# ducha-aiki/pydegensac

Hardware: AMD Instinct MI355X
Metric: models/sec, findFundamentalMatrix @2000 corrs (LO-RANSAC + DEGENSAC, batched pairs) (higher is better)
Workload: dtype f64

## Files before the change

include/mi_degensac.h:

```cpp
#ifndef MI_DEGENSAC_H
#define MI_DEGENSAC_H
#include <stdint.h>

#ifdef __cplusplus
extern "C" {
#endif

#define MI_DEGENSAC_OK        0
#define MI_DEGENSAC_EINVAL   -1
#define MI_DEGENSAC_ENODEV   -2
#define MI_DEGENSAC_EHIP     -3
#define MI_DEGENSAC_ENOMEM   -4

#define MI_DEGENSAC_F_SAMPSON        0
#define MI_DEGENSAC_F_SYMM_EPIPOLAR  1
#define MI_DEGENSAC_H_SAMPSON        0
#define MI_DEGENSAC_H_SYMM_SQ_MAX    1
#define MI_DEGENSAC_H_SYMM_MAX       2
#define MI_DEGENSAC_H_SYMM_SQ_SUM    3
#define MI_DEGENSAC_H_SYMM_SUM       4

#define MI_DEGENSAC_FLAG_FINAL_LAF_FILTER 1u

#define MI_DEGENSAC_FLAG_LEGACY_F 2u
// ... 150 lines not shown
const char *mi_degensac_match_last_error(void);

int mi_degensac_match_knn2_batch_dev(int norm, const void *d_desc1, const void *d_desc2, const int64_t *offsets1_host,
                                     const int64_t *offsets2_host, int n_pairs, int dim, int device, void *stream,
                                     int32_t *d_idx, float *d_dist);
int mi_degensac_match_fginn_knn2_batch_dev(int norm, const void *d_desc1, const void *d_desc2, const int64_t *offsets1_host,
                                           const int64_t *offsets2_host, int n_pairs, int dim, const double *d_kp2, int kp_dim,
                                           double spatial_th, int device, void *stream, int32_t *d_idx, float *d_dist);
typedef struct mi_degensac_match_params {
    int32_t norm;
    int32_t dim;
    float   ratio;
    int32_t mutual;
    int32_t struct_size;
    int32_t second_nn;
    double  spatial_th;
} mi_degensac_match_params;
int mi_degensac_match_verify_batch_dev(int homography, const mi_degensac_match_params *mp, const void *d_desc1, const void *d_desc2,
                                       const int64_t *offsets1_host, const int64_t *offsets2_host, const double *d_kp1, const double *d_kp2,
                                       int kp_dim, int n_pairs, const mi_degensac_params *prm, const uint32_t *d_seeds, int device, void *stream,
                                       double *d_model, int32_t *d_match, uint8_t *d_inlier, int32_t *d_stats, int32_t *h_counts );
int mi_degensac_match_verify_batch(int homography, const mi_degensac_match_params *mp, const void *desc1, const void *desc2,
                                   const int64_t *offsets1, const int64_t *offsets2, const double *kp1, const double *kp2, int kp_dim,
                                   int n_pairs, const mi_degensac_params *prm, const uint32_t *seeds, int device,
                                   double *model, int32_t *match, uint8_t *inlier, int32_t *stats , int32_t *counts );

int mi_degensac_match_knn2_pairs_dev(int norm, const void *d_desc1, const void *d_desc2, const int64_t *offsets1_host, int n_images1,
                                     const int64_t *offsets2_host, int n_images2, const int32_t *pairs_host, int n_pairs, int dim,
                                     int device, void *stream, int32_t *d_idx, float *d_dist);
int mi_degensac_match_verify_pairs_dev(int homography, const mi_degensac_match_params *mp, const void *d_desc1, const void *d_desc2,
                                       const int64_t *offsets1_host, int n_images1, const int64_t *offsets2_host, int n_images2,
                                       const double *d_kp1, const double *d_kp2, int kp_dim, const int32_t *pairs_host, int n_pairs,
                                       const mi_degensac_params *prm, const uint32_t *d_seeds, int device, void *stream, double *d_model,
                                       int32_t *d_match, uint8_t *d_inlier, int32_t *d_stats, int32_t *h_counts );
int mi_degensac_match_verify_pairs(int homography, const mi_degensac_match_params *mp, const void *desc1, const void *desc2,
                                   const int64_t *offsets1, int n_images1, const int64_t *offsets2, int n_images2, const double *kp1,
                                   const double *kp2, int kp_dim, const int32_t *pairs, int n_pairs, const mi_degensac_params *prm,
                                   const uint32_t *seeds, int device, double *model, int32_t *match, uint8_t *inlier,
                                   int32_t *stats , int32_t *counts );

typedef struct mi_degensac_guide_params {
    int32_t homography;
    int32_t error_type;
    double  px_th;
    int32_t struct_size;
    int32_t reserved;
} mi_degensac_guide_params;
int mi_degensac_match_guided_knn2_batch_dev(int norm, const void *d_desc1, const void *d_desc2, const int64_t *offsets1_host,
                                            const int64_t *offsets2_host, int n_pairs, int dim, const double *d_kp1, const double *d_kp2,
                                            int kp_dim, const double *d_models, const mi_degensac_guide_params *gp, int device, void *stream,
                                            int32_t *d_idx, float *d_dist);
int mi_degensac_match_guided_batch_dev(const mi_degensac_match_params *mp, const void *d_desc1, const void *d_desc2, const int64_t *offsets1_host,
                                       const int64_t *offsets2_host, const double *d_kp1, const double *d_kp2, int kp_dim, int n_pairs,
                                       const double *d_models, const mi_degensac_guide_params *gp, int device, void *stream, int32_t *d_idx,
                                       float *d_dist, int32_t *d_match, int32_t *d_counts , int32_t *h_counts );
int mi_degensac_match_guided_batch(const mi_degensac_match_params *mp, const void *desc1, const void *desc2, const int64_t *offsets1,
                                   const int64_t *offsets2, const double *kp1, const double *kp2, int kp_dim, int n_pairs, const double *models,
                                   const mi_degensac_guide_params *gp, int device, int32_t *idx, float *dist, int32_t *match,
                                   int32_t *counts );

int mi_degensac_score_models(const double *pts1, const double *pts2, int n, int dim,
                             const double *models, int n_models, int kind, double th, int device,
                             uint32_t *I, double *J, double *resid );
int mi_degensac_sample_stream(uint32_t seed, int n, int sample_size, int iters, int device,
                              int32_t *samples );
int mi_degensac_sample_stream_ex(uint32_t seed, int n, int sample_size, int iters, int device,
                                 int seq_pool, int32_t *samples);
int mi_degensac_solve7(const double *pts1, const double *pts2, int n, int dim,
                       const int32_t *samples, int n_samples, int device,
                       int32_t *nsol, int32_t *root_idx , double *models );
int mi_degensac_mat3(int op, const double *in, int count, int device, double *out, int32_t *flag);
int mi_degensac_screen_counts(const double *pts1, const double *pts2, int n, int dim, const double *models, int n_models,
                              int kind, double th, int device, uint32_t *c1, uint32_t *c2);

int mi_degensac_screen_counts_h(const double *pts1, const double *pts2, int n, int dim, const double *models, int n_models,
                                double th, int device, uint32_t *cnt, uint8_t *cand);

int mi_degensac_rng_wave(uint32_t seed, int skip, int block, int count, int device, int32_t *out);

#define MI_DEGENSAC_TIMING_LEN 8
int mi_degensac_set_call_timing(int on);
int mi_degensac_last_call_timing(double *out );

int         mi_degensac_device_count(void);
const char *mi_degensac_last_error(void);
const char *mi_degensac_version(void);
const char *mi_degensac_kernel_name(int homography);
int         mi_degensac_pool_stage_parallel(int device);

#ifdef __cplusplus
}
#endif
#endif
```

pydegensac_amd/_lib.py:

```python
import ctypes as C
import os
import numpy as np

_HERE = os.path.dirname(os.path.abspath(__file__))
LIB_PATH = os.environ.get("MI_DEGENSAC_LIB") or os.path.join(_HERE, "libmi_degensac.so")
STATS_LEN = 16
STAT_NAMES = ["samples", "lo_runs", "rejected", "I", "models", "degen", "Ih", "best_sample",
              "full_passes", "ex_passes", "h_passes", "aux_passes", "ticks_best", "ticks_total", "threads", "placement"]
FLAG_FINAL_LAF_FILTER = 1
FLAG_LEGACY_F = 2
FLAG_NO_STREAM, FLAG_STREAM_ON, FLAG_NO_HJOB, FLAG_STREAM_AUTO, FLAG_HJOB_ON = 4, 8, 16, 64, 128


def FLAG_STREAM_TEST(b): return (int(b) & 3) << 8
TUNE_LATENCY, TUNE_THROUGHPUT, TUNE_THROUGHPUT4 = 1, 2, 3
TUNE_PLACE_HBM, TUNE_PLACE_LDS, TUNE_PLACE_POOL_LDS = 1 << 2, 2 << 2, 3 << 2
TUNE_SEQ_POOL = 1 << 4
TUNE_H_SERIAL_LO = 1 << 5
TUNE_COOP_ALL_PASSES = 1 << 6
TUNE_F_SERIAL_REPS = 1 << 7


def TUNE_HELPERS(h): return (int(h) & 255) << 8
def TUNE_SET_ASIDE(t): return (int(t) & 255) << 16
# ... 106 lines not shown
        l.mi_degensac_ctx_destroy.argtypes = [C.c_void_p]
        l.mi_degensac_ctx_stream.restype = C.c_void_p
        l.mi_degensac_ctx_stream.argtypes = [C.c_void_p]
        if hasattr(l, "mi_degensac_ctx_set_scheduling"):
            l.mi_degensac_ctx_set_scheduling.restype = C.c_int
            l.mi_degensac_ctx_set_scheduling.argtypes = [C.c_void_p, C.c_int, C.c_int]
        l.mi_degensac_release_scratch.restype = C.c_int
        l.mi_degensac_release_scratch.argtypes = [C.c_int, C.c_void_p]
        l.mi_degensac_pool_stage_parallel.restype = C.c_int
        l.mi_degensac_pool_stage_parallel.argtypes = [C.c_int]
        l.mi_degensac_sample_stream_ex.restype = C.c_int
        l.mi_degensac_sample_stream_ex.argtypes = [C.c_uint32, C.c_int, C.c_int, C.c_int, C.c_int, C.c_int, ip]
        l.mi_degensac_score_models.restype = C.c_int
        l.mi_degensac_score_models.argtypes = [dp, dp, C.c_int, C.c_int, dp, C.c_int, C.c_int, C.c_double, C.c_int, up, dp, dp]
        l.mi_degensac_sample_stream.restype = C.c_int
        l.mi_degensac_sample_stream.argtypes = [C.c_uint32, C.c_int, C.c_int, C.c_int, C.c_int, ip]
        l.mi_degensac_solve7.restype = C.c_int
        l.mi_degensac_solve7.argtypes = [dp, dp, C.c_int, C.c_int, ip, C.c_int, C.c_int, ip, ip, dp]
        for name in ("mi_degensac_find_fundamental_resids", "mi_degensac_find_homography_resids"):
            f = getattr(l, name); f.restype = C.c_int
            f.argtypes = [dp, dp, C.c_int, C.c_int, pp, C.c_uint32, C.c_int, dp, bp, ip, dp, C.c_int]
        l.mi_degensac_find_fundamental_hist.restype = C.c_int
        l.mi_degensac_find_fundamental_hist.argtypes = [dp, dp, C.c_int, C.c_int, pp, C.c_uint32, C.c_int, dp, bp, ip, ip]
        l.mi_degensac_match.restype = C.c_int
        l.mi_degensac_match.argtypes = [C.c_int, C.c_void_p, C.c_int, C.c_void_p, C.c_int, C.c_int, C.c_float, C.c_int, C.c_int, ip,
                                        C.POINTER(C.c_float), bp]
        l.mi_degensac_match_knn2_dev.restype = C.c_int
        l.mi_degensac_match_knn2_dev.argtypes = [C.c_int, C.c_void_p, C.c_int, C.c_void_p, C.c_int, C.c_int, C.c_int, C.c_void_p, C.c_void_p, C.c_void_p]
        l.mi_degensac_match_filter_dev.restype = C.c_int
        l.mi_degensac_match_filter_dev.argtypes = [C.c_void_p, C.c_void_p, C.c_int, C.c_float, C.c_void_p, C.c_int, C.c_void_p, C.c_void_p]
        l.mi_degensac_match_knn2_batch_dev.restype = C.c_int
        l.mi_degensac_match_knn2_batch_dev.argtypes = [C.c_int, C.c_void_p, C.c_void_p, lp, lp, C.c_int, C.c_int, C.c_int, C.c_void_p, C.c_void_p,
                                                       C.c_void_p]
        if hasattr(l, "mi_degensac_match_fginn_knn2_batch_dev"):
            l.mi_degensac_match_fginn_knn2_batch_dev.restype = C.c_int
            l.mi_degensac_match_fginn_knn2_batch_dev.argtypes = [C.c_int, C.c_void_p, C.c_void_p, lp, lp, C.c_int, C.c_int, C.c_void_p, C.c_int,
                                                                 C.c_double, C.c_int, C.c_void_p, C.c_void_p, C.c_void_p]
        mpp = C.POINTER(MatchParams)
        l.mi_degensac_match_verify_batch_dev.restype = C.c_int
        l.mi_degensac_match_verify_batch_dev.argtypes = [C.c_int, mpp, C.c_void_p, C.c_void_p, lp, lp, C.c_void_p, C.c_void_p, C.c_int, C.c_int, pp,
                                                         C.c_void_p, C.c_int, C.c_void_p, C.c_void_p, C.c_void_p, C.c_void_p, C.c_void_p, ip]
        l.mi_degensac_match_verify_batch.restype = C.c_int
        l.mi_degensac_match_verify_batch.argtypes = [C.c_int, mpp, C.c_void_p, C.c_void_p, lp, lp, dp, dp, C.c_int, C.c_int, pp, up, C.c_int,
                                                     dp, ip, bp, ip, ip]
        if hasattr(l, "mi_degensac_match_knn2_pairs_dev"):
            l.mi_degensac_match_knn2_pairs_dev.restype = C.c_int
            l.mi_degensac_match_knn2_pairs_dev.argtypes = [C.c_int, C.c_void_p, C.c_void_p, lp, C.c_int, lp, C.c_int, ip, C.c_int, C.c_int, C.c_int,
                                                           C.c_void_p, C.c_void_p, C.c_void_p]
            l.mi_degensac_match_verify_pairs_dev.restype = C.c_int
            l.mi_degensac_match_verify_pairs_dev.argtypes = [C.c_int, mpp, C.c_void_p, C.c_void_p, lp, C.c_int, lp, C.c_int, C.c_void_p, C.c_void_p,
                                                             C.c_int, ip, C.c_int, pp, C.c_void_p, C.c_int, C.c_void_p, C.c_void_p, C.c_void_p,
                                                             C.c_void_p, C.c_void_p, ip]
            l.mi_degensac_match_verify_pairs.restype = C.c_int
            l.mi_degensac_match_verify_pairs.argtypes = [C.c_int, mpp, C.c_void_p, C.c_void_p, lp, C.c_int, lp, C.c_int, dp, dp, C.c_int, ip, C.c_int,
                                                         pp, up, C.c_int, dp, ip, bp, ip, ip]
        gpp = C.POINTER(GuideParams)
        l.mi_degensac_match_guided_knn2_batch_dev.restype = C.c_int
        l.mi_degensac_match_guided_knn2_batch_dev.argtypes = [C.c_int, C.c_void_p, C.c_void_p, lp, lp, C.c_int, C.c_int, C.c_void_p, C.c_void_p, C.c_int,
                                                              C.c_void_p, gpp, C.c_int, C.c_void_p, C.c_void_p, C.c_void_p]
        l.mi_degensac_match_guided_batch_dev.restype = C.c_int
        l.mi_degensac_match_guided_batch_dev.argtypes = [mpp, C.c_void_p, C.c_void_p, lp, lp, C.c_void_p, C.c_void_p, C.c_int, C.c_int, C.c_void_p, gpp,
                                                         C.c_int, C.c_void_p, C.c_void_p, C.c_void_p, C.c_void_p, C.c_void_p, ip]
        l.mi_degensac_match_guided_batch.restype = C.c_int
        l.mi_degensac_match_guided_batch.argtypes = [mpp, C.c_void_p, C.c_void_p, lp, lp, dp, dp, C.c_int, C.c_int, dp, gpp, C.c_int, ip,
                                                     C.POINTER(C.c_float), ip, ip]
        l.mi_degensac_kpts_to_xyA.restype = C.c_int
        l.mi_degensac_kpts_to_xyA.argtypes = [C.POINTER(C.c_float), C.c_int, C.c_int, dp]
        l.mi_degensac_kpts_to_xyA_dev.restype = C.c_int
        l.mi_degensac_kpts_to_xyA_dev.argtypes = [C.c_void_p, C.c_int, C.c_int, C.c_void_p, C.c_void_p]
        l.mi_degensac_match_last_error.restype = C.c_char_p
        l.mi_degensac_mat3.restype = C.c_int
        l.mi_degensac_mat3.argtypes = [C.c_int, dp, C.c_int, C.c_int, dp, ip]
        l.mi_degensac_screen_counts.restype = C.c_int
        l.mi_degensac_screen_counts.argtypes = [dp, dp, C.c_int, C.c_int, dp, C.c_int, C.c_int, C.c_double, C.c_int, up, up]
        l.mi_degensac_screen_counts_h.restype = C.c_int
        l.mi_degensac_screen_counts_h.argtypes = [dp, dp, C.c_int, C.c_int, dp, C.c_int, C.c_double, C.c_int, up, bp]
        l.mi_degensac_rng_wave.restype = C.c_int
        l.mi_degensac_rng_wave.argtypes = [C.c_uint32, C.c_int, C.c_int, C.c_int, C.c_int, ip]
        if hasattr(l, "mi_degensac_set_call_timing"):
            l.mi_degensac_set_call_timing.restype = C.c_int
            l.mi_degensac_set_call_timing.argtypes = [C.c_int]
            l.mi_degensac_last_call_timing.restype = C.c_int
            l.mi_degensac_last_call_timing.argtypes = [dp]
        l.mi_degensac_last_error.restype = C.c_char_p
        l.mi_degensac_version.restype = C.c_char_p
        l.mi_degensac_kernel_name.restype = C.c_char_p
        l.mi_degensac_device_count.restype = C.c_int
        _lib = l
    return _lib


def check(rc):
    if rc != 0:
        msg = lib().mi_degensac_last_error().decode()
        if rc == -1:
            raise ValueError(msg)
        raise MiDegensacError(f"mi_degensac error {rc}: {msg}")


def check_match(rc):
    if rc != 0:
        msg = lib().mi_degensac_match_last_error().decode()
        if rc == -1:
            raise ValueError(msg)
        raise MiDegensacError(f"mi_degensac error {rc}: {msg}")


def dptr(a):
    return a.ctypes.data_as(C.POINTER(C.c_double))


def make_params(px_th, conf, max_iters, error_type, sym_check, laf_coef, degen=True, flags=0, tuning=0):
    return Params(float(px_th), float(conf), int(max_iters), int(error_type), int(bool(sym_check)), int(bool(degen)),
                  float(laf_coef), int(flags), int(tuning))


def set_stream_mode(mode):
    f = lib().mi_degensac_set_stream_mode
    f.restype = C.c_int; f.argtypes = [C.c_int]
    return int(f(int(mode)))


def set_hjob_mode(mode):
    f = lib().mi_degensac_set_hjob_mode
    f.restype = C.c_int; f.argtypes = [C.c_int]
    return int(f(int(mode)))


def set_wait_ticks(ticks):
    return int(lib().mi_degensac_set_wait_ticks(int(ticks)))


TIMING_NAMES = ["call_ms", "pack_ms", "enqueue_ms", "wait_ms", "unpack_ms", "dev_h2d_ms", "dev_kernel_ms", "dev_d2h_ms"]


def set_call_timing(on):
    return int(lib().mi_degensac_set_call_timing(int(bool(on))))


def last_call_timing():
    out = (C.c_double * len(TIMING_NAMES))()
    check(lib().mi_degensac_last_call_timing(out))
    return {k: float(v) for k, v in zip(TIMING_NAMES, out)}


def stats_dict(st):
    d = {k: int(v) for k, v in zip(STAT_NAMES, st)}
    d["set_aside"] = (d["placement"] >> 8) & 1
    d["streamed"] = (d["placement"] >> 9) & 1
    d["discarded"] = (d["placement"] >> 10) & 1
    d["rerun"] = (d["placement"] >> 11) & 1
    d["placement"] &= 255
    return d
```

pydegensac_amd/csrc/dg_f_lo.h:

```cpp
#ifndef DG_F_LO_H
#define DG_F_LO_H

__device__ __forceinline__ unsigned dg_hash_list(const int *list, int count, bool small_ids = false)
{
    if (count <= 0) return 0;
    const int lane = (int)(threadIdx.x & 63);
    unsigned hash = (unsigned)__builtin_amdgcn_readfirstlane(count * 4), tmp;
#define DG_HSTEP(v_) { unsigned v = (unsigned)(v_); \
        hash += v & 0xffffu; tmp = ((v >> 16) << 11) ^ hash; hash = (hash << 16) ^ tmp; hash += hash >> 11; }
#define DG_HSTEP16(v_) { unsigned v = (unsigned)(v_); \
        hash += v; hash = (hash << 16) ^ hash; hash += hash >> 11; }
    int k = 0;
    int cur = (lane < count) ? list[lane] : 0;
    int n1 = (64 + lane < count) ? list[64 + lane] : 0, n2 = (128 + lane < count) ? list[128 + lane] : 0, n3 = (192 + lane < count) ? list[192 + lane] : 0;
    for (; k + 64 <= count; k += 64) {
        const int n4 = (k + 256 + lane < count) ? list[k + 256 + lane] : 0;
        if (small_ids) {
#pragma unroll
            for (int i = 0; i < 64; i++) DG_HSTEP16(__builtin_amdgcn_readlane(cur, i))
        } else {
#pragma unroll
            for (int i = 0; i < 64; i++) DG_HSTEP(__builtin_amdgcn_readlane(cur, i))
        }
        cur = n1; n1 = n2; n2 = n3; n3 = n4;
// ... 357 lines not shown
                DG_WSYNC();
                dg_rand_skip(&S->lo_work, assumed, lane);
            }
        }
        __syncthreads();
        DG_LW(0);
        if constexpr (COOP) dg_lo_round_coop<LDSPTS>(c, nr, ssiz, th, mk_full, mk_ex);
        else {
            const int wv = __builtin_amdgcn_readfirstlane(wave);
            if (wv < __builtin_amdgcn_readfirstlane(nr)) dg_lo_rep_wave<LDSPTS>(c, &S->lo[wv], ssiz, th, mk_full, mk_ex, lane, wv);
        }
        __syncthreads();
        DG_LW(1);
        if (tid == 0) {
            int v = 0;
            for (int q = 0; q < nr; q++) {
                dg_lo_log *g = LG(q);
                if (g->aborted) break;
                const int id = *iterID + next + q + 1;
                int draws = 0, cut = 0, n_ex = 0;
                if (g->I0 >= 8) {
                    draws = g->drew0;
                    for (int i = 0; i < g->nit; i++) {
                        n_ex++;
                        const int ret = dg_ht_contains(c.ht, g->it[i].hash, g->it[i].I, id);
                        if (ret == -1) dg_ht_insert(c.ht, g->it[i].hash, g->it[i].I, id);
                        if (ret != -1 && ret != id) { cut = 1; break; }
                        draws += g->it[i].drew;
                    }
                }
                g->cut = cut; g->draws = draws; g->n_ex = n_ex; g->n_fd = (!cut && g->has_fin) ? 2 : 1;
                v++;
                if (draws != assumed) break;
            }
            S->red.bi[0] = v;
        }
        __syncthreads();
        DG_LW(2);
        const int v = S->red.bi[0];
#ifdef DG_LO_PROF
        if (tid == 0) { S->lt[5] += 100000; S->lt[6] += 100000 * v; }
#endif
        for (int q = 0; q < v; q++) {
            const dg_lo_log *g = LG(q);
            c.n_exfds += g->n_ex; c.n_fds += g->n_fd;
            const int cut = g->cut;
            if (!cut && maxS.J < g->J) {
                maxS.I = (unsigned)g->I; maxS.J = g->J; maxS.Is = 0; maxS.Ilafs = 0; *kindBest = g->kind0;
                const int *ibq = COOP ? dg_coop_lo_list(*c.A, c.coop_slot, 2 * q) : c.K->wlist + (size_t)q * c.K->n_max;
                __syncthreads();
                if (tid < 9) Fout[tid] = g->f[tid];
                for (int j = tid; j < g->I; j += DG_T) intbuff_best[j] = ibq[j];
                __syncthreads();
            }
        }
        __syncthreads();
        DG_LW(3);
        if (__builtin_amdgcn_readfirstlane(wave) == 0) {
            for (int q = nr - 1; q >= v; q--) {
                if (lane < 2 * ssiz && LG(q)->upos[lane] >= 0) inliers[LG(q)->upos[lane]] = LG(q)->uval[lane];
                DG_WSYNC();
            }
            if (lane == 0) S->rng = LG(v - 1)->g0;
            DG_WSYNC();
            dg_rand_skip(&S->rng, LG(v - 1)->draws, lane);
        }
        next += v;
        if constexpr (COOP) {
            for (int q = 0; q < v; q++) { const int d = LG(q)->draws; if (d == c.lo_prev || c.lo_prev < 0) assumed = d; c.lo_prev = d; }
        }
#ifdef DG_LO_PROF
        __syncthreads();
#endif
        DG_LW(4);
    }
    if constexpr (COOP) c.lo_assumed = assumed;
    *iterID += DG_RAN_REP;
    __syncthreads();
    for (int j = tid; j < (int)maxS.I; j += DG_T) inliers[j] = intbuff_best[j];
    __syncthreads();
    return maxS;
}

template <int LDSPTS>
__device__ __forceinline__ dg_score dg_inFrani(CTX &c, int ninl, double th, double *Fout, int *iterID, int mk_full, int mk_ex, int *kindBest)
{
    if (c.rrun || c.A->innerh_serial || c.A->trace) return dg_inFrani_serial<LDSPTS>(c, ninl, th, Fout, iterID, mk_full, mk_ex, kindBest);
    if (c.cb) {
        if constexpr (LDSPTS == 0) return dg_inFrani_waves<LDSPTS, true>(c, ninl, th, Fout, iterID, mk_full, mk_ex, kindBest);
        else return dg_inFrani_serial<LDSPTS>(c, ninl, th, Fout, iterID, mk_full, mk_ex, kindBest);
    }
    return dg_inFrani_waves<LDSPTS, false>(c, ninl, th, Fout, iterID, mk_full, mk_ex, kindBest);
}

#endif
```

pydegensac_amd/csrc/dg_f_sched.h:

```cpp
#ifndef DG_F_SCHED_H
#define DG_F_SCHED_H

#define DG_FLAST(M) do { if (legacy_sym) { __syncthreads(); if (tid < 9) S->flast[tid] = (M)[tid]; D.flast_k = no_sam; __syncthreads(); } } while (0)
#define DG_PARK_SPARE   0
#define DG_PARK_CLAIMED 32
#define DG_PARK_HEAD    64
#define DG_PARK_DYN_OFF ((sizeof(dg_f_shared) + 255) & ~(size_t)255)

__device__ __forceinline__ void dg_copy16(void *dst, const void *src, size_t bytes, int tid)
{
    const size_t nv = bytes / 16;
    const uint4 *s4 = (const uint4 *)src; uint4 *d4 = (uint4 *)dst;
    for (size_t i = tid; i < nv; i += DG_T) d4[i] = s4[i];
    const size_t done = nv * 16;
    for (size_t i = done + tid; i < bytes; i += DG_T) ((unsigned char *)dst)[i] = ((const unsigned char *)src)[i];
}

__device__ __forceinline__ long long dg_park_take(const dg_args &A, long long *bc , const int q)
{
    __syncthreads();
    if (__builtin_amdgcn_readfirstlane((int)(threadIdx.x >> 6)) == 0) {
        int *const p_head = A.park_ctl + DG_PARK_HEAD + 64 * q, *const p_cl = A.park_ctl + DG_PARK_CLAIMED + 64 * q;
        const long long *const pq = A.park_q + (size_t)q * A.park_cap;
        int h;
        for (;;) {
            h = __builtin_amdgcn_readfirstlane(__hip_atomic_load(p_head, __ATOMIC_RELAXED, __HIP_MEMORY_SCOPE_AGENT));
            const int cl = __builtin_amdgcn_readfirstlane(__hip_atomic_load(p_cl, __ATOMIC_RELAXED, __HIP_MEMORY_SCOPE_AGENT));
            if (h >= cl) { h = -1; break; }
            int ok = 0;
            if (threadIdx.x == 0) {
                int expect = h;
                ok = __hip_atomic_compare_exchange_strong(p_head, &expect, h + 1, __ATOMIC_RELAXED, __ATOMIC_RELAXED, __HIP_MEMORY_SCOPE_AGENT) ? 1 : 0;
            }
            if (__builtin_amdgcn_readfirstlane(ok)) break;
        }
        long long e = -1;
        if (h >= 0) {
            for (;;) {
                const long long v = __hip_atomic_load(pq + h, __ATOMIC_RELAXED, __HIP_MEMORY_SCOPE_AGENT);
                const int lo = __builtin_amdgcn_readfirstlane((int)(v & 0xffffffffll)), hi = __builtin_amdgcn_readfirstlane((int)(v >> 32));
                e = ((long long)hi << 32) | (unsigned)lo;
                if (e >= 0) break;
                __builtin_amdgcn_s_sleep(4);
            }
            __builtin_amdgcn_fence(__ATOMIC_ACQUIRE, "agent");
        }
        *bc = e;
    }
    __syncthreads();
    return *bc;
}

#define DG_STREAM_TIMEOUT 400000000ll
__device__ __forceinline__ dg_stream_ent *dg_stream_entry(const dg_args &A, int oslot, int seq)
{
    return (dg_stream_ent *)(A.ring + ((size_t)oslot * A.stream_depth + (size_t)(seq % A.stream_depth)) * A.stream_ent_bytes);
}
template <class Pred>
__device__ __forceinline__ int dg_stream_wait(const dg_args &A, int *flag, int *stop, Pred pred, int *bc , const long long limit = DG_STREAM_TIMEOUT)
{
    __syncthreads();
    if (__builtin_amdgcn_readfirstlane((int)(threadIdx.x >> 6)) == 0) {
        const long long t0 = wall_clock64();
        int v;
        for (;;) {
            v = __builtin_amdgcn_readfirstlane(__hip_atomic_load(flag, __ATOMIC_RELAXED, __HIP_MEMORY_SCOPE_AGENT));
            if (pred(v) && limit != 0) break;
            if (stop && __builtin_amdgcn_readfirstlane(__hip_atomic_load(stop, __ATOMIC_RELAXED, __HIP_MEMORY_SCOPE_AGENT))) { v = -1; break; }
            if (wall_clock64() - t0 > limit) { if (threadIdx.x == 0) __hip_atomic_store(A.err_flag, 1, __ATOMIC_RELAXED, __HIP_MEMORY_SCOPE_AGENT); v = -1;
                break; }
            __builtin_amdgcn_s_sleep(8);
        }
        __builtin_amdgcn_fence(__ATOMIC_ACQUIRE, "agent");
        *bc = v;
    }
    __syncthreads();
    return *bc;
}
__device__ __forceinline__ void dg_stream_publish(int *flag, int v)
{
    __syncthreads();
    if (__builtin_amdgcn_readfirstlane((int)(threadIdx.x >> 6)) == 0) {
        __builtin_amdgcn_fence(__ATOMIC_RELEASE, "agent");
        asm volatile("s_waitcnt vmcnt(0)" ::: "memory");
        if (threadIdx.x == 0) __hip_atomic_store(flag, v, __ATOMIC_RELAXED, __HIP_MEMORY_SCOPE_AGENT);
    }
// ... 49 lines not shown
```

pydegensac_amd/csrc/dg_kernel_common.h:

```cpp
#ifndef DG_KERNEL_COMMON_H
#define DG_KERNEL_COMMON_H
#include "dg_geom.h"

#ifndef DG_CHUNK
#define DG_CHUNK   256
#endif
#ifdef MI_DEGENSAC_DEV
#define DG_CLK() wall_clock64()
#define DG_DEVT(x) x
#else
#define DG_CLK() 0ll
#define DG_DEVT(x) do {} while (0)
#endif
#ifndef DG_MINW
#define DG_MINW    2
#endif
#define DG_MCAP    96
#define DG_HT_CAP  4096
#define DG_MTAB_BYTES ((((size_t)3 * DG_CHUNK * 9 * sizeof(double)) + 255) & ~(size_t)255)
#define DG_PRE_BYTES  ((size_t)DG_CHUNK * 2 * sizeof(int))

#define DG_ITER_SAM 50
#define DG_RAN_REP 10
#define DG_ILSQ_ITERS 4
#define DG_TC 4
#define DG_MWM (9/4)

struct dg_params {
    double th;
    double sym_th;
    double laf_coef;
    double conf;
    int    max_iters;
    int    error_type;
    int    degen;
    int    final_laf_filter;
    int    h2_do_lo, h2_inl_limit;
    int    legacy;
};

struct dg_ws_layout {
    size_t stride;
    size_t off_lists;
    size_t off_flags;
    size_t off_ht;
    size_t off_models;
    size_t off_pts;
    size_t off_pool;
    size_t off_stage;
    size_t off_wave;
    size_t off_res;
    size_t off_mslot;
    size_t off_park;
    size_t off_hjbuf;
    size_t off_job;
    size_t off_hrep;
    int    hrep;
    int    n_max;
};

struct dg_hrep_it { double hl[9]; double J; unsigned hash; int I; };
struct alignas(128) dg_hrep_log {
    double h0[9]; double J0; int I0;
    int nit;
    int last_short;
    int has_fin;
    dg_hrep_it it[4];
    double hf[9]; double Jf; int If;
    int ids[12];
};

struct dg_coop_cb {
    int gen;
    int done;
    int next;
    int fpad0;
    unsigned long long tau_bits;
    int fpad[26];
    int stage, n_units, Mtot, n, kind, slice, use_l1, err;
    double th, ext[4];
    int mtab, mpad;
    double ppad[6];
};
static_assert(sizeof(dg_coop_cb) == 256, "control block = two 128-byte lines");

struct dg_coop_job {
    double F[9], thJ, thL, thL2;
    int kind, wantJ, listStrict, has_list, has_list2, slice, n, pad;
};
struct dg_coop_rec { unsigned I, nL, nL2, nJ; };
#define DG_COOP_MAX_SLICES 64

enum { DG_ST_IDLE = 0, DG_ST_REQ = 1, DG_ST_BUSY = 2, DG_ST_ATTACHED = 3, DG_ST_RELEASED = 4 };
struct dg_stream_cb {
    int state;
    int head;
    int tail;
    int stop;
    int owner_sam;
    int max_sam;
    unsigned long long tau_bits;
    int claim;
    int fpad[23];
    int pair, wsid, img_sam, fan_kind;
    double fan_th, fan_ext[4];
    int ppad[18];
};
static_assert(sizeof(dg_stream_cb) == 256, "stream control block = two 128-byte lines");

struct dg_hjob_cb {
    int gen;
    int next;
    int done;
    int fpad[29];
    int n, kind, ssiz, wsid; double th; int ppad[26];
};
static_assert(sizeof(dg_hjob_cb) == 256, "job control block = two 128-byte lines");

struct dg_args {
    const double *pts1, *pts2;
    const long long *offsets;
    const unsigned *seeds;
    double *model_out;
    unsigned char *mask_out;
    int *stats_out;
    char *ws;
    dg_ws_layout wl;
    dg_params prm;
    int dim, n_pairs, pts_in_lds;
    int dev_knob;
    double *resids_out;
    int resid_runs;
    int lo_width;
    int *hist_out;
    int *screen_out;
    int *ticket;
    const int *order;
    int coop_k;
    int coop_pass_min;
    dg_coop_cb *coop;
    int park_sam;
    int n_res, n_ws;
    int dyn_bytes;
    int *park_ctl;
    long long *park_q;
    int park_cap;
    int park_long;
    int lo_serial;
    int pool_seq;
    int innerh_serial;
    int variant_threads, mode;
    int stream_on;
    int stream_early;
    int stream_min_sam, stream_min_left;
    int stream_depth;
    int stream_test;
    size_t stream_ent_bytes;
    dg_stream_cb *scb;
    char *ring;
    int *done_pairs;
    dg_hjob_cb *hjob;
    int fan_k;
    int fan_ws0;
    int *fan_flags;
    int *err_flag;
    int *trace;
    int trace_cap;
    int wait_ticks;
    long long *phase_out;
};

__device__ __forceinline__ bool dg_wait_count(const dg_args &A, int *cnt, int target, int code, int sleep_ticks)
{
    const long long t0 = wall_clock64(), limit = (long long)A.wait_ticks;
    for (;;) {
// ... 194 lines not shown
```

pydegensac_amd/csrc/dg_kernel_f.h:

```cpp
#ifndef DG_KERNEL_F_H
#define DG_KERNEL_F_H
#include <stddef.h>
#include "dg_lsq.h"

struct dg_score { unsigned I; double J; unsigned Is; unsigned Ilafs; };

#define DG_WPAD ((2 * DG_CHUNK * 7 * 4 > DG_NW * (int)sizeof(dg_wave_ws)) ? (2 * DG_CHUNK * 7 * 4 - DG_NW * (int)sizeof(dg_wave_ws) + 7) / 8 : 1)
struct dg_f_drv {
    dg_score maxS, maxSs;
    int no_sam, max_sam, iter_cnt, degen_cnt, iterID, Ihmax; unsigned non_degen;
    int best_sample; long long t_best, t_start;
    long long t_parked;
    int flast_k, has_last;
    int finKind, accepted, perm[4], p4, e4kind, track, done;
    unsigned seed; int cur, chunk_s[3], chunk_base;
    int n_fds, n_exfds, n_hds, n_aux;
};

#ifndef DG_LO_AHEAD_MAX
#define DG_LO_AHEAD_MAX 5
#endif
#define DG_LO_AHEAD (DG_NW - 1 < DG_LO_AHEAD_MAX ? DG_NW - 1 : DG_LO_AHEAD_MAX)
struct dg_lo_ahead { dg_rng before, after; int pos[32], val[32]; double F[9]; };

// ... 76 lines not shown

struct dg_stream_ev { double model[9]; double J; unsigned I; short k; unsigned char r, pad; unsigned char ridx[4]; };
#define DG_STREAM_EV_MAX 40
struct dg_stream_ent {
    int cn, Mtot, n_ev, overflow; double tau_used, pad1;
    unsigned seeds[DG_CHUNK]; int draws[DG_CHUNK][8];
    unsigned char nv[DG_CHUNK];
    dg_stream_ev ev[DG_STREAM_EV_MAX];
};

template <int LDSPTS>
struct dg_f_ctx {
    dg_f_shared *S;
    const __attribute__((address_space(3))) dg_f_cshared *K;
    const dg_pt *P;
    int *pool;
    int n, tid;
    const dg_args *A;
    long long off;
    dg_ht ht;
    unsigned *seeds; int (*draws)[8];
    int n_fds, n_exfds, n_hds, n_aux;
    double *rrun;
    dg_coop_cb *cb; int *coop_gen; int coop_slot;
    double *hlt;
    int hjob_gen;
    int lo_assumed, lo_prev;

    __device__ __forceinline__ dg_pt pt(int i) const { return P[i]; }
    __device__ __forceinline__ dg_pt laf_pt(int i, int which) const {
        const double *a = A->pts1 + (size_t)(off + i) * 6, *b = A->pts2 + (size_t)(off + i) * 6;
        dg_pt p;
        if (which == 1) { p.x1 = a[0] + a[3]; p.y1 = a[1] + a[5]; p.x2 = b[0] + b[3]; p.y2 = b[1] + b[5]; }
        else            { p.x1 = a[0] + a[2]; p.y1 = a[1] + a[4]; p.x2 = b[0] + b[2]; p.y2 = b[1] + b[4]; }
        return p;
    }
};

#define DG_JBUF_LDS_BYTES (offsetof(dg_f_shared, wpad) + sizeof(((dg_f_shared *)0)->wpad) - offsetof(dg_f_shared, ww))
static_assert(offsetof(dg_f_shared, wpad) == offsetof(dg_f_shared, ww) + sizeof(((dg_f_shared *)0)->ww), "ww and wpad must be contiguous");
static_assert(DG_JBUF_LDS_BYTES >= 2 * DG_CHUNK * 7 * sizeof(int), "pool-stage scratch does not fit");

__device__ __forceinline__ void dg_fill_views(dg_f_cshared *K, char *ws, const dg_ws_layout &wl)
{
    for (int i = 0; i < 10; i++) K->L[i] = (int *)(ws + wl.off_lists) + (size_t)i * wl.n_max;
    for (int i = 0; i < 5; i++) K->Fl[i] = (unsigned char *)(ws + wl.off_flags) + (size_t)i * wl.n_max;
    K->gmodels = (double *)(ws + wl.off_models);
    K->stage = (dg_pt *)(ws + wl.off_stage);
    K->res_J = (double *)(ws + wl.off_res); K->res_I = (unsigned *)(K->res_J + 3 * DG_CHUNK); K->rf = (int (*)[5])(K->res_I + 3 * DG_CHUNK);
    K->hrep = wl.hrep ? ws + wl.off_hrep : (char *)0;
    K->n_max = wl.n_max; K->wlist = (int *)(ws + wl.off_wave); K->wstage = (dg_pt *)(ws + wl.off_wave + (size_t)DG_NW * wl.n_max * sizeof(int));
}

#define CTX dg_f_ctx<LDSPTS>
#define DG_RESIDS_M 62

template <int LDSPTS>
__device__ __forceinline__ void dg_dump_resid(CTX &c, int row, const double *M, int kind)
{
    if (!c.rrun) return;
    double m[9], Hinv[9], H1[9];
#pragma unroll
    for (int i = 0; i < 9; i++) { m[i] = M[i]; Hinv[i] = 0; H1[i] = 0; }
    if (kind > 10) dg_hsym_prepare(m, Hinv, H1);
    double *out = c.rrun + (size_t)row * c.n;
    for (int j = c.tid; j < c.n; j += DG_T) {
        const dg_pt q = dg_ldpt<LDSPTS>(c.P, j);
        out[j] = kind < 10 ? dg_Ferr(kind, m, q) : dg_Herr(kind - 10, m, Hinv, H1, q);
    }
}
template <int LDSPTS>
__device__ __forceinline__ void dg_resid_begin(CTX &c, int run )
{
    c.rrun = 0;
    if (!c.A->resids_out || run >= c.A->resid_runs) return;
    c.rrun = c.A->resids_out + ((size_t)c.off * c.A->resid_runs + (size_t)run * c.n) * DG_RESIDS_M;
    const double nan_ = __longlong_as_double(0x7ff8000000000000ll);
    for (size_t j = c.tid; j < (size_t)DG_RESIDS_M * c.n; j += DG_T) c.rrun[j] = nan_;
}

#define DG_TRACE(c, tag, I, J) do { if ((c).A->trace && (c).tid == 0) { int *t_ = (c).A->trace; int k_ = t_[0]; \
    if (k_ < (c).A->trace_cap) { long long jb_ = __double_as_longlong((double)(J)); t_[1+4*k_] = (tag); t_[2+4*k_] = (int)(I); \
    t_[3+4*k_] = (int)(jb_ & 0xffffffffll); t_[4+4*k_] = (int)(jb_ >> 32); t_[0] = k_ + 1; } } } while (0)

template <int LDSPTS>
__device__ __noinline__ dg_pass_res dg_coop_pass(CTX &c, const double *Fm , int kind, const dg_pass_cfg &cfg);

template <int LDSPTS>
__device__ __forceinline__ dg_pass_res dg_f_pass(CTX &c, const double *Fm , int kind, dg_pass_cfg cfg)
{
    if (LDSPTS == 0 && c.cb && !cfg.src && !cfg.flags && !cfg.wantC && cfg.n >= c.A->coop_pass_min) return dg_coop_pass<LDSPTS>(c, Fm, kind, cfg);
    double F[9];
#pragma unroll
    for (int i = 0; i < 9; i++) F[i] = Fm[i];
    const dg_pt *P = c.P;
    cfg.jbuf = (double *)c.K->stage; cfg.jl = (double *)c.S->ww; cfg.jl_cap = (int)(DG_JBUF_LDS_BYTES / sizeof(double));
    return dg_pass(&c.S->red, cfg, [&](int pid, int) { return dg_Ferr(kind, F, dg_ldpt<LDSPTS>(P, pid)); }, c.tid);
}
template <int LDSPTS>
__device__ __forceinline__ dg_pass_res dg_h_pass(CTX &c, const double *Hm , dg_pass_cfg cfg)
{
    double H[9];
#pragma unroll
    for (int i = 0; i < 9; i++) H[i] = Hm[i];
    const dg_pt *P = c.P;
    cfg.jbuf = (double *)c.K->stage; cfg.jl = (double *)c.S->ww; cfg.jl_cap = (int)(DG_JBUF_LDS_BYTES / sizeof(double));
    return dg_pass(&c.S->red, cfg, [&](int pid, int) { dg_pt p = dg_ldpt<LDSPTS>(P, pid); return dg_HDs(H, p.x1, p.y1, p.x2, p.y2); }, c.tid);
}
__device__ __forceinline__ dg_pass_cfg dg_cfg0(int n)
{
    dg_pass_cfg c; c.n = n; c.src = 0; c.p0 = 0; c.wantJ = 0; c.thJ = 0; c.jbuf = 0; c.jl = 0; c.jl_cap = 0; c.wantC = 0; c.thC = 0; c.list = 0; c.thL = 0;
        c.listStrict = 0; c.list2 = 0; c.thL2 = 0; c.flags = 0; c.thF = 0;
    return c;
}

template <int LDSPTS>
__device__ __forceinline__ void dg_gather(CTX &c, const int *ids, int len, double *px)
{
    for (int i = 0; i < len; i++) { dg_pt p = dg_ldpt<LDSPTS>(c.P, ids[i]); px[4*i] = p.x1; px[4*i+1] = p.y1; px[4*i+2] = p.x2; px[4*i+3] = p.y2; }
}

template <int LDSPTS>
__device__ __forceinline__ void dg_gather_wave(CTX &c, int id, int len, double *px, int lane)
{
    if (lane < len) { dg_pt p = dg_ldpt<LDSPTS>(c.P, id); px[4*lane] = p.x1; px[4*lane+1] = p.y1; px[4*lane+2] = p.x2; px[4*lane+3] = p.y2; }
}

template <int LDSPTS>
__device__ __forceinline__ void dg_u2f_list(CTX &c, const int *list, int len, const double *wmodel, int wkind, double *Fout)
{
    dg_f_shared *S = c.S;
    if (len <= 16) {
        __syncthreads();
        if (c.tid < 64) {
            const int lane = c.tid;
            dg_gather_wave(c, lane < len ? list[lane] : 0, len, S->lsq.px, lane);
            if (wmodel && lane < len) {
                dg_pt q = dg_ldpt<LDSPTS>(c.P, list[lane]);
                if (wkind == DG_K_FDS) S->lsq.part[0][lane] = dg_exFDs_w(wmodel, q.x1, q.y1, q.x2, q.y2);
                else { double w; dg_exFDsSym(wmodel, q.x1, q.y1, q.x2, q.y2, &w); S->lsq.part[0][lane] = w; }
            }
            DG_WSYNC();
            dg_u2f_small_w(&S->lsq, S->lsq.px, wmodel ? S->lsq.part[0] : 0, len, Fout, c.tid);
        }
        __syncthreads();
    } else {
        const dg_pt *P = c.P;
        dg_u2f_big(&S->red, &S->lsq, [&](int i) { return dg_ldpt<LDSPTS>(P, i); }, list, len, c.tid, Fout, c.K->stage, 2 * c.K->n_max,
                   DG_LSQ_LTAB(S));
    }
}

template <int LDSPTS>
__device__ __forceinline__ int dg_f_checks(CTX &c, const double *f, const int *list, int cnt, dg_score &S, const dg_score &maxS, int mkind)
{
    const dg_params &pr = c.A->prm;
    if (pr.sym_th > 0) {
        dg_pass_cfg cfg = pr.legacy ? dg_cfg0(c.n) : dg_cfg0(cnt); if (!pr.legacy) cfg.src = list; cfg.wantC = 1; cfg.thC = pr.sym_th;
        dg_pass_res r = dg_f_pass(c, f, DG_K_FSYM, cfg);
        S.Is = r.C;
        if (S.Is < maxS.Is) return 0;
    }
    if (pr.laf_coef > 0) {
        double thl = pr.laf_coef * pr.th;
        double F[9];
        for (int i = 0; i < 9; i++) F[i] = f[i];
        dg_pass_cfg cfg = dg_cfg0(cnt); cfg.src = list; cfg.wantC = 1; cfg.thC = thl;
        dg_pass_res r1 = dg_pass(&c.S->red, cfg, [&](int pid, int) { return dg_Ferr(mkind, F, c.laf_pt(pid, 1)); }, c.tid);
        dg_pass_res r2 = dg_pass(&c.S->red, cfg, [&](int pid, int) { return dg_Ferr(mkind, F, c.laf_pt(pid, 2)); }, c.tid);
        S.Ilafs = r2.C < r1.C ? r2.C : r1.C;
        if (S.Ilafs < maxS.Ilafs) { if (c.tid == 0) c.S->n_lafrej++; return 0; }
    }
    return 1;
}

template <int LDSPTS>
__device__ __noinline__ int dg_checksample(CTX &c, const double *F , const double (*u7)[4] , double th, double *H )
{
    dg_f_shared *S = c.S; const int tid = c.tid, lane = tid & 63, wave = tid >> 6;
    __syncthreads();
#if DG_NW >= 5
    for (int tr = wave; tr < 5; tr += DG_NW) {
        dg_wave_ws *w = &S->ww[wave];
        const unsigned char IDXS[5][3] = {{0,1,2}, {3,4,5}, {0,1,6}, {3,4,6}, {2,5,6}};
        if (lane == 0) {
            dg_Hdetect(F, u7, IDXS[tr], w->H);
            for (int j = 0; j < 7; j++) { w->Ds[j] = dg_HDs(w->H, u7[j][0], u7[j][1], u7[j][2], u7[j][3]); w->sDs[j] = w->Ds[j]; w->idx[j] = j; }
            for (int a = 0; a < 7; ++a)
                for (int b = a + 1; b < 7; ++b)
                    if (w->sDs[b] < w->sDs[a]) { double t = w->sDs[b]; w->sDs[b] = w->sDs[a]; w->sDs[a] = t; int ti = w->idx[b]; w->idx[b] = w->idx[a];
                        w->idx[a] = ti; }
            for (int j = 0; j < 5; ++j) { const double *q = u7[w->idx[j]]; w->cpx[4*j] = q[0]; w->cpx[4*j+1] = q[1]; w->cpx[4*j+2] = q[2]; w->cpx[4*j+3] = q[3];
                }
        }
        DG_WSYNC();
        dg_u2h_norm_w(w, w->cpx, 5, w->H, lane);
        if (lane == 0) {
            int inlCount = 0;
            for (int j = 0; j < 7; ++j) if (dg_HDs(w->H, u7[j][0], u7[j][1], u7[j][2], u7[j][3]) < th) ++inlCount;
            S->csRes[tr] = inlCount > 4;
            for (int j = 0; j < 9; j++) S->csH[tr][j] = w->H[j];
        }
        DG_WSYNC();
    }
#else
    static_assert(sizeof(dg_lsq_scratch) >= (size_t)DG_NW * DG_X2_DOUBLES * sizeof(double), "second-problem scratch");
    for (int base = wave; base < 5; base += 2 * DG_NW) {
        dg_wave_ws *w = &S->ww[wave];
        double *x2 = (double *)&S->lsq + (size_t)wave * DG_X2_DOUBLES;
        const bool uph = lane >= 32, two = base + DG_NW < 5, mine = (lane & 31) == 0 && (!uph || two);
        const int tr = uph ? base + DG_NW : base;
        double *Hh = uph ? x2 + DG_X2_USER : w->H, *Ds = uph ? x2 + DG_X2_USER + 9 : w->Ds, *sDs = uph ? x2 + DG_X2_USER + 16 : w->sDs;
        int *idx = uph ? (int *)(x2 + DG_X2_USER + 23) : w->idx;
        double *cpx = uph ? x2 + DG_X2_USER + 27 : w->cpx;
        const unsigned char IDXS[5][3] = {{0,1,2}, {3,4,5}, {0,1,6}, {3,4,6}, {2,5,6}};
        if (mine) {
            dg_Hdetect(F, u7, IDXS[tr], Hh);
            for (int j = 0; j < 7; j++) { Ds[j] = dg_HDs(Hh, u7[j][0], u7[j][1], u7[j][2], u7[j][3]); sDs[j] = Ds[j]; idx[j] = j; }
            for (int a = 0; a < 7; ++a)
                for (int b = a + 1; b < 7; ++b)
                    if (sDs[b] < sDs[a]) { double t = sDs[b]; sDs[b] = sDs[a]; sDs[a] = t; int ti = idx[b]; idx[b] = idx[a]; idx[a] = ti; }
            for (int j = 0; j < 5; ++j) { const double *q = u7[idx[j]]; cpx[4*j] = q[0]; cpx[4*j+1] = q[1]; cpx[4*j+2] = q[2]; cpx[4*j+3] = q[3]; }
        }
        DG_WSYNC();
        dg_fit_norm_w2<true>(w, x2, w->cpx, x2 + DG_X2_USER + 27, 5, w->H, two ? x2 + DG_X2_USER : (double *)0, lane);
        if (mine) {
            int inlCount = 0;
            for (int j = 0; j < 7; ++j) if (dg_HDs(Hh, u7[j][0], u7[j][1], u7[j][2], u7[j][3]) < th) ++inlCount;
            S->csRes[tr] = inlCount > 4;
            for (int j = 0; j < 9; j++) S->csH[tr][j] = Hh[j];
        }
        DG_WSYNC();
    }
#endif
    __syncthreads();
    int win = -1;
    for (int i = 4; i >= 0; i--) if (S->csRes[i]) win = i;
    if (win >= 0 && tid < 9) H[tid] = S->csH[win][tid];
    __syncthreads();
    return win >= 0;
}
// ... 232 lines not shown
        }
        itJ = mJ;
    }
    DG_WSYNC();
    if (lane < 9) lg->h[lane] = h[lane];
    if (lane == 0) { lg->itJ = itJ; lg->passes = passes; lg->draws = draws; __hip_atomic_store(&lg->pub, draws, __ATOMIC_RELAXED, __HIP_MEMORY_SCOPE_WORKGROUP);
        }
    DG_WSYNC();
}

template <int LDSPTS>
__device__ __noinline__ unsigned dg_innerH_waves(CTX &c, double *H , double th, unsigned inlLimit, unsigned char *inl_flags)
{
    dg_f_shared *S = c.S; const int n = c.n, tid = c.tid, lane = tid & 63, wave = tid >> 6;
    int *inliers = c.K->L[3], *bak = c.K->L[4];
    const int lim = (int)inlLimit;
    dg_pass_cfg cfg = dg_cfg0(n); cfg.list = inliers; cfg.thL = th;
    dg_pass_res r0 = dg_h_pass(c, H, cfg); c.n_hds++;
    const int ninl = (int)r0.nL;
    if (ninl >= 8) {
        int ssiz = ninl / 2; if (ssiz > 12) ssiz = 12;
        double maxJ = 0;
        int next = 0;
        while (next < DG_RAN_REP) {
            const int nr = DG_RAN_REP - next < DG_NW ? DG_RAN_REP - next : DG_NW;
            __syncthreads();
            if (__builtin_amdgcn_readfirstlane(wave) == 0) {
                if (lane == 0) { S->ih_start = S->rng; S->ih_work = S->rng; }
                for (int j = lane; j < ninl; j += 64) bak[j] = inliers[j];
                DG_WSYNC();
                for (int q = 0; q < nr; q++) {
                    int id = 0;
                    dg_randsubset_wave(&S->ih_work, inliers, ninl, ssiz, lane, &id);
                    if (lane < ssiz) S->ih[q].ids[lane] = id;
                    if (lane == 0) { S->ih[q].g = S->ih_work; S->ih[q].pub = -1; S->ih[q].aborted = 0; }
                    DG_WSYNC();
                    dg_rand_skip(&S->ih_work, 5 * (int)lim, lane);
                }
            }
            __syncthreads();
            if (wave < nr) dg_innerH_rep_wave<LDSPTS>(c, &S->ih[wave], ssiz, th, lim, lane, wave);
            __syncthreads();
            int v = 0;
            for (int q = 0; q < nr; q++) {
                if (S->ih[q].aborted) break;
                c.n_hds += S->ih[q].passes;
                if (maxJ < S->ih[q].itJ) { maxJ = S->ih[q].itJ; __syncthreads(); if (tid < 9) H[tid] = S->ih[q].h[tid]; __syncthreads(); }
                v++;
                if (S->ih[q].draws != 5 * lim) break;
            }
            __syncthreads();
            if (__builtin_amdgcn_readfirstlane(wave) == 0) {
                if (lane == 0) S->rng = S->ih[v - 1].g;
                if (v < nr) {
                    for (int j = lane; j < ninl; j += 64) inliers[j] = bak[j];
                    if (lane == 0) S->ih_work = S->ih_start;
                    DG_WSYNC();
                    for (int q = 0; q < v; q++) {
                        int id = 0;
                        dg_randsubset_wave(&S->ih_work, inliers, ninl, ssiz, lane, &id);
                        dg_rand_skip(&S->ih_work, S->ih[q].draws, lane);
                    }
                }
            }
            next += v;
        }
        __syncthreads();
    }
    {
        double Hr[9]; for (int i = 0; i < 9; i++) Hr[i] = H[i];
        const dg_pt *P = c.P;
        unsigned cnt = 0;
        for (int base = 0; base < n; base += DG_T) {
            int j = base + tid; bool in = false;
            if (j < n) { dg_pt p = dg_ldpt<LDSPTS>(P, j); in = dg_HDs(Hr, p.x1, p.y1, p.x2, p.y2) <= th; inl_flags[j] = in ? 1 : 0; }
            cnt += in ? 1u : 0u;
        }
        cnt = dg_block_sum_u(&c.S->red, cnt, tid);
        __syncthreads();
        return cnt;
    }
}

template <int LDSPTS>
__device__ __forceinline__ unsigned dg_innerH(CTX &c, double *H , double th, unsigned inlLimit, unsigned char *inl_flags)
{
    if (c.A->innerh_serial || inlLimit > 12) return dg_innerH_serial<LDSPTS>(c, H, th, inlLimit, inl_flags);
    return dg_innerH_waves<LDSPTS>(c, H, th, inlLimit, inl_flags);
}

template <int LDSPTS>
__device__ __forceinline__ unsigned dg_wave_count_lt(const dg_pt *P, int n, const double *F, double thr, int lane)
{
    unsigned cnt = 0;
    for (int p0 = lane; p0 < n; p0 += 64 * DG_PU) {
        dg_pt q[DG_PU];
#pragma unroll
        for (int u = 0; u < DG_PU; u++) { const int p = p0 + 64 * u; q[u] = dg_ldpt<LDSPTS>(P, p < n ? p : p0); }
#pragma unroll
        for (int u = 0; u < DG_PU; u++) cnt += (p0 + 64 * u < n && dg_FDs(F, q[u].x1, q[u].y1, q[u].x2, q[u].y2) < thr) ? 1u : 0u;
    }
    return dg_wave_sum_u(cnt);
}
template <int LDSPTS>
__device__ __forceinline__ unsigned dg_wave_list_lt(const dg_pt *P, int n, const double *F, double thr, int *list, int lane)
{
    unsigned off = 0;
    for (int base = 0; base < n; base += 64 * DG_PU) {
        dg_pt q[DG_PU]; bool in[DG_PU];
#pragma unroll
        for (int u = 0; u < DG_PU; u++) { const int p = base + 64 * u + lane; q[u] = dg_ldpt<LDSPTS>(P, p < n ? p : 0); }
#pragma unroll
        for (int u = 0; u < DG_PU; u++) in[u] = base + 64 * u + lane < n && dg_FDs(F, q[u].x1, q[u].y1, q[u].x2, q[u].y2) < thr;
#pragma unroll
        for (int u = 0; u < DG_PU; u++) {
            const unsigned long long b = __ballot(in[u]);
            if (in[u]) list[off + (unsigned)__popcll(b & ((1ull << lane) - 1ull))] = base + 64 * u + lane;
            off += (unsigned)__popcll(b);
        }
    }
    return off;
}

template <int LDSPTS>
__device__ __forceinline__ unsigned dg_wave_list_lt_stage(const dg_pt *P, int n, const double *F, double thr, int *list, dg_pt *stage_, int lane)
{
    typedef __attribute__((address_space(1))) double dg_gdbl;
    dg_gdbl *stage = (dg_gdbl *)(double *)stage_;
    unsigned off = 0;
    for (int base = 0; base < n; base += 64 * DG_PU) {
        dg_pt q[DG_PU]; bool in[DG_PU];
#pragma unroll
        for (int u = 0; u < DG_PU; u++) { const int p = base + 64 * u + lane; q[u] = dg_ldpt<LDSPTS>(P, p < n ? p : 0); }
#pragma unroll
        for (int u = 0; u < DG_PU; u++) in[u] = base + 64 * u + lane < n && dg_FDs(F, q[u].x1, q[u].y1, q[u].x2, q[u].y2) < thr;
#pragma unroll
        for (int u = 0; u < DG_PU; u++) {
            const unsigned long long b = __ballot(in[u]);
            if (in[u]) {
                const unsigned pos = off + (unsigned)__popcll(b & ((1ull << lane) - 1ull));
                list[pos] = base + 64 * u + lane;
                dg_gdbl *o = stage + 4 * (size_t)pos; o[0] = q[u].x1; o[1] = q[u].y1; o[2] = q[u].x2; o[3] = q[u].y2;
            }
            off += (unsigned)__popcll(b);
        }
    }
    return off;
}

template <int LDSPTS>
__device__ __noinline__ unsigned dg_u2Fit_wave(dg_wave_ws *w, const dg_pt *P, int n, double *F, double th, double ths, unsigned iters,
                                              int *list, dg_pt *stage, int stage_cap, int lane, double *thf, int *n_aux)
{
    double dth = (ths - th) / (iters - 1);
    for (unsigned iter = 0; iter < iters; ++iter) {
        double Fr[9];
#pragma unroll
        for (int i = 0; i < 9; i++) Fr[i] = F[i];
        unsigned cnt = dg_wave_list_lt_stage<LDSPTS>(P, n, Fr, ths, list, stage, lane); (*n_aux)++;
        if (cnt < 8) { *thf = ths; return cnt; }
        DG_WSYNC();
        if (cnt <= 14) {
            if (lane < (int)cnt) { dg_pt q = dg_ldpt<LDSPTS>(P, list[lane]); w->px[4*lane] = q.x1; w->px[4*lane+1] = q.y1; w->px[4*lane+2] = q.x2;
                w->px[4*lane+3] = q.y2; }
            DG_WSYNC();
            if (cnt > 8) dg_u2f_norm_w(w, w->px, (const double *)0, (int)cnt, F, lane);
            else {
                if (lane == 0) { for (int i = 0; i < 72; i++) w->Z[i] = 0.;
                    for (int i = 0; i < 8; i++) { double a[3] = {w->px[4*i], w->px[4*i+1], 1.0}, b[3] = {w->px[4*i+2], w->px[4*i+3], 1.0};
                    for (int k = 0; k < 3; k++) for (int l = 0; l < 3; l++) w->Z[(k*3+l)*8 + i] = b[k] * a[l]; } }
// ... 281 lines not shown
```

pydegensac_amd/csrc/dg_kernel_f_main.h:

```cpp
#ifndef DG_KERNEL_F_MAIN_H
#define DG_KERNEL_F_MAIN_H
#include "dg_kernel_f.h"
#include "dg_score_tiles.h"

#include "dg_f_lo.h"
#include "dg_f_solve7.h"
#include "dg_f_sampler.h"
#include "dg_f_score.h"
#include "dg_f_sched.h"
#include "dg_f_fan.h"
#include "dg_f_coop.h"

template <int T, int LDSPTS>
__device__ __forceinline__ int dg_f_pair(const dg_args &A, dg_f_shared *S, unsigned char *dyn_smem, const int pair, const int slot, const int wsid,
                                         const int resume, int &coop_gen, const int own_wsid, const int oslot)
{
    const int producer = resume == 2;
    dg_stream_cb *const scb = (A.stream_on || A.fan_k > 0) ? A.scb + oslot : (dg_stream_cb *)0;
    int head_seen = 0;
    int gpar = 0, pend_draws = 0;
    int mtab = 0, presolved = 0;
    int strm = 0, img_sam = 0;
    const int coopK = LDSPTS == 0 ? A.coop_k : 0;
    dg_coop_cb *const cb = coopK > 0 ? A.coop + slot : (dg_coop_cb *)0;
    const int tid = threadIdx.x, lane = tid & 63, wave = tid >> 6;
    const bool fan = LDSPTS == 0 && A.fan_k > 0 && coopK > 0 && !resume && !(A.prm.legacy && A.prm.sym_th > 0);
    const bool deep = DG_NW >= 8 && LDSPTS == 0 && coopK > 0 && !A.hist_out && !fan;
    const long long off = A.offsets[pair];
    const int n = (int)(A.offsets[pair + 1] - off);
    const dg_params &pr = A.prm;
    const double th = pr.th;

    char *ws = A.ws + (size_t)wsid * A.wl.stride;
    char *const wsown = A.ws + (size_t)own_wsid * A.wl.stride;
    CTX c;
    c.S = S; c.K = (const __attribute__((address_space(3))) dg_f_cshared *)&S->K; c.n = n; c.tid = tid; c.A = &A; c.off = off;
    __syncthreads();
    if (tid == 0) dg_fill_views(&S->K, wsown, A.wl);
    __syncthreads();
    c.ht.heads = (int *)(ws + A.wl.off_ht); c.ht.count = c.ht.heads + 64; c.ht.ent = c.ht.heads + 80;
    c.seeds = S->seeds3[0]; c.draws = S->draws3[0];
    c.n_fds = c.n_exfds = c.n_hds = c.n_aux = 0; c.rrun = 0; c.hlt = (double *)0;
    c.cb = cb; c.coop_gen = &coop_gen; c.coop_slot = slot; c.lo_assumed = DG_LO_ASSUMED_DRAWS; c.lo_prev = -1;
    dg_pt *Pw; int *pool;
    if (LDSPTS == 1) { Pw = (dg_pt *)dyn_smem; pool = (int *)(dyn_smem + (size_t)n * sizeof(dg_pt)); }
    else             { Pw = (dg_pt *)(ws + A.wl.off_pts); pool = LDSPTS == 2 ? (int *)dyn_smem : (int *)(ws + A.wl.off_pool); }
    c.P = Pw; c.pool = pool;
    const dg_pt *P = Pw;
    int *const pscr = A.pool_seq ? (int *)0 : (int *)S->ww;

    const int mk_full = pr.error_type == 1 ? DG_K_FSYM : DG_K_FDS;
    const int mk_ex   = pr.error_type == 1 ? DG_K_EXFSYM : DG_K_FDS;
    const int doSym = pr.sym_th > 0, doLaf = pr.laf_coef > 0;
    const int legacy_sym = pr.legacy && doSym;

    dg_f_drv D;
    dg_score &maxS = D.maxS, &maxSs = D.maxSs;
    int &no_sam = D.no_sam, &max_sam = D.max_sam, &iter_cnt = D.iter_cnt, &degen_cnt = D.degen_cnt, &iterID = D.iterID, &Ihmax = D.Ihmax;
    unsigned &non_degen = D.non_degen;
    int &best_sample = D.best_sample; long long &t_best = D.t_best, &t_start = D.t_start;
    int &finKind = D.finKind, &accepted = D.accepted;
    int (&perm)[4] = D.perm, &p4 = D.p4, &e4kind = D.e4kind, &track = D.track;
    double *e4F = S->bufF[0];
    int &done = D.done;
    unsigned &seed = D.seed;
    int &cur = D.cur, (&chunk_s)[3] = D.chunk_s, &chunk_base = D.chunk_base;
    int park_on = (A.park_sam > 0 && !resume) ? 1 : 0;

  if (!resume) {
    t_start = wall_clock64();
    double ex0 = 0., ex1 = 0., ex2 = 0., ex3 = 0.;
    for (int i = tid; i < n; i += DG_T) {
        const double *a = A.pts1 + (size_t)(off + i) * A.dim, *b = A.pts2 + (size_t)(off + i) * A.dim;
        dg_pt p; p.x1 = a[0]; p.y1 = a[1]; p.x2 = b[0]; p.y2 = b[1];
        Pw[i] = p; pool[i] = i;
        ex0 = fmax(ex0, fabs(p.x1)); ex1 = fmax(ex1, fabs(p.y1)); ex2 = fmax(ex2, fabs(p.x2)); ex3 = fmax(ex3, fabs(p.y2));
    }
#pragma unroll
    for (int o = 32; o >= 1; o >>= 1) {
        ex0 = fmax(ex0, __shfl_xor(ex0, o, 64)); ex1 = fmax(ex1, __shfl_xor(ex1, o, 64));
        ex2 = fmax(ex2, __shfl_xor(ex2, o, 64)); ex3 = fmax(ex3, __shfl_xor(ex3, o, 64));
    }
    if (lane == 0) { S->extw[wave][0] = ex0; S->extw[wave][1] = ex1; S->extw[wave][2] = ex2; S->extw[wave][3] = ex3; }
    dg_ht_init(c.ht, tid);
    if (A.hist_out) for (int j = tid; j < n + 3; j += DG_T) A.hist_out[(size_t)off + 3 * (size_t)pair + j] = 0;
    if (tid < 9) { S->F[tid] = 0; S->FBest[tid] = 0; }
    if (tid == 0) { S->n_lafrej = 0; S->scnt[0] = S->scnt[1] = S->scnt[2] = S->scnt[3] = 0; }
    __syncthreads();
    if (tid < 4) { double e = 0.; for (int w = 0; w < DG_NW; w++) e = fmax(e, S->extw[w][tid]); S->ext[tid] = e; }
    __syncthreads();

    maxS.I = 8; maxS.J = 0; maxS.Is = 0; maxS.Ilafs = 0; maxSs = maxS;
    no_sam = 0; max_sam = pr.max_iters; iter_cnt = 0; degen_cnt = 0; iterID = 0; Ihmax = 0;
    non_degen = 0;
    best_sample = 0; t_best = t_start;
    finKind = mk_full; accepted = 0;
    perm[0] = 0; perm[1] = 1; perm[2] = 2; perm[3] = 3; p4 = 3; e4kind = mk_full; track = 1;
    done = 0;
    D.flast_k = 0; D.has_last = 0;
    if (coopK > 0 && tid == 0) __hip_atomic_store(&cb->tau_bits, 0ull, __ATOMIC_RELAXED, __HIP_MEMORY_SCOPE_AGENT);

    if (__builtin_amdgcn_readfirstlane(wave) == 0) { dg_srand_wave(&S->rng, A.seeds[pair], lane); const int v_ = dg_rand_block(&S->rng, 1, lane);
        if (lane == 0) S->itmp[31] = v_; }
    __syncthreads();
    seed = (unsigned)S->itmp[31];
    __syncthreads();

    DG_DEVT(if (tid == 0) { for (int i = 0; i < 8; i++) { S->ph[i] = 0; S->dbg[i] = 0; } S->tq = DG_CLK(); });
#ifdef DG_LO_PROF
    if (tid == 0) { for (int i = 0; i < 16; i++) S->lt[i] = 0; S->ltq = wall_clock64(); }
#endif
#define DG_PH(i) DG_DEVT(if (tid == 0) { long long tq2_ = DG_CLK(); S->ph[i] += tq2_ - S->tq; S->tq = tq2_; })
    cur = 0; chunk_s[0] = chunk_s[1] = chunk_s[2] = 0; chunk_base = 0;
    if (tid == 0) S->itmp[23] = 0;
    {
        const int first = (A.stream_on || coopK > 0) ? DG_CHUNK : (DG_CHUNK < 64 ? DG_CHUNK : 64);
        int cn0 = max_sam - no_sam; if (cn0 > first) cn0 = first; if (cn0 < 0) cn0 = 0;
        int cn1 = max_sam - no_sam - cn0; if (cn1 > DG_CHUNK) cn1 = DG_CHUNK; if (cn1 < 0) cn1 = 0;
        chunk_s[0] = cn0; chunk_s[1] = cn1;
        if (wave == 0) {
            unsigned sd = seed;
            if (cn0 > 0) sd = dg_sample_chunk<7, LDSPTS>(sd, cn0, n, pool, S->seeds3[0], S->draws3[0], S->alm3[0], pscr, lane);
            if (cn1 > 0) sd = dg_sample_draws<7>(sd, cn1, n, S->seeds3[1], S->draws3[1], S->alm3[1], lane);
            if (deep) {
                int cn2_ = max_sam - no_sam - cn0 - cn1; if (cn2_ > DG_CHUNK) cn2_ = DG_CHUNK; if (cn2_ < 0) cn2_ = 0;
                if (cn1 > 0) dg_sample_pool<7, LDSPTS>(cn1, n, pool, S->draws3[1], S->alm3[1], pscr, lane, S->dbg);
                if (cn2_ > 0) sd = dg_sample_draws<7>(sd, cn2_, n, S->seeds3[2], S->draws3[2], S->alm3[2], lane);
            }
            if (lane == 0) S->itmp[31] = (int)sd;
        }
        if (deep) { int cn2_ = max_sam - no_sam - cn0 - cn1; if (cn2_ > DG_CHUNK) cn2_ = DG_CHUNK; if (cn2_ < 0) cn2_ = 0; chunk_s[2] = cn2_; }
        __syncthreads();
        seed = (unsigned)S->itmp[31];
        if (fan) {
            if (tid == 0) {
                scb->pair = pair; scb->wsid = wsid; scb->img_sam = 0; scb->fan_kind = mk_full; scb->fan_th = th;
                for (int i = 0; i < 4; i++) scb->fan_ext[i] = S->ext[i];
                __hip_atomic_store(&scb->tau_bits, 0ull, __ATOMIC_RELAXED, __HIP_MEMORY_SCOPE_AGENT);
                __hip_atomic_store(&scb->max_sam, max_sam, __ATOMIC_RELAXED, __HIP_MEMORY_SCOPE_AGENT);
                __hip_atomic_store(&scb->tail, 0, __ATOMIC_RELAXED, __HIP_MEMORY_SCOPE_AGENT);
                __hip_atomic_store(&scb->head, 0, __ATOMIC_RELAXED, __HIP_MEMORY_SCOPE_AGENT);
                __hip_atomic_store(&scb->claim, 0, __ATOMIC_RELAXED, __HIP_MEMORY_SCOPE_AGENT);
                __hip_atomic_store(&scb->stop, 0, __ATOMIC_RELAXED, __HIP_MEMORY_SCOPE_AGENT);
            }
            dg_stream_publish(&scb->state, DG_ST_ATTACHED);
            strm = 2;
        }
    }
  } else {
    const char *pk = ws + A.wl.off_park;
    dg_copy16(S, pk, sizeof(dg_f_shared), tid);
    dg_copy16(dyn_smem, pk + DG_PARK_DYN_OFF, (size_t)A.dyn_bytes, tid);
    __syncthreads();
    if (tid == 0) dg_fill_views(&S->K, wsown, A.wl);
    D = S->park;
    { const long long waited = wall_clock64() - D.t_parked; D.t_start += waited; D.t_best += waited; }
    c.n_fds = D.n_fds; c.n_exfds = D.n_exfds; c.n_hds = D.n_hds; c.n_aux = D.n_aux;
    DG_DEVT(if (tid == 0) S->tq = DG_CLK());
    __syncthreads();
  }
    auto write_image = [&]() {
        D.n_fds = c.n_fds; D.n_exfds = c.n_exfds; D.n_hds = c.n_hds; D.n_aux = c.n_aux; D.t_parked = wall_clock64();
        __syncthreads();
        if (tid == 0) S->park = D;
        __syncthreads();
        char *pk = ws + A.wl.off_park;
        dg_copy16(pk, S, sizeof(dg_f_shared), tid);
        dg_copy16(pk + DG_PARK_DYN_OFF, dyn_smem, (size_t)A.dyn_bytes, tid);
        if (tid == 0) { scb->pair = pair; scb->wsid = wsid; scb->img_sam = no_sam; }
    };
    while (!done && no_sam < max_sam) {
        int coop_no_ev = 0;
        int pre_cnt = 0, cn3 = 0;
        int ff = 0, tail_p = 0;
        int seq = no_sam / DG_CHUNK;
        dg_stream_ent *ent = (dg_stream_ent *)0;
        if (producer) {
            __syncthreads();
            if (tid == 0) {
                S->itmp[24] = __hip_atomic_load(&scb->stop, __ATOMIC_RELAXED, __HIP_MEMORY_SCOPE_AGENT);
                S->itmp[25] = __hip_atomic_load(&scb->tail, __ATOMIC_RELAXED, __HIP_MEMORY_SCOPE_AGENT);
                S->itmp[26] = __hip_atomic_load(&scb->max_sam, __ATOMIC_RELAXED, __HIP_MEMORY_SCOPE_AGENT);
            }
            __syncthreads();
            const int stop_ = S->itmp[24], tail_ = S->itmp[25], omax_ = S->itmp[26];
            tail_p = tail_;
            __syncthreads();
            if (stop_) break;
            if (omax_ < max_sam) max_sam = omax_;
            if (no_sam >= max_sam) break;
            ff = seq < tail_;
            if (!ff) {
                if (seq - tail_ >= A.stream_depth) {
                    const int depth_ = A.stream_depth;
                    if (dg_stream_wait(A, &scb->tail, &scb->stop, [=](int t) { return seq - t < depth_; }, &S->itmp[28], A.wait_ticks) < 0) break;
                }
                ent = dg_stream_entry(A, oslot, seq);
            }
        } else if (scb) {
            if (strm >= 1 && tid == 0) {
                const double tau_ = maxS.J < maxSs.J ? maxS.J : maxSs.J;
                __hip_atomic_store(&scb->tau_bits, (unsigned long long)__double_as_longlong(tau_ < 0 ? 0.0 : tau_), __ATOMIC_RELAXED, __HIP_MEMORY_SCOPE_AGENT);
                __hip_atomic_store(&scb->max_sam, max_sam, __ATOMIC_RELAXED, __HIP_MEMORY_SCOPE_AGENT);
                __hip_atomic_store(&scb->tail, seq, __ATOMIC_RELAXED, __HIP_MEMORY_SCOPE_AGENT);
            }
            if (strm < 2 && !legacy_sym && no_sam >= A.stream_min_sam && max_sam - no_sam >= A.stream_min_left && (strm == 1 || (seq & 3) == 0 ||
                no_sam < 1024)) {
                __syncthreads();
                if (tid == 0) {
                    int act = 0;
                    if (strm == 0) {
                        if ((A.stream_test & 2) || A.stream_early || __hip_atomic_load(A.ticket, __ATOMIC_RELAXED, __HIP_MEMORY_SCOPE_AGENT) >= A.n_pairs) {
                            int e = DG_ST_IDLE;
                            if (__hip_atomic_compare_exchange_strong(&scb->state, &e, DG_ST_BUSY, __ATOMIC_RELAXED, __ATOMIC_RELAXED,
                                __HIP_MEMORY_SCOPE_AGENT)) act = 1;
                        }
                    } else {
                        const int st_ = __hip_atomic_load(&scb->state, __ATOMIC_RELAXED, __HIP_MEMORY_SCOPE_AGENT);
                        if (st_ == DG_ST_REQ) {
                            if (no_sam - img_sam >= 8192) {
                                int e = DG_ST_REQ;
                                if (__hip_atomic_compare_exchange_strong(&scb->state, &e, DG_ST_BUSY, __ATOMIC_RELAXED, __ATOMIC_RELAXED,
                                    __HIP_MEMORY_SCOPE_AGENT)) {
                                    act = 1; __hip_atomic_fetch_add(A.done_pairs + 1, -1, __ATOMIC_RELAXED, __HIP_MEMORY_SCOPE_AGENT);
                                }
                            }
                        } else if (__hip_atomic_load(&scb->head, __ATOMIC_RELAXED, __HIP_MEMORY_SCOPE_AGENT) > seq) act = 2;
                    }
                    S->itmp[30] = act;
                }
                __syncthreads();
                const int act = S->itmp[30];
                __syncthreads();
                if (act == 1) {
                    if (tid == 0) {
                        const double tau_ = maxS.J < maxSs.J ? maxS.J : maxSs.J;
                        __hip_atomic_store(&scb->tau_bits, (unsigned long long)__double_as_longlong(tau_ < 0 ? 0.0 : tau_), __ATOMIC_RELAXED,
                            __HIP_MEMORY_SCOPE_AGENT);
                        __hip_atomic_store(&scb->max_sam, max_sam, __ATOMIC_RELAXED, __HIP_MEMORY_SCOPE_AGENT);
                        __hip_atomic_store(&scb->tail, seq, __ATOMIC_RELAXED, __HIP_MEMORY_SCOPE_AGENT);
                        __hip_atomic_store(&scb->head, 0, __ATOMIC_RELAXED, __HIP_MEMORY_SCOPE_AGENT);
                        __hip_atomic_store(&scb->stop, 0, __ATOMIC_RELAXED, __HIP_MEMORY_SCOPE_AGENT);
                        __hip_atomic_store(&scb->owner_sam, (int)(t_start >> 10), __ATOMIC_RELAXED, __HIP_MEMORY_SCOPE_AGENT);
                    }
                    write_image();
                    dg_stream_publish(&scb->state, DG_ST_REQ);
                    if (tid == 0) __hip_atomic_fetch_add(A.done_pairs + 1, 1, __ATOMIC_RELAXED, __HIP_MEMORY_SCOPE_AGENT);
                    strm = 1; img_sam = no_sam; park_on = 0;
                } else if (act == 2) strm = 2;
            }
        }
        if (fan) {
            DG_PH(3);
            {
                const double tau_now = maxS.J < maxSs.J ? maxS.J : maxSs.J;
                __syncthreads();
                if (__builtin_amdgcn_readfirstlane(wave) == 0) {
                    int cnt = 0, ns = no_sam, msum = 0;
                    const bool fl_ = __hip_atomic_load(dg_fan_flag(A, oslot, seq + lane), __ATOMIC_RELAXED, __HIP_MEMORY_SCOPE_AGENT) == seq + lane + 1;
                    const unsigned long long nb_ = ~__ballot(fl_);
                    const int nready = nb_ ? __ffsll((long long)nb_) - 1 : 64;
                    __builtin_amdgcn_fence(__ATOMIC_ACQUIRE, "agent");
                    for (int s_ = seq; cnt < nready; s_++) {
                        const dg_stream_ent *q_ = dg_stream_entry(A, oslot, s_);
                        const int cn_ = __builtin_amdgcn_readfirstlane(q_->cn), mt_ = __builtin_amdgcn_readfirstlane(q_->Mtot);
                        const int ne_ = __builtin_amdgcn_readfirstlane(q_->n_ev), ov_ = __builtin_amdgcn_readfirstlane(q_->overflow);
                        const double tu_ = q_->tau_used;
                        const bool quiet = ne_ == 0 && !ov_ && !(tu_ > tau_now) && !(A.stream_test & 1) && ns >= DG_ITER_SAM && cn_ > 0 && ns + cn_ < max_sam;
                        if (!__builtin_amdgcn_readfirstlane(quiet ? 1 : 0)) break;
                        ns += cn_; msum += mt_; cnt++;
                    }
                    if (lane == 0) { S->itmp[20] = cnt; S->itmp[21] = ns; S->itmp[22] = msum; }
                }
                __syncthreads();
                if (S->itmp[20] > 0) {
                    DG_DEVT(if (tid == 0) S->dbg[5] += 100000ll * S->itmp[20]);
                    no_sam = S->itmp[21]; c.n_fds += S->itmp[22]; track = 0;
                    seq = no_sam / DG_CHUNK;
                    if (tid == 0) __hip_atomic_store(&scb->tail, seq, __ATOMIC_RELAXED, __HIP_MEMORY_SCOPE_AGENT);
                }
                __syncthreads();
            }
            DG_PH(2);
            {
                const int want = seq + 1;
                if (dg_stream_wait(A, dg_fan_flag(A, oslot, seq), (int *)0, [=](int v) { return v == want; }, &S->itmp[28], A.wait_ticks) < 0) { done = 1;
                    break; }
            }
            DG_PH(0);
        }
        if (park_on && no_sam >= A.park_sam) {
            park_on = 0;
            __syncthreads();
            if (tid == 0) {
                int nw = -1;
                if (__hip_atomic_load(A.ticket, __ATOMIC_RELAXED, __HIP_MEMORY_SCOPE_AGENT) < A.n_pairs) {
                    nw = A.n_res + __hip_atomic_fetch_add(A.park_ctl + DG_PARK_SPARE, 1, __ATOMIC_RELAXED, __HIP_MEMORY_SCOPE_AGENT);
                    if (nw >= A.n_ws) nw = -1;
                }
                S->itmp[30] = nw;
            }
            __syncthreads();
            const int nw = S->itmp[30];
            __syncthreads();
            if (nw >= 0) {
                D.n_fds = c.n_fds; D.n_exfds = c.n_exfds; D.n_hds = c.n_hds; D.n_aux = c.n_aux; D.t_parked = wall_clock64();
                DG_DEVT(if (A.phase_out && tid == 0) { long long *o_ = A.phase_out + ((size_t)A.n_pairs + 4096 + pair) * 16; o_[0] = max_sam - no_sam;
                    o_[1] = iter_cnt; o_[2] = degen_cnt; o_[3] = D.t_parked - t_start; o_[4] = (long long)maxS.I; });
                if (tid == 0) S->park = D;
                __syncthreads();
                char *pk = ws + A.wl.off_park;
                dg_copy16(pk, S, sizeof(dg_f_shared), tid);
                dg_copy16(pk + DG_PARK_DYN_OFF, dyn_smem, (size_t)A.dyn_bytes, tid);
                __syncthreads();
                const int q = (max_sam - no_sam >= A.park_long) ? 1 : 0;
                if (__builtin_amdgcn_readfirstlane(tid >> 6) == 0) {
                    int idx = 0;
                    if (tid == 0) idx = __hip_atomic_fetch_add(A.park_ctl + DG_PARK_CLAIMED + 64 * q, 1, __ATOMIC_RELAXED, __HIP_MEMORY_SCOPE_AGENT);
                    idx = __builtin_amdgcn_readfirstlane(idx);
                    __builtin_amdgcn_fence(__ATOMIC_RELEASE, "agent");
                    asm volatile("s_waitcnt vmcnt(0)" ::: "memory");
                    if (tid == 0) __hip_atomic_store(A.park_q + (size_t)q * A.park_cap + idx, ((long long)pair << 32) | (long long)(unsigned)wsid,
                        __ATOMIC_RELAXED, __HIP_MEMORY_SCOPE_AGENT);
                }
                return nw;
            }
        }
        int chunk = chunk_s[cur]; if (chunk > max_sam - no_sam) chunk = max_sam - no_sam;
        c.seeds = S->seeds3[cur]; c.draws = S->draws3[cur]; chunk_base = no_sam;
        DG_PH(3);
        DG_PH(0);
        int Mtot = 0, nxt = cur, cn2 = 0;
        double tau_scored = 0.0;
      int full = 1;
      if (strm == 2) {
        if (!fan && seq >= head_seen) {
            const int h_ = dg_stream_wait(A, &scb->head, (int *)0, [=](int h) { return h > seq; }, &S->itmp[28], A.wait_ticks);
            if (h_ < 0) { done = 1; break; }
            head_seen = h_;
        }
        DG_PH(0);
        const dg_stream_ent *e_ = dg_stream_entry(A, oslot, seq);
        __syncthreads();
        if (tid == 0) { S->itmp[24] = e_->cn; S->itmp[25] = e_->Mtot; S->itmp[26] = e_->n_ev; S->itmp[27] = e_->overflow; S->dtmp[31] = e_->tau_used; }
        __syncthreads();
        const int cn_ = S->itmp[24], n_ev = S->itmp[26], ovf = S->itmp[27];
        const double tau_used = S->dtmp[31], tau_now = A.hist_out ? 0.0 : (maxS.J < maxSs.J ? maxS.J : maxSs.J);
        if (n_ev == 0 && !ovf && !(tau_used > tau_now) && !(A.stream_test & 1) && no_sam >= DG_ITER_SAM && cn_ > 0 && no_sam + cn_ < max_sam) {
            const int Mt_ = S->itmp[25];
            __syncthreads();
            track = 0;
            no_sam += cn_; c.n_fds += Mt_;
            DG_DEVT(if (tid == 0) S->dbg[5] += 100000);
            continue;
        }
        if (fan) {
            c.seeds = (unsigned *)e_->seeds; c.draws = (int (*)[8])e_->draws;
        } else {
            for (int i = tid; i < DG_CHUNK; i += DG_T) {
                S->seeds3[cur][i] = e_->seeds[i];
#pragma unroll
                for (int q = 0; q < 8; q++) S->draws3[cur][i][q] = e_->draws[i][q];
            }
        }
        __syncthreads();
        chunk = cn_ < max_sam - no_sam ? cn_ : max_sam - no_sam;
        full = ovf || tau_used > tau_now || (A.stream_test & 1);
        __syncthreads();
        if (!full) {
            const unsigned char nvb = tid < DG_CHUNK ? e_->nv[tid] : (unsigned char)0;
            const unsigned v = (tid < chunk && nvb != 255) ? (unsigned)nvb : 0u;
            unsigned incl = v;
#pragma unroll
            for (int o = 1; o < 64; o <<= 1) { unsigned t = __shfl_up(incl, o, 64); if (lane >= o) incl += t; }
            if (lane == 63) S->wave_cnt[wave] = incl;
            __syncthreads();
            unsigned wbase = 0;
            for (int w = 0; w < wave; w++) wbase += S->wave_cnt[w];
            const unsigned excl = wbase + incl - v;
            if (tid < DG_CHUNK) {
                S->moff[tid] = (unsigned short)excl; S->nv[tid] = nvb; S->nsolv[tid] = 0;
                for (unsigned r = 0; r < v; r++) S->mslot[excl + r] = (unsigned short)(tid * 3 + r);
            }
            if (tid == DG_T - 1) S->moff[DG_CHUNK] = (unsigned short)(excl + v);
            __syncthreads();
            Mtot = (int)S->moff[DG_CHUNK];
            for (int i = tid; i < Mtot; i += DG_T) { c.K->res_I[i] = 0; c.K->res_J[i] = 0; }
            __syncthreads();
            for (int e = tid; e < n_ev; e += DG_T) {
                const dg_stream_ev *ev = &e_->ev[e];
                const int k_ = ev->k, r_ = ev->r, mi = (int)S->moff[k_] + r_;
                c.K->res_I[mi] = ev->I; c.K->res_J[mi] = ev->J;
#pragma unroll
                for (int j = 0; j < 9; j++) c.K->gmodels[(size_t)(k_ * 3 + r_) * 9 + j] = ev->model[j];
#pragma unroll
                for (int q = 0; q < 4; q++) S->ridx[k_][q] = ev->ridx[q];
            }
            __syncthreads();
            c.n_fds += Mtot;
            tau_scored = tau_used;
        }
      }
      if (full) {
        const bool fuse = DG_NW >= 8 && !(LDSPTS == 0 && coopK > 0) && strm != 2 && !ff;
        if (fuse) { __syncthreads(); if (tid == 0) { S->itmp[21] = 0; S->itmp[22] = 0; } __syncthreads(); }
        int nvalid = 0, nullbad = 0; unsigned rixp = 0;
        if (presolved >= chunk && chunk > 0) {
            if (tid < chunk) { const int *pre = (const int *)(ws + A.wl.off_models + 2 * DG_MTAB_BYTES) + 2 * tid; const int a_ = pre[0]; nvalid = a_ & 0xff;
                nullbad = (a_ >> 8) & 1; rixp = (unsigned)pre[1]; }
        } else
        if (!fuse && !ff && tid < chunk) {
            int r_ = dg_solve7_lane(P, c.draws[tid], c.K->gmodels + (size_t)tid * 27, &rixp, (double *)&S->ww[wave]);
            if (r_ < 0) nullbad = 1; else nvalid = r_;
        }
        if (!fuse) {
            unsigned v = (unsigned)nvalid, incl = v;
#pragma unroll
            for (int o = 1; o < 64; o <<= 1) { unsigned t = __shfl_up(incl, o, 64); if (lane >= o) incl += t; }
            if (lane == 63) S->wave_cnt[wave] = incl;
            __syncthreads();
            unsigned wbase = 0;
            for (int w = 0; w < wave; w++) wbase += S->wave_cnt[w];
            unsigned excl = wbase + incl - v;
            if (tid < chunk) {
                S->moff[tid] = (unsigned short)excl;
                S->nv[tid] = nullbad ? 255 : (unsigned char)nvalid;
                S->nsolv[tid] = (unsigned char)((rixp >> 8) & 3u);
                for (int r = 0; r < nvalid; r++) {
                    S->ridx[tid][r] = (unsigned char)((rixp >> (2*r)) & 3u);
                    S->mslot[excl + r] = (unsigned short)(tid * 3 + r);
                }
            }
            if (tid == DG_T - 1) S->moff[DG_CHUNK] = (unsigned short)(excl + v);
            __syncthreads();
        }
        Mtot = (ff || fuse) ? 0 : __builtin_amdgcn_readfirstlane((int)S->moff[DG_CHUNK]);
        double tau_c = A.hist_out ? 0.0 : (maxS.J < maxSs.J ? maxS.J : maxSs.J);
        if (producer) {
            __syncthreads();
            if (tid == 0) S->dtmp[31] = __longlong_as_double((long long)__hip_atomic_load(&scb->tau_bits, __ATOMIC_RELAXED, __HIP_MEMORY_SCOPE_AGENT));
            __syncthreads();
            tau_c = S->dtmp[31];
            __syncthreads();
        }
        tau_scored = tau_c;
        const bool coop_screen = th != 0 && tau_c >= 4.0;
        int coop_units = 0;
        if (LDSPTS == 0 && coopK > 0) {
            const dg_coop_ws cv = dg_coop_views(A, slot);
            unsigned short *gms = (unsigned short *)(ws + A.wl.off_mslot);
            for (int i = tid; i < Mtot; i += DG_T) { gms[i] = S->mslot[i]; cv.cnt[i] = 0u; if (!coop_screen) cv.surv[i] = (unsigned short)i; }
            int slice = (n + DG_COOP_SPW * (coopK + 1) - 1) / (DG_COOP_SPW * (coopK + 1)); if (slice < 64 * DG_PU * 4) slice = 64 * DG_PU * 4;
            slice = (slice + 64 * DG_PU - 1) / (64 * DG_PU) * (64 * DG_PU);
            coop_units = coop_screen ? (n + slice - 1) / slice : Mtot;
            if (tid == 0) cb->mtab = mtab;
            if (coop_units > 0) dg_coop_publish(cb, coop_gen, coop_screen ? 1 : 2, coop_units, Mtot, n, mk_full, slice, 0, th, S->ext, tau_c);
        }

        DG_PH(1);
        nxt = cur == 2 ? 0 : cur + 1; const int nx2 = nxt == 2 ? 0 : nxt + 1;
        {
            if (deep) {
                cn3 = max_sam - (no_sam + chunk_s[cur] + chunk_s[nxt] + chunk_s[nx2]); if (cn3 > DG_CHUNK) cn3 = DG_CHUNK; if (cn3 < 0) cn3 = 0;
            } else {
                cn2 = max_sam - (no_sam + chunk_s[cur] + chunk_s[nxt]); if (cn2 > DG_CHUNK) cn2 = DG_CHUNK; if (cn2 < 0) cn2 = 0;
                if (strm == 2) cn2 = 0;
                chunk_s[nx2] = cn2;
            }
            const bool presolve = deep && chunk_s[nxt] > 0;
            if (presolve) pre_cnt = chunk_s[nxt];
            unsigned *const gseedT = (unsigned *)(ws + A.wl.off_models + 2 * DG_MTAB_BYTES + DG_PRE_BYTES) + (size_t)gpar * DG_CHUNK;
            const unsigned *const gseedP = (const unsigned *)(ws + A.wl.off_models + 2 * DG_MTAB_BYTES + DG_PRE_BYTES) + (size_t)(gpar ^ 1) * DG_CHUNK;
            if (strm == 2) {  }
            else if (wave == 0) {
                const int ps = deep ? nx2 : nxt;
                if (deep && pend_draws) {
                    while (__builtin_amdgcn_readfirstlane(__hip_atomic_load(&S->itmp[23], __ATOMIC_RELAXED,
                        __HIP_MEMORY_SCOPE_WORKGROUP)) < 2) __builtin_amdgcn_s_sleep(1);
                    __builtin_amdgcn_fence(__ATOMIC_ACQUIRE, "workgroup");
                }
                if (chunk_s[ps] > 0) dg_sample_pool<7, LDSPTS>(chunk_s[ps], n, pool, S->draws3[ps], S->alm3[ps], pscr, lane, S->dbg);
            } else if (presolve && wave >= 2 && wave < 2 + DG_CHUNK / 64) {
                const int k_ = (wave - 2) * 64 + lane;
                if (k_ < chunk_s[nxt]) {
                    unsigned rx = 0;
                    double *tab = (double *)(ws + A.wl.off_models + (size_t)(mtab ^ 1) * DG_MTAB_BYTES);
                    const int r_ = dg_solve7_lane(P, S->draws3[nxt][k_], tab + (size_t)k_ * 27, &rx, (double *)((char *)&S->lsq + (size_t)(wave - 2) * 1024));
                    int *pre = (int *)(ws + A.wl.off_models + 2 * DG_MTAB_BYTES) + 2 * k_;
                    pre[0] = r_ < 0 ? 0x100 : r_; pre[1] = (int)rx;
                }
            } else if (deep && pend_draws && wave >= 6 && wave < 8) {
                const int cnp = chunk_s[nx2];
                for (int rd = 2 * (wave - 6); rd < 2 * (wave - 6) + 2 && rd < DG_CHUNK / 64; rd++) {
                    dg_sample_draws_round<7>(rd, cnp, n, gseedP, S->draws3[nx2], S->alm3[nx2], lane, S->dbg);
                    const int i_ = rd * 64 + lane; if (i_ < cnp) S->seeds3[nx2][i_] = gseedP[i_];
                }
                __builtin_amdgcn_fence(__ATOMIC_RELEASE, "workgroup");
                if (lane == 0) __hip_atomic_fetch_add(&S->itmp[23], 1, __ATOMIC_RELAXED, __HIP_MEMORY_SCOPE_WORKGROUP);
            } else if (wave == 1) {
                if (cn3 > 0) { unsigned sd = dg_sample_chain<7>(seed, cn3, gseedT, lane, S->dbg); if (lane == 0) S->itmp[31] = (int)sd; }
                else if (cn2 > 0) { unsigned sd = dg_sample_chain<7>(seed, cn2, S->seeds3[nx2], lane, S->dbg); if (lane == 0) S->itmp[31] = (int)sd; }
            }
            {
                const int NS = DG_NW >= 4 ? DG_NW - 2 : DG_NW, wsi = DG_NW >= 4 ? wave - 2 : wave;
                const int capw = (int)((sizeof(dg_lsq_scratch) / NS) & ~(size_t)15);
                int Ms = Mtot;
                if (fuse && wsi >= 0) {
                    constexpr int NB = DG_CHUNK / 64;
                    int nv_ = 0, nb_ = 0; unsigned rx = 0, incl = 0; const int k_ = wsi * 64 + lane;
                    if (wsi < NB) {
                        if (k_ < chunk) {
                            const int r_ = dg_solve7_lane(P, c.draws[k_], c.K->gmodels + (size_t)k_ * 27, &rx,
                                (double *)((char *)&S->lsq + (size_t)wsi * capw));
                            if (r_ < 0) nb_ = 1; else nv_ = r_;
                        }
                        incl = (unsigned)nv_;
#pragma unroll
                        for (int o = 1; o < 64; o <<= 1) { unsigned t = __shfl_up(incl, o, 64); if (lane >= o) incl += t; }
                        if (lane == 63) S->wave_cnt[wsi] = incl;
                        __builtin_amdgcn_fence(__ATOMIC_RELEASE, "workgroup");
                        if (lane == 0) __hip_atomic_fetch_add(&S->itmp[21], 1, __ATOMIC_RELAXED, __HIP_MEMORY_SCOPE_WORKGROUP);
                    }
                    while (__builtin_amdgcn_readfirstlane(__hip_atomic_load(&S->itmp[21], __ATOMIC_RELAXED,
                        __HIP_MEMORY_SCOPE_WORKGROUP)) < NB) __builtin_amdgcn_s_sleep(1);
                    __builtin_amdgcn_fence(__ATOMIC_ACQUIRE, "workgroup");
                    unsigned tot = 0, wbase = 0;
#pragma unroll
                    for (int b = 0; b < NB; b++) { const unsigned t = S->wave_cnt[b]; if (b < wsi) wbase += t; tot += t; }
                    if (wsi < NB) {
                        const unsigned excl = wbase + incl - (unsigned)nv_;
                        if (k_ < chunk) {
                            S->moff[k_] = (unsigned short)excl;
                            S->nv[k_] = nb_ ? 255 : (unsigned char)nv_;
                            S->nsolv[k_] = (unsigned char)((rx >> 8) & 3u);
                            for (int r = 0; r < nv_; r++) {
                                S->ridx[k_][r] = (unsigned char)((rx >> (2*r)) & 3u);
                                S->mslot[excl + r] = (unsigned short)(k_ * 3 + r);
                            }
                        }
                        if (wsi == 0 && lane == 0) S->moff[DG_CHUNK] = (unsigned short)tot;
                        __builtin_amdgcn_fence(__ATOMIC_RELEASE, "workgroup");
                        if (lane == 0) __hip_atomic_fetch_add(&S->itmp[22], 1, __ATOMIC_RELAXED, __HIP_MEMORY_SCOPE_WORKGROUP);
                    }
                    while (__builtin_amdgcn_readfirstlane(__hip_atomic_load(&S->itmp[22], __ATOMIC_RELAXED,
                        __HIP_MEMORY_SCOPE_WORKGROUP)) < NB) __builtin_amdgcn_s_sleep(1);
                    __builtin_amdgcn_fence(__ATOMIC_ACQUIRE, "workgroup");
                    Ms = (int)__builtin_amdgcn_readfirstlane(tot);
                }
                if (!(LDSPTS == 0 && coopK > 0) && wsi >= 0 && !ff)
                    dg_score_chunk_F<LDSPTS>(P, n, c.K->gmodels, S->mslot, Ms, wsi, NS, mk_full, th,
                                             tau_c, S->ext, (char *)&S->lsq + (size_t)wsi * capw, capw,
                                             (double *)(c.K->wstage + (size_t)wave * c.K->n_max), c.K->res_I, c.K->res_J, lane, S->scnt);
            }
        }
        c.n_fds += Mtot;
        if (LDSPTS == 0 && coopK > 0 && coop_units > 0) {
            const dg_coop_ws cv = dg_coop_views(A, slot);
            double *jb0 = (double *)(ws + A.wl.off_hjbuf);
            int units = coop_units;
            for (int st = coop_screen ? 1 : 2; st <= 2; st++) {
                dg_coop_work<T>(A, slot, S, cv, cb, coop_gen, jb0, &S->itmp[28], tid);
                if (__builtin_amdgcn_readfirstlane(tid >> 6) == 0) {
                    dg_wait_count(A, &cb->done, units, 4, 2);
                    if (st == 2) __builtin_amdgcn_fence(__ATOMIC_ACQUIRE, "agent");
                }
                __syncthreads();
                if (st == 2) break;
                unsigned ns = 0;
                for (int base = 0; base < Mtot; base += DG_T) {
                    const int mi = base + tid; const bool have = mi < Mtot;
                    const bool keep = have && ((double)__hip_atomic_load(cv.cnt + (have ? mi : 0), __ATOMIC_RELAXED, __HIP_MEMORY_SCOPE_AGENT) > tau_c);
                    if (have && !keep) { c.K->res_I[mi] = 0; c.K->res_J[mi] = 0; }
                    const unsigned long long bk = __ballot(keep);
                    if (lane == 0) S->wave_cnt[wave] = (unsigned)__popcll(bk);
                    __syncthreads();
                    unsigned off = ns;
                    for (int w = 0; w < DG_NW; w++) { if (w < wave) off += S->wave_cnt[w]; ns += S->wave_cnt[w]; }
                    if (keep) cv.surv[off + (unsigned)__popcll(bk & ((1ull << lane) - 1ull))] = (unsigned short)mi;
                    __syncthreads();
                }
                units = (int)ns;
                if (units == 0) { coop_no_ev = 1; break; }
                dg_coop_publish(cb, coop_gen, 2, units, Mtot, n, mk_full, 0, 0, th, S->ext, tau_c);
            }
        }
        __syncthreads();
        if (tid == 0) S->itmp[23] = 0;
        if (fuse) { Mtot = __builtin_amdgcn_readfirstlane((int)S->moff[DG_CHUNK]); c.n_fds += Mtot; }
        if (cn2 > 0 || cn3 > 0) seed = (unsigned)S->itmp[31];
        if (cn2 > 0 && wave < DG_CHUNK / 64) {
            for (int rd = wave; rd < DG_CHUNK / 64; rd += DG_NW) dg_sample_draws_round<7>(rd, cn2, n, S->seeds3[nx2], S->draws3[nx2], S->alm3[nx2], lane,
                S->dbg);
        }
        DG_PH(2);
        if (producer) {
            if (!ff) {
                __syncthreads();
                if (tid == 0) S->itmp[24] = 0;
                __syncthreads();
                for (int i = tid; i < DG_CHUNK; i += DG_T) {
                    ent->seeds[i] = S->seeds3[cur][i];
#pragma unroll
                    for (int q = 0; q < 8; q++) ent->draws[i][q] = S->draws3[cur][i][q];
                }
                if (tid < DG_CHUNK) {
                    const unsigned char nvb = tid < chunk ? S->nv[tid] : (unsigned char)0;
                    ent->nv[tid] = nvb;
                    if (tid < chunk && nvb != 255)
                        for (int r = 0; r < (int)nvb; r++) {
                            const int mi = (int)S->moff[tid] + r;
                            const double J_ = c.K->res_J[mi];
                            if (J_ > tau_c) {
                                const int sl = atomicAdd(&S->itmp[24], 1);
                                if (sl < DG_STREAM_EV_MAX) {
                                    dg_stream_ev *ev = &ent->ev[sl];
                                    ev->J = J_; ev->I = c.K->res_I[mi]; ev->k = (short)tid; ev->r = (unsigned char)r; ev->pad = 0;
#pragma unroll
                                    for (int j = 0; j < 9; j++) ev->model[j] = c.K->gmodels[(size_t)S->mslot[mi] * 9 + j];
#pragma unroll
                                    for (int q = 0; q < 4; q++) ev->ridx[q] = S->ridx[tid][q];
                                }
                            }
                        }
                }
                __syncthreads();
                if (tid == 0) {
                    const int ne = S->itmp[24];
                    ent->cn = chunk; ent->Mtot = Mtot; ent->n_ev = ne < DG_STREAM_EV_MAX ? ne : DG_STREAM_EV_MAX; ent->overflow = ne > DG_STREAM_EV_MAX ? 1 : 0;
                        ent->tau_used = tau_c;
                }
            }
            if ((seq & 7) == 7 || seq - tail_p < 16 || no_sam + chunk >= max_sam) dg_stream_publish(&scb->head, seq + 1);
            no_sam += chunk;
            __syncthreads();
            cur = nxt;
            continue;
        }
      }
        int k;
        for (k = 0; k < chunk; k++) {
            if (no_sam >= max_sam) break;
            if (no_sam >= DG_ITER_SAM) {
                track = 0;
                int stop = chunk;
                if (!coop_no_ev) {
                    const double tau = maxS.J < maxSs.J ? maxS.J : maxSs.J;
                    bool ev = false;
                    if (tid >= k && tid < chunk && S->nv[tid] != 255)
                        for (int r = 0; r < S->nv[tid]; r++) ev = ev || (tau < c.K->res_J[S->moff[tid] + r]);
                    unsigned long long bal = __ballot(ev);
                    __syncthreads();
                    if (lane == 0) S->wave_cnt[wave] = bal ? (unsigned)(wave * 64 + __ffsll((long long)bal) - 1) : 0xffffffffu;
                    __syncthreads();
                    unsigned kE = S->wave_cnt[0];
                    for (int w = 1; w < DG_NW; w++) kE = S->wave_cnt[w] < kE ? S->wave_cnt[w] : kE;
                    stop = kE == 0xffffffffu ? chunk : (int)kE;
                }
                int skip = stop - k; if (skip > max_sam - no_sam) skip = max_sam - no_sam;
                no_sam += skip; k += skip;
                if (k >= chunk || no_sam >= max_sam) break;
            }
            no_sam++;
            const int nvk = S->nv[k];
            if (nvk == 255) continue;
            int new_max = 0, do_iterate = 0, rng_ready = 0, brk = 0;
            for (int r = 0; r < nvk && !brk; r++) {
                const int mi = S->moff[k] + r, ri = S->ridx[k][r];
                dg_score Sc = {c.K->res_I[mi], c.K->res_J[mi], 0, 0};
                const int phys = perm[ri];
                const bool ev1 = maxS.J < Sc.J, ev2 = maxSs.J < Sc.J;
                if (!(ev1 || ev2)) {
                    if (track && phys == p4) { __syncthreads(); if (tid < 9) e4F[tid] = c.K->gmodels[(size_t)S->mslot[mi]*9 + tid]; e4kind = mk_full;
                        __syncthreads(); }
                    continue;
                }
                __syncthreads();
                if (tid < 9) S->f[tid] = c.K->gmodels[(size_t)S->mslot[mi]*9 + tid];
                __syncthreads();
                if (track && phys == p4) { if (tid < 9) e4F[tid] = S->f[tid]; e4kind = mk_full; __syncthreads(); }
                if (ev1) {
                    int pass = 1;
                    if (doSym || doLaf) {
                        dg_pass_cfg cl = dg_cfg0(n); cl.list = c.K->L[0]; cl.thL = th;
                        dg_pass_res rl = dg_f_pass(c, S->f, mk_full, cl);
                        pass = dg_f_checks(c, S->f, c.K->L[0], (int)rl.nL, Sc, maxS, mk_full);
                    }
                    if (!pass) continue;
                    { int t = perm[ri]; perm[ri] = perm[3]; perm[3] = t; }
                    maxS = Sc;
                    __syncthreads();
                    if (tid < 9) S->F[tid] = S->f[tid];
                    __syncthreads();
                    new_max = 1; accepted = 1; finKind = mk_full; best_sample = no_sam; t_best = wall_clock64();
                }
                if (maxSs.J < Sc.J) {
                    maxSs = Sc;
                    DG_TRACE(c, 30, Sc.I, Sc.J);
                    int degenerate = 0;
                    if (pr.degen) {
                        __syncthreads();
                        if (tid < 7) {
                            dg_pt q = dg_ldpt<LDSPTS>(P, c.draws[k][6 - tid]);
                            S->u7[tid][0] = q.x1; S->u7[tid][1] = q.y1; S->u7[tid][2] = q.x2; S->u7[tid][3] = q.y2;
                        }
                        __syncthreads();
                        { int dgn = dg_checksample(c, S->f, S->u7, 3*th, S->H); if (tid == 0) S->itmp[1] = dgn; }
                        __syncthreads();
                        degenerate = S->itmp[1];
                    }
                    if (degenerate) {
                        DG_PH(3);
                        if (!rng_ready) {
                            __syncthreads();
                            if (__builtin_amdgcn_readfirstlane(wave) == 0) { dg_srand_wave(&S->rng, c.seeds[k], lane); dg_rand_skip(&S->rng, 8, lane); }
                            __syncthreads();
                            rng_ready = 1;
                        }
                        dg_pass_cfg ch = dg_cfg0(n); ch.flags = c.K->Fl[1]; ch.thF = th*3;
                        dg_pass_res rh = dg_h_pass(c, S->H, ch); c.n_hds++;
                        unsigned I = rh.nF;
                        DG_TRACE(c, 31, I, no_sam);
                        if (I < 8) { DG_FLAST(S->f); brk = 1; c.n_fds -= (nvk - 1 - r); if (A.hist_out) { __syncthreads();
                            if (tid == 0) S->nv[k] = (unsigned char)(r + 1); __syncthreads(); } break; }
                        { long long ti0 = DG_CLK(); I = dg_innerH(c, S->H, 16*th, 10, c.K->Fl[0]); DG_DEVT(if (tid == 0) S->dbg[0] += DG_CLK() - ti0);
                            (void)ti0; }
                        DG_TRACE(c, 32, I, 0);
                        if ((int)I > Ihmax) Ihmax = (int)I;
                        if (I > 6) {
                            I = dg_rFtH(c, c.K->Fl[0], th, S->H, S->f);
                            DG_TRACE(c, 33, I, maxS.I);
                            if (ri == (int)S->nsolv[k] - 1) DG_FLAST(S->f);
                            int dphys;
                            if (I > maxS.I) {
                                maxS.I = I;
                                __syncthreads();
                                if (tid < 9) S->F[tid] = S->f[tid];
                                __syncthreads();
                                new_max = 1; accepted = 1; finKind = mk_full; best_sample = no_sam; t_best = wall_clock64();
                                dphys = perm[3];
                            } else dphys = perm[ri];
                            dg_pass_cfg cj = dg_cfg0(n); cj.wantJ = 1; cj.thJ = th;
                            dg_pass_res rj = dg_f_pass(c, S->f, mk_full, cj); c.n_fds++;
                            if (new_max) maxS.J = rj.J;
                            if (track && dphys == p4) { __syncthreads(); if (tid < 9) e4F[tid] = S->f[tid]; e4kind = mk_full; __syncthreads(); }
                            ++degen_cnt;
                            {
                                const double tau_new = maxS.J < maxSs.J ? maxS.J : maxSs.J;
                                if (tau_new < tau_scored && !A.hist_out && th != 0) {
                                    __syncthreads();
                                    if (strm == 2 && !full) {
                                        if (tid >= k && tid < chunk) {
                                            unsigned rixp = 0;
                                            const int r_ = dg_solve7_lane(P, c.draws[tid], c.K->gmodels + (size_t)tid * 27, &rixp, (double *)&S->ww[wave]);
                                            const int nvv = r_ < 0 ? 0 : r_;
                                            S->nsolv[tid] = (unsigned char)((rixp >> 8) & 3u);
                                            for (int q = 0; q < nvv; q++) S->ridx[tid][q] = (unsigned char)((rixp >> (2*q)) & 3u);
                                        }
                                        __syncthreads();
                                    }
                                    if (LDSPTS == 0 && coopK > 0 && tid == 0)
                                        __hip_atomic_store(&cb->tau_bits, (unsigned long long)__double_as_longlong(tau_new < 0 ? 0.0 : tau_new),
                                            __ATOMIC_RELAXED, __HIP_MEMORY_SCOPE_AGENT);
                                    {
                                        const int capr = (int)((sizeof(dg_lsq_scratch) / DG_NW) & ~(size_t)15);
                                        dg_score_chunk_F<LDSPTS>(P, n, c.K->gmodels, S->mslot, Mtot, wave, DG_NW, mk_full, th, tau_new, S->ext,
                                                                 (char *)&S->lsq + (size_t)wave * capr, capr,
                                                                 (double *)(c.K->wstage + (size_t)wave * c.K->n_max), c.K->res_I, c.K->res_J, lane,
                                                                     (unsigned *)0,
                                                                 (int)S->moff[k] + r + 1);
                                    }
                                    __syncthreads();
                                    tau_scored = tau_new;
                                }
                            }
                        }
                        DG_PH(5);
                    } else {
                        do_iterate = (no_sam > DG_ITER_SAM);
                        p4 = phys;
                        track = 1;
                        __syncthreads();
                        if (tid < 9) { e4F[tid] = S->f[tid]; S->FBest[tid] = S->f[tid]; }
                        if (tid < 7) S->samidxBest[tid] = c.draws[k][6 - tid];
                        e4kind = mk_full;
                        __syncthreads();
                        non_degen++;
                    }
                }
            }
            if (no_sam == DG_ITER_SAM && non_degen) do_iterate = 1;
            if (scb && strm >= 1 && tid == 0) {
                const double tau_ = maxS.J < maxSs.J ? maxS.J : maxSs.J;
                __hip_atomic_store(&scb->tau_bits, (unsigned long long)__double_as_longlong(tau_ < 0 ? 0.0 : tau_), __ATOMIC_RELAXED, __HIP_MEMORY_SCOPE_AGENT);
                __hip_atomic_store(&scb->max_sam, max_sam, __ATOMIC_RELAXED, __HIP_MEMORY_SCOPE_AGENT);
            }

            if (do_iterate) {
                if (!rng_ready) {
                    __syncthreads();
                    if (__builtin_amdgcn_readfirstlane(wave) == 0) { dg_srand_wave(&S->rng, c.seeds[k], lane); dg_rand_skip(&S->rng, 8, lane); }
                    __syncthreads();
                    rng_ready = 1;
                }
                iter_cnt++; track = 0;
                DG_PH(3);
                dg_resid_begin(c, iter_cnt - 1); __syncthreads();
                dg_dump_resid(c, 0, e4F, e4kind);
                dg_pass_cfg ca = dg_cfg0(n); ca.list = c.K->L[0]; ca.thL = DG_TC * th * DG_MWM;
                dg_pass_res ra = dg_f_pass(c, e4F, e4kind, ca);
                DG_TRACE(c, 1, ra.nL, no_sam);
                dg_u2f_list(c, c.K->L[0], (int)ra.nL, 0, 0, S->f);
                dg_pass_cfg cb = dg_cfg0(n); cb.wantJ = 1; cb.thJ = th; cb.list = c.K->L[0]; cb.thL = th;
                dg_pass_res rb = dg_f_pass(c, S->f, mk_full, cb); c.n_fds++;
                dg_dump_resid(c, 1, S->f, mk_full);
                DG_TRACE(c, 2, rb.nL, rb.J);
                int kb;
                DG_FLAST(S->f);
                dg_score Sl = dg_inFrani(c, (int)rb.nL, th, S->Hx , &iterID, mk_full, mk_ex, &kb);
                if (Sl.J > 0) DG_FLAST(S->Hx);
                if (maxS.J < Sl.J) {
                    if (dg_f_checks(c, S->Hx, c.K->L[0], (int)Sl.I, Sl, maxS, mk_full)) {
                        maxS = Sl;
                        __syncthreads();
                        if (tid < 9) S->F[tid] = S->Hx[tid];
                        __syncthreads();
                        new_max = 1; accepted = 1; finKind = kb; best_sample = no_sam; t_best = wall_clock64();
                    }
                }
                if (new_max && !pr.legacy) {
                    int new_sam = dg_nsamples((int)maxS.I + 1, n, 7, pr.conf);
                    if (new_sam < max_sam) max_sam = new_sam;
                }
                if (scb && strm >= 1 && tid == 0) {
                    const double tau_ = maxS.J < maxSs.J ? maxS.J : maxSs.J;
                    __hip_atomic_store(&scb->tau_bits, (unsigned long long)__double_as_longlong(tau_ < 0 ? 0.0 : tau_), __ATOMIC_RELAXED,
                        __HIP_MEMORY_SCOPE_AGENT);
                    __hip_atomic_store(&scb->max_sam, max_sam, __ATOMIC_RELAXED, __HIP_MEMORY_SCOPE_AGENT);
                }
                DG_PH(4);
            }
            if (new_max && pr.legacy) {
                int new_sam = dg_nsamples((int)maxS.I + 1, n, 7, pr.conf);
                if (new_sam < max_sam) max_sam = new_sam;
            }
        }
        if (A.hist_out) {
            int *hist = A.hist_out + (size_t)off + 3 * (size_t)pair;
            const int reached = no_sam - chunk_base;
            if (tid < reached && tid < chunk && S->nv[tid] != 255) {
                unsigned best = 0;
                for (int r = 0; r < S->nv[tid]; r++) { const unsigned I_ = c.K->res_I[S->moff[tid] + r]; best = I_ > best ? I_ : best; }
                atomicAdd(&hist[2 + best], 1);
            }
        }
        if (k < chunk) { c.n_fds -= (Mtot - (int)S->moff[k]); done = 1; }
        else if (no_sam >= max_sam) done = 1;
        __syncthreads();
        if (legacy_sym && !done) {
            const bool cand = tid < chunk && S->nv[tid] != 255;
            const unsigned long long bal = __ballot(cand);
            if (lane == 0) S->wave_cnt[wave] = bal ? (unsigned)(wave * 64 + 63 - __clzll((long long)bal)) : 0xffffffffu;
            __syncthreads();
            int kf = -1;
            for (int w = 0; w < DG_NW; w++) if (S->wave_cnt[w] != 0xffffffffu) kf = (int)S->wave_cnt[w];
            __syncthreads();
            if (kf >= 0) { if (tid < 7) S->lastIds[tid] = c.draws[kf][tid]; D.has_last = 1; }
            __syncthreads();
        }
        if (!done) {
            if (deep) { chunk_s[cur] = cn3; pend_draws = cn3 > 0; gpar ^= 1; }
            cur = nxt;
            presolved = pre_cnt;
            if (pre_cnt > 0) { mtab ^= 1; if (tid == 0) S->K.gmodels = (double *)(ws + A.wl.off_models + (size_t)mtab * DG_MTAB_BYTES); }
        }
    }
    if (producer) {
        dg_stream_publish(&scb->head, no_sam / DG_CHUNK + (no_sam % DG_CHUNK ? 1 : 0));
        __syncthreads();
        if (tid == 0) __hip_atomic_store(&scb->state, DG_ST_RELEASED, __ATOMIC_RELAXED, __HIP_MEMORY_SCOPE_AGENT);
        return -1;
    }

    if (!iter_cnt && !degen_cnt && non_degen) {
        int degenerate = 0;
        __syncthreads();
        {
            int dgn = 0;
            if (pr.degen) {
                if (tid < 7) { dg_pt q = dg_ldpt<LDSPTS>(P, S->samidxBest[tid]); S->u7[tid][0] = q.x1; S->u7[tid][1] = q.y1; S->u7[tid][2] = q.x2;
                    S->u7[tid][3] = q.y2; }
                __syncthreads();
                dgn = dg_checksample(c, S->FBest, S->u7, 3*th, S->H);
            }
            if (tid == 0) S->itmp[1] = dgn;
        }
        __syncthreads();
        degenerate = S->itmp[1];
        __syncthreads();
        if (__builtin_amdgcn_readfirstlane(wave) == 0) {
            int li = no_sam - 1 - chunk_base; if (li < 0) li = 0;
            dg_srand_wave(&S->rng, c.seeds[li], lane); dg_rand_skip(&S->rng, 8, lane);
        }
        __syncthreads();
        if (degenerate) {
            dg_pass_cfg ch = dg_cfg0(n); ch.flags = c.K->Fl[1]; ch.thF = th*3;
            dg_pass_res rh = dg_h_pass(c, S->H, ch); c.n_hds++;
            unsigned I = rh.nF;
            if (I >= 8) I = dg_innerH(c, S->H, 16*th, 10, c.K->Fl[0]);
            else { for (int j = tid; j < n; j += DG_T) c.K->Fl[0][j] = 0; __syncthreads(); }
            if ((int)I > Ihmax) Ihmax = (int)I;
            if (I > 6) {
                __syncthreads();
                if (tid < 9) S->f[tid] = S->FBest[tid];
                __syncthreads();
                I = dg_rFtH(c, c.K->Fl[0], th, S->H, S->f);
                DG_FLAST(S->f);
                int nm = 0;
                if (I > maxS.I) {
                    maxS.I = I;
                    __syncthreads();
                    if (tid < 9) S->F[tid] = S->f[tid];
                    __syncthreads();
                    nm = 1; accepted = 1; finKind = mk_full; best_sample = no_sam; t_best = wall_clock64();
                }
                dg_pass_cfg cj = dg_cfg0(n); cj.wantJ = 1; cj.thJ = th;
                dg_pass_res rj = dg_f_pass(c, S->f, mk_full, cj); c.n_fds++;
                if (nm) maxS.J = rj.J;
                ++degen_cnt;
            }
        } else {
            iter_cnt++;
            dg_resid_begin(c, iter_cnt - 1); __syncthreads();
            dg_pass_cfg ca = dg_cfg0(n); ca.list = c.K->L[0]; ca.thL = DG_TC * th * DG_MWM;
            dg_pass_res ra = dg_f_pass(c, S->FBest, mk_full, ca);
            dg_u2f_list(c, c.K->L[0], (int)ra.nL, 0, 0, S->f);
            dg_pass_cfg cb = dg_cfg0(n); cb.list = c.K->L[0]; cb.thL = th;
            dg_pass_res rb = dg_f_pass(c, S->f, mk_full, cb); c.n_fds++;
            dg_dump_resid(c, 1, S->f, mk_full);
            int kb;
            DG_FLAST(S->f);
            dg_score Sl = dg_inFrani(c, (int)rb.nL, th, S->Hx, &iterID, mk_full, mk_ex, &kb);
            if (Sl.J > 0) DG_FLAST(S->Hx);
            if (maxS.J < Sl.J) {
                if (dg_f_checks(c, S->Hx, c.K->L[0], (int)Sl.I, Sl, maxS, mk_full)) {
                    maxS = Sl;
                    __syncthreads();
                    if (tid < 9) S->F[tid] = S->Hx[tid];
                    __syncthreads();
                    accepted = 1; finKind = kb; best_sample = no_sam; t_best = wall_clock64();
                }
            }
        }
    }

    DG_PH(3);
    unsigned char *mask = A.mask_out + off;
    if (!accepted) {
        for (int j = tid; j < n; j += DG_T) mask[j] = 0;
    } else {
        double F[9];
        for (int i = 0; i < 9; i++) F[i] = S->F[i];
        for (int j = tid; j < n; j += DG_T) mask[j] = dg_Ferr(finKind, F, dg_ldpt<LDSPTS>(P, j)) <= th ? 1 : 0;
        __syncthreads();
        if (legacy_sym) {
            const int li = no_sam - 1 - chunk_base;
            const bool cand = tid <= li && tid < DG_CHUNK && S->nv[tid] != 255;
            const unsigned long long bal = __ballot(cand);
            if (lane == 0) S->wave_cnt[wave] = bal ? (unsigned)(wave * 64 + 63 - __clzll((long long)bal)) : 0xffffffffu;
            __syncthreads();
            int kf = -1;
            for (int w = 0; w < DG_NW; w++) if (S->wave_cnt[w] != 0xffffffffu) kf = (int)S->wave_cnt[w];
            __syncthreads();
            int have = 0;
            if (kf >= 0 && D.flast_k == chunk_base + kf + 1) have = 1;
            else if (kf >= 0 || D.has_last) {
                if (tid == 0) { int ids[7]; for (int i = 0; i < 7; i++) ids[i] = kf >= 0 ? c.draws[kf][i] : S->lastIds[i];
                                S->itmp[2] = dg_solve7_lastroot(P, ids, S->flast, (double *)&S->ww[0]); }
                __syncthreads();
                have = S->itmp[2];
            }
            __syncthreads();
            if (have) {
                double Fl[9]; for (int i = 0; i < 9; i++) Fl[i] = S->flast[i];
                for (int j = tid; j < n; j += DG_T) if (dg_Ferr(DG_K_FSYM, Fl, dg_ldpt<LDSPTS>(P, j)) > pr.sym_th) mask[j] = 0;
            }
        } else if (doSym || (doLaf && pr.final_laf_filter)) {
            dg_pass_cfg cl = dg_cfg0(n); cl.list = c.K->L[0]; cl.thL = th;
            dg_pass_res rl = dg_f_pass(c, S->F, finKind, cl);
            const int cnt = (int)rl.nL; const int *lst = c.K->L[0];
            if (doSym)
                for (int j = tid; j < cnt; j += DG_T) if (dg_Ferr(DG_K_FSYM, F, dg_ldpt<LDSPTS>(P, lst[j])) > pr.sym_th) mask[j] = 0;
            if (doLaf && pr.final_laf_filter) {
                double thl = pr.laf_coef * th;
                for (int j = tid; j < cnt; j += DG_T) {
                    if (dg_Ferr(mk_full, F, c.laf_pt(lst[j], 1)) > thl) mask[j] = 0;
                    if (dg_Ferr(mk_full, F, c.laf_pt(lst[j], 2)) > thl) mask[j] = 0;
                }
            }
        }
    }
    if (tid < 9) A.model_out[(size_t)pair * 9 + tid] = accepted ? S->F[tid] : 0.0;
    if (A.hist_out && tid == 0) { int *hist = A.hist_out + (size_t)off + 3 * (size_t)pair; hist[0] = no_sam; hist[1] = iter_cnt; }
    if (A.screen_out && tid == 0) { int *so = A.screen_out + (size_t)pair * 4; for (int i = 0; i < 4; i++) so[i] = (int)S->scnt[i]; }
    if (A.stats_out && tid == 0) {
        int *st = A.stats_out + (size_t)pair * 16;
        long long t_end = wall_clock64();
        st[0] = no_sam; st[1] = iter_cnt; st[2] = S->n_lafrej; st[3] = (int)maxS.I; st[4] = c.n_fds + c.n_exfds;
        st[5] = degen_cnt; st[6] = Ihmax; st[7] = best_sample; st[8] = c.n_fds; st[9] = c.n_exfds;
        st[10] = c.n_hds; st[11] = c.n_aux; st[12] = (int)(t_best - t_start); st[13] = (int)(t_end - t_start);
        st[14] = A.variant_threads; st[15] = A.mode | (resume ? 256 : 0) | (strm == 2 ? 512 : 0);
    }
    if (fan) {
        if (tid == 0) __hip_atomic_store(&scb->stop, 1, __ATOMIC_RELAXED, __HIP_MEMORY_SCOPE_AGENT);
    } else if (scb && strm >= 1) {
        __syncthreads();
        int gone = 0;
        if (tid == 0) {
            int e = DG_ST_REQ;
                gone = __hip_atomic_compare_exchange_strong(&scb->state, &e, DG_ST_IDLE, __ATOMIC_RELAXED, __ATOMIC_RELAXED, __HIP_MEMORY_SCOPE_AGENT) ? 1 : 0;
                S->itmp[30] = gone;
            if (gone) __hip_atomic_fetch_add(A.done_pairs + 1, -1, __ATOMIC_RELAXED, __HIP_MEMORY_SCOPE_AGENT);
        }
        __syncthreads();
        gone = S->itmp[30];
        __syncthreads();
        if (!gone) {
            if (tid == 0) __hip_atomic_store(&scb->stop, 1, __ATOMIC_RELAXED, __HIP_MEMORY_SCOPE_AGENT);
            dg_stream_wait(A, &scb->state, (int *)0, [](int st_) { return st_ == DG_ST_RELEASED; }, &S->itmp[28]);
            if (tid == 0) {
                __hip_atomic_store(&scb->head, 0, __ATOMIC_RELAXED, __HIP_MEMORY_SCOPE_AGENT);
                __hip_atomic_store(&scb->stop, 0, __ATOMIC_RELAXED, __HIP_MEMORY_SCOPE_AGENT);
                __hip_atomic_store(&scb->state, DG_ST_IDLE, __ATOMIC_RELAXED, __HIP_MEMORY_SCOPE_AGENT);
            }
        }
    }
    if (A.done_pairs && tid == 0) __hip_atomic_fetch_add(A.done_pairs, 1, __ATOMIC_RELAXED, __HIP_MEMORY_SCOPE_AGENT);
    DG_PH(6);
#ifdef DG_LO_PROF
    if (A.phase_out && tid == 0) { for (int i = 0; i < 16; i++) A.phase_out[(size_t)pair * 16 + i] = S->lt[i]; }
    if (0)
#endif
    DG_DEVT(if (A.phase_out && tid == 0) { S->ph[7] = DG_CLK() - t_start; for (int i = 0; i < 8; i++) A.phase_out[(size_t)pair * 16 + i] = S->ph[i];
        for (int i = 0; i < 8; i++) A.phase_out[(size_t)pair * 16 + 8 + i] = S->dbg[i]; A.phase_out[(size_t)pair * 16 + 15] = DG_CLK(); });
#undef DG_PH
    return -1;
}

__device__ __forceinline__ int dg_next_pair(const dg_args &A, int *bc )
{
    __syncthreads();
    if (threadIdx.x == 0) *bc = atomicAdd(A.ticket, 1);
    __syncthreads();
    const int t = *bc;
    if (t >= A.n_pairs) return -1;
    return A.order ? A.order[t] : t;
}

__device__ __noinline__ void dg_discard_if_failed(const dg_args &A, const int pair, int *bc )
{
    __syncthreads();
    if (threadIdx.x == 0) *bc = __hip_atomic_load(A.err_flag, __ATOMIC_RELAXED, __HIP_MEMORY_SCOPE_AGENT);
    __syncthreads();
    const int failed = *bc;
    __syncthreads();
    if (!failed) return;
    const long long off = A.offsets[pair];
    const int n = (int)(A.offsets[pair + 1] - off);
    for (int j = (int)threadIdx.x; j < n; j += (int)blockDim.x) A.mask_out[(size_t)off + j] = 0;
    if (threadIdx.x < 9) A.model_out[(size_t)pair * 9 + threadIdx.x] = 0.0;
    if (A.stats_out && threadIdx.x == 0) { A.stats_out[(size_t)pair * 16 + 3] = 0; A.stats_out[(size_t)pair * 16 + 15] |= 1024; }
}

template <int T, int LDSPTS>
__global__ __launch_bounds__(DG_T, DG_MINW) void dg_find_fundamental_kernel(dg_args A)
{
    extern __shared__ __attribute__((aligned(16))) unsigned char dyn_smem[];
    __shared__ __attribute__((aligned(16))) dg_f_shared Sh;
    __shared__ int next_pair;
    __shared__ long long next_parked;
    __shared__ dg_args As;
    if (threadIdx.x == 0) As = A;
    __syncthreads();
    if (LDSPTS == 0 && As.fan_k > 0) {
        const int base = As.n_res * (As.coop_k + 1);
        if ((int)blockIdx.x >= base) {
            const int w = (int)blockIdx.x - base;
            if (w % As.fan_k == 0) dg_f_fan_sampler<T>(As, &Sh, w / As.fan_k, As.fan_ws0 + w, &next_pair);
            else dg_f_fan_worker<T>(As, &Sh, w / As.fan_k, As.fan_ws0 + w, &next_pair);
            return;
        }
    }
    int slot = (int)blockIdx.x, coop_gen = 0;
    DG_DEVT(if (As.phase_out && threadIdx.x == 0) { long long *o_ = As.phase_out + ((size_t)As.n_pairs + blockIdx.x) * 16; o_[10] = DG_CLK(); o_[11] = 0; });
    if (LDSPTS == 0 && As.coop_k > 0) {
        slot = (int)blockIdx.x / (As.coop_k + 1);
        const int h = (int)blockIdx.x % (As.coop_k + 1);
        if (h != 0) { dg_f_helper<T>(As, &Sh, slot, h, &next_pair); return; }
    }
    int wsid = slot;
    for (;;) {
        int resume = 0;
        int pair = dg_next_pair(As, &next_pair);
        if (pair < 0 && As.park_sam > 0) {
            long long e = dg_park_take(As, &next_parked, 1);
            if (e < 0) e = dg_park_take(As, &next_parked, 0);
            if (e < 0) e = dg_park_take(As, &next_parked, 1);
            if (e >= 0) { pair = (int)(e >> 32); wsid = (int)(e & 0xffffffffll); resume = 1; }
        }
        int img_wsid = wsid, oslot = slot;
        if (pair < 0 && As.stream_on) {
            const int j = dg_stream_find(As, &next_pair);
            if (j >= 0) { pair = As.scb[j].pair; img_wsid = As.scb[j].wsid; oslot = j; resume = 2; }
        }
        if (pair < 0) break;
        const int spare = dg_f_pair<T, LDSPTS>(As, &Sh, dyn_smem, pair, slot, img_wsid, resume, coop_gen, wsid, oslot);
        if (spare >= 0) wsid = spare;
        else if (resume != 2) dg_discard_if_failed(As, pair, &next_pair);
    }
    if (LDSPTS == 0 && As.coop_k > 0 && threadIdx.x == 0)
        __hip_atomic_store(&As.coop[slot].gen, -1, __ATOMIC_RELAXED, __HIP_MEMORY_SCOPE_AGENT);
    DG_DEVT(if (As.phase_out && threadIdx.x == 0) As.phase_out[((size_t)As.n_pairs + blockIdx.x) * 16] = DG_CLK());
    DG_DEVT(if (As.phase_out && (threadIdx.x & 63) == 0) As.phase_out[((size_t)As.n_pairs + blockIdx.x) * 16 + 1 + (threadIdx.x >> 6)] =
                (long long)__builtin_amdgcn_s_getreg((31 << 11) | 4) | ((long long)__builtin_amdgcn_s_getreg((31 << 11) | 20) << 32));

}

#endif
```

pydegensac_amd/csrc/dg_variant.h:

```cpp
#ifndef DG_VARIANT_H
#define DG_VARIANT_H
#include <hip/hip_runtime.h>
#include "dg_kernel_common.h"

enum { DG_MODE_HBM = 0, DG_MODE_LDS = 1, DG_MODE_POOL_LDS = 2 };

#define DG_VARIANT_DECL(T_) \
    hipError_t dg_variant_##T_##_init(const unsigned C[8][32], const unsigned Ct[32][8], const unsigned G[32], const unsigned T[31][32], int max_lds, \
        int static_lds[2]); \
    hipError_t dg_variant_##T_##_resident(int homography, int mode, size_t dyn, int *blocks_per_cu); \
    hipError_t dg_variant_##T_##_launch(int homography, int mode, int grid, size_t dyn, hipStream_t stream, const dg_args &A);
DG_VARIANT_DECL(512)
DG_VARIANT_DECL(256)
DG_VARIANT_DECL(128)
#endif
```

pydegensac_amd/csrc/dg_variant_impl.h:

```cpp
#define DG_VCAT2(a, b, c) a##b##c
#define DG_VCAT(a, b, c) DG_VCAT2(a, b, c)
#include "dg_variant.h"

hipError_t DG_VCAT(dg_variant_, DG_T, _init)(const unsigned C[8][32], const unsigned Ct[32][8], const unsigned G[32], const unsigned T[31][32], int max_lds,
    int static_lds[2])
{
    hipError_t e;
    if ((e = hipMemcpyToSymbol(HIP_SYMBOL(dg_rng_T), T, sizeof(unsigned) * 31 * 32)) != hipSuccess) return e;
    if ((e = hipMemcpyToSymbol(HIP_SYMBOL(dg_rng_C), C, sizeof(unsigned) * 8 * 32)) != hipSuccess) return e;
    if ((e = hipMemcpyToSymbol(HIP_SYMBOL(dg_rng_Ct), Ct, sizeof(unsigned) * 32 * 8)) != hipSuccess) return e;
    if ((e = hipMemcpyToSymbol(HIP_SYMBOL(dg_rng_G), G, sizeof(unsigned) * 32)) != hipSuccess) return e;
    hipFuncAttributes fa;
    const void *kf[3] = {(const void *)dg_find_fundamental_kernel<DG_T, DG_MODE_LDS>, (const void *)dg_find_fundamental_kernel<DG_T, DG_MODE_POOL_LDS>,
                         (const void *)dg_find_fundamental_kernel<DG_T, DG_MODE_HBM>};
    const void *kh[3] = {(const void *)dg_find_homography_kernel<DG_T, DG_MODE_LDS>, (const void *)dg_find_homography_kernel<DG_T, DG_MODE_POOL_LDS>,
                         (const void *)dg_find_homography_kernel<DG_T, DG_MODE_HBM>};
    for (int h = 0; h < 2; h++) {
        const void **k = h ? kh : kf;
        static_lds[h] = (int)sizeof(dg_f_shared);
        for (int m = 0; m < 3; m++) {
            if ((e = hipFuncGetAttributes(&fa, k[m])) != hipSuccess) return e;
            if ((int)fa.sharedSizeBytes > static_lds[h]) static_lds[h] = (int)fa.sharedSizeBytes;
        }
        for (int m = 0; m < 2; m++)
            if ((e = hipFuncSetAttribute(k[m], hipFuncAttributeMaxDynamicSharedMemorySize, max_lds - static_lds[h] - 256)) != hipSuccess) return e;
    }
    return hipSuccess;
}

static const void *DG_VCAT(dg_variant_, DG_T, _fn)(int homography, int mode)
{
    if (!homography) {
        if (mode == DG_MODE_LDS)      return (const void *)dg_find_fundamental_kernel<DG_T, DG_MODE_LDS>;
        if (mode == DG_MODE_POOL_LDS) return (const void *)dg_find_fundamental_kernel<DG_T, DG_MODE_POOL_LDS>;
        return (const void *)dg_find_fundamental_kernel<DG_T, DG_MODE_HBM>;
    }
    if (mode == DG_MODE_LDS)      return (const void *)dg_find_homography_kernel<DG_T, DG_MODE_LDS>;
    if (mode == DG_MODE_POOL_LDS) return (const void *)dg_find_homography_kernel<DG_T, DG_MODE_POOL_LDS>;
    return (const void *)dg_find_homography_kernel<DG_T, DG_MODE_HBM>;
}

hipError_t DG_VCAT(dg_variant_, DG_T, _resident)(int homography, int mode, size_t dyn, int *blocks_per_cu)
{
    return hipOccupancyMaxActiveBlocksPerMultiprocessor(blocks_per_cu, DG_VCAT(dg_variant_, DG_T, _fn)(homography, mode), DG_T, dyn);
}

hipError_t DG_VCAT(dg_variant_, DG_T, _launch)(int homography, int mode, int grid, size_t dyn, hipStream_t stream, const dg_args &A)
{
    const dim3 g(grid), b(DG_T);
    if (!homography) {
        if (mode == DG_MODE_LDS)           hipLaunchKernelGGL((dg_find_fundamental_kernel<DG_T, DG_MODE_LDS>), g, b, dyn, stream, A);
        else if (mode == DG_MODE_POOL_LDS) hipLaunchKernelGGL((dg_find_fundamental_kernel<DG_T, DG_MODE_POOL_LDS>), g, b, dyn, stream, A);
        else                               hipLaunchKernelGGL((dg_find_fundamental_kernel<DG_T, DG_MODE_HBM>), g, b, 0, stream, A);
    } else {
        if (mode == DG_MODE_LDS)           hipLaunchKernelGGL((dg_find_homography_kernel<DG_T, DG_MODE_LDS>), g, b, dyn, stream, A);
        else if (mode == DG_MODE_POOL_LDS) hipLaunchKernelGGL((dg_find_homography_kernel<DG_T, DG_MODE_POOL_LDS>), g, b, dyn, stream, A);
        else                               hipLaunchKernelGGL((dg_find_homography_kernel<DG_T, DG_MODE_HBM>), g, b, 0, stream, A);
    }
    return hipGetLastError();
}
```

pydegensac_amd/csrc/mi_degensac_host.inc:

```
#include <math.h>
#include "mi_match_batch.h"

static thread_local char g_err[512] = "";
static void set_err(const char *fmt, const char *a = "", const char *b = "") { snprintf(g_err, sizeof g_err, fmt, a, b); }
#define HIPCHK(x) do { hipError_t e_ = (x); if (e_ != hipSuccess) { set_err("%s failed: %s", #x, hipGetErrorString(e_)); (void)hipGetLastError(); \
    return MI_DEGENSAC_EHIP; } } while (0)

extern "C" const char *mi_degensac_last_error(void) { return g_err; }
extern "C" const char *mi_degensac_version(void) { return "mi_degensac 0.2 (gfx950)"; }
extern "C" const char *mi_degensac_kernel_name(int homography) { return homography ? "dg_find_homography_kernel" : "dg_find_fundamental_kernel"; }
extern "C" int mi_degensac_device_count(void) { int n = 0; if (hipGetDeviceCount(&n) != hipSuccess) { (void)hipGetLastError(); return 0; } return n; }

struct DevGuard {
    int prev = -1; bool armed = false;
    int enter(int device)
    {
        if (hipGetDevice(&prev) != hipSuccess) { (void)hipGetLastError(); prev = -1; }
        if (prev != device) { HIPCHK(hipSetDevice(device)); armed = prev >= 0; }
        return 0;
    }
    ~DevGuard() { if (armed) (void)hipSetDevice(prev); }
};

struct DevState { bool init = false; int max_lds = 0, cus = 0, pool_par_ok = 0;
                  int static_lds[3][2] = {{0, 0}, {0, 0}, {0, 0}};    };
static const int g_variant_threads[3] = {512, 256, 128};
typedef hipError_t (*dg_resident_fn)(int, int, size_t, int *);
typedef hipError_t (*dg_launch_fn)(int, int, int, size_t, hipStream_t, const dg_args &);
static const dg_resident_fn g_variant_resident[3] = {dg_variant_512_resident, dg_variant_256_resident, dg_variant_128_resident};
static const dg_launch_fn   g_variant_launch[3]   = {dg_variant_512_launch, dg_variant_256_launch, dg_variant_128_launch};
static DevState g_dev[64];
static std::mutex g_mu;
static std::mutex g_dev_mu[64];
static uint32_t g_env_tuning = 0;

static void rng_state_table(unsigned T[31][32])
{
    for (int j = 0; j < 31; j++) {
        unsigned r[31]; for (int i = 0; i < 31; i++) r[i] = (i == j);
        int f = 3, b = 0;
        for (int t = 0; t < 310; t++) { r[f] += r[b]; if (++f >= 31) f = 0; if (++b >= 31) b = 0; }
        for (int p = 0; p < 31; p++) T[j][p] = r[p];
        T[j][31] = 0;
    }
}
static void rng_tables(unsigned C[8][32], unsigned G[32])
{
    for (int j = 0; j < 31; j++) {
        unsigned r[31]; for (int i = 0; i < 31; i++) r[i] = (i == j);
        int f = 3, b = 0;
        for (int t = 0; t < 310 + 8; t++) {
            r[f] += r[b];
            if (t >= 310) C[t - 310][j] = r[f];
            if (++f >= 31) f = 0; if (++b >= 31) b = 0;
        }
    }
    for (int k = 0; k < 8; k++) C[k][31] = 0;
    unsigned long long g = 1;
    for (int j = 0; j < 32; j++) { G[j] = (unsigned)g; g = (g * 16807ull) % 2147483647ull; }
}

__global__ void dg_exchange_order_kernel(int reps, long long *out)
{
    __shared__ int tab[64];
    const int lane = threadIdx.x; long long bad = 0, tot = 0;
    for (int rep = 0; rep < reps; rep++) {
        for (int K = 1; K <= 64; K = (K < 8 ? K + 1 : K * 2)) {
            tab[lane] = 0;
            DG_WSYNC();
            const int addr = (lane * 7 + rep) % K;
            const int old = __hip_atomic_exchange(&tab[addr], lane + 1, __ATOMIC_RELAXED, __HIP_MEMORY_SCOPE_WORKGROUP);
            int expect = 0;
            for (int l2 = 0; l2 < lane; l2++) if ((l2 * 7 + rep) % K == addr) expect = l2 + 1;
            bad += (old != expect); tot++;
            DG_WSYNC();
        }
    }
    for (int o = 32; o >= 1; o >>= 1) { bad += __shfl_xor(bad, o, 64); tot += __shfl_xor(tot, o, 64); }
    if (lane == 0) { out[0] = bad; out[1] = tot; }
}

static int exchange_order_probe(int reps, long long out[2])
{
    long long *d = nullptr;
    HIPCHK(hipMalloc((void **)&d, 16));
    hipLaunchKernelGGL(dg_exchange_order_kernel, dim3(1), dim3(64), 0, 0, reps, d);
    hipError_t e = hipGetLastError();
    if (e == hipSuccess) e = hipMemcpy(out, d, 16, hipMemcpyDeviceToHost);
    (void)hipFree(d);
    HIPCHK(e);
    return 0;
}

static int dev_init(int device)
{
    if (device < 0 || device >= 64) { set_err("bad device index"); return MI_DEGENSAC_EINVAL; }
    int ndev = 0;
    if (hipGetDeviceCount(&ndev) != hipSuccess || ndev == 0) { (void)hipGetLastError(); set_err("no HIP device: this library has no CPU path");
        return MI_DEGENSAC_ENODEV; }
    if (device >= ndev) { set_err("device index out of range"); return MI_DEGENSAC_ENODEV; }
    std::lock_guard<std::mutex> lk(g_mu);
    DevState &d = g_dev[device];
    if (!d.init) {
        hipDeviceProp_t prop; HIPCHK(hipGetDeviceProperties(&prop, device));
        if (strncmp(prop.gcnArchName, "gfx950", 6) != 0) { set_err("device is %s, this build targets gfx950 only", prop.gcnArchName); return MI_DEGENSAC_ENODEV;
            }
        unsigned C[8][32], G[32], Ct[32][8]; rng_tables(C, G);
        static unsigned T[31][32]; rng_state_table(T);
        for (int j = 0; j < 32; j++) for (int k = 0; k < 8; k++) Ct[j][k] = C[k][j];
        d.max_lds = (int)prop.sharedMemPerBlock; d.cus = prop.multiProcessorCount;
        HIPCHK(dg_variant_512_init(C, Ct, G, T, d.max_lds, d.static_lds[0]));
// ... 93 lines not shown
            g_retired.push_back(r);
            s->p = nullptr; s->bytes = 0;
        }
        const size_t want = bytes + bytes / 8;
        if (hipMalloc((void **)&s->p, want) != hipSuccess) { (void)hipGetLastError(); s->p = nullptr; set_err("scratch allocation failed");
            return MI_DEGENSAC_ENOMEM; }
        s->bytes = want;
    }
    *out = s->p;
    return 0;
}

extern "C" int mi_degensac_release_scratch(int device, void *stream_or_null)
{
    DevGuard g; int rc = g.enter(device); if (rc) return rc;
    if (device < 0 || device >= 64) { set_err("bad device index"); return MI_DEGENSAC_EINVAL; }
    std::lock_guard<std::mutex> lk(g_dev_mu[device]);
    std::vector<Scratch> &g_scratch = g_scratch_dev[device];
    for (size_t i = 0; i < g_scratch.size();) {
        Scratch &e = g_scratch[i];
        if (e.device == device && (!stream_or_null || e.stream == (hipStream_t)stream_or_null)) {
            if (e.p) { (void)hipStreamSynchronize(e.stream); (void)hipFree(e.p); (void)hipGetLastError(); }
            g_scratch[i] = g_scratch.back(); g_scratch.pop_back();
        } else i++;
    }
    reap_retired_locked(device, true);
    return 0;
}

static int fill_params(const mi_degensac_params *p, int homography, int dim, dg_params *o)
{
    if (!p) { set_err("params is NULL"); return MI_DEGENSAC_EINVAL; }
    memset(o, 0, sizeof *o);
    const double coef = 3.0 * (p->symmetric_error_check ? 1 : 0);
    if (!homography) {
        if (p->error_type != 0 && p->error_type != 1) { set_err("error_type must be 0 or 1 for the fundamental matrix"); return MI_DEGENSAC_EINVAL; }
        o->th = p->px_th * p->px_th; o->sym_th = p->px_th * p->px_th * coef;
    } else {
        switch (p->error_type) {
        case 0: o->th = p->px_th * p->px_th; o->sym_th = p->px_th * coef; break;
        case 1: o->th = p->px_th * p->px_th; o->sym_th = 0; break;
        case 2: o->th = p->px_th;            o->sym_th = 0; break;
        case 3: o->th = p->px_th * p->px_th; o->sym_th = p->px_th * coef; break;
        case 4: o->th = p->px_th;            o->sym_th = p->px_th * coef; break;
        default: set_err("error_type must be 0..4 for the homography"); return MI_DEGENSAC_EINVAL;
        }
    }
    o->laf_coef = (p->laf_consistensy_coef > 0 && dim == 6) ? p->laf_consistensy_coef : 0.0;
    o->conf = p->conf; o->max_iters = p->max_iters; o->error_type = p->error_type;
    o->degen = p->enable_degeneracy_check ? 1 : 0;
    o->final_laf_filter = (p->flags & MI_DEGENSAC_FLAG_FINAL_LAF_FILTER) ? 1 : 0;
    if (p->flags & MI_DEGENSAC_FLAG_LEGACY_F) {
        if (homography) { set_err("MI_DEGENSAC_FLAG_LEGACY_F applies to the fundamental matrix only"); return MI_DEGENSAC_EINVAL; }
        if (o->laf_coef > 0) { set_err("MI_DEGENSAC_FLAG_LEGACY_F takes no LAF check"); return MI_DEGENSAC_EINVAL; }
        if (p->symmetric_error_check) o->sym_th = 16.0 * o->th;
        o->legacy = 1;
    }
    return 0;
}

#ifdef MI_DEGENSAC_DEV
static int *g_trace_dev = nullptr; static int g_trace_cap = 0;
static long long *g_phase_dev = nullptr;
#endif

static std::atomic<int> g_stream_mode{[] { const char *e = getenv("MI_DEGENSAC_STREAM"); return e ? atoi(e) : -1; }()};
extern "C" int mi_degensac_set_stream_mode(int mode) { return g_stream_mode.exchange(mode); }
static std::atomic<int> g_hjob_mode{[] { const char *e = getenv("MI_DEGENSAC_HJOB"); return e ? atoi(e) : 1; }()};
extern "C" int mi_degensac_set_hjob_mode(int mode) { return g_hjob_mode.exchange(mode); }
static const int g_stream_min_sam = [] { const char *e = getenv("MI_DEGENSAC_STREAM_MIN_SAM"); const int v = e ? atoi(e) : -1; return v >= 0 ? v : -1; }();
static std::atomic<int> g_stream_depth{[] { const char *e = getenv("MI_DEGENSAC_STREAM_DEPTH"); const int v = e ? atoi(e) : 0;
    return v >= 2 && v <= 1024 ? v : 0; }()};

static std::atomic<int> g_lo_width{-1};
static std::atomic<int> g_dev_knob{0};
static std::atomic<int> g_fan_k{-1};
static std::atomic<int> g_per_cu_cap{0};
#ifdef MI_DEGENSAC_DEV
extern "C" int mi_degensac_dev_set_per_cu(int v) { return g_per_cu_cap.exchange(v); }
extern "C" int mi_degensac_dev_set_fan(int k) { return g_fan_k.exchange(k); }
extern "C" int mi_degensac_dev_set_lo_width(int w) { return g_lo_width.exchange(w); }
extern "C" int mi_degensac_dev_set_knob(int v) { return g_dev_knob.exchange(v); }
#endif
static std::atomic<long long> g_wait_ticks{400000000ll};
extern "C" long long mi_degensac_set_wait_ticks(long long ticks) { return g_wait_ticks.exchange(ticks >= 0 ? ticks : 400000000ll); }

static int launch_batch_impl(int homography, const double *d_p1, const double *d_p2, const int64_t *d_off, const int64_t *h_off,
                             int n_pairs, int dim, const mi_degensac_params *prm, const uint32_t *d_seeds, int device,
                             hipStream_t stream, double *d_model, uint8_t *d_mask, int32_t *d_stats, const mi_degensac_diag *diag,
                             int *d_err_copy);

static int launch_batch(int homography, const double *d_p1, const double *d_p2, const int64_t *d_off, const int64_t *h_off,
                        int n_pairs, int dim, const mi_degensac_params *prm, const uint32_t *d_seeds, int device,
                        hipStream_t stream, double *d_model, uint8_t *d_mask, int32_t *d_stats, const mi_degensac_diag *diag = nullptr,
                        int *d_err_copy = nullptr )
{
    if (n_pairs <= 0) return 0;
    if (device < 0 || device >= 64) { set_err("bad device index"); return MI_DEGENSAC_EINVAL; }
    std::lock_guard<std::mutex> lk(g_dev_mu[device]);
    return launch_batch_impl(homography, d_p1, d_p2, d_off, h_off, n_pairs, dim, prm, d_seeds, device, stream, d_model, d_mask, d_stats, diag, d_err_copy);
}

static int launch_batch_impl(int homography, const double *d_p1, const double *d_p2, const int64_t *d_off, const int64_t *h_off,
                        int n_pairs, int dim, const mi_degensac_params *prm, const uint32_t *d_seeds, int device,
                             hipStream_t stream, double *d_model, uint8_t *d_mask, int32_t *d_stats, const mi_degensac_diag *diag,
                             int *d_err_copy)
{
    if (n_pairs <= 0) return 0;
    if (dim != 2 && dim != 6) { set_err("points must be [n,2] or [n,6]"); return MI_DEGENSAC_EINVAL; }
    if (!h_off) { set_err("offsets_host is NULL"); return MI_DEGENSAC_EINVAL; }
    int rc = dev_init(device); if (rc) return rc;
    dg_args A; memset(&A, 0, sizeof A);
    rc = fill_params(prm, homography, dim, &A.prm); if (rc) return rc;
    int n_max = 0, n_min = 1 << 30;
    for (int p = 0; p < n_pairs; p++) {
        long long n = h_off[p+1] - h_off[p];
        if (n > 0x7fffffff / 64) { set_err("too many correspondences in one pair"); return MI_DEGENSAC_EINVAL; }
        if (n > n_max) n_max = (int)n; if (n < n_min) n_min = (int)n;
    }
    const int min_pts = homography ? 4 : 8;
    if (n_min < min_pts) { set_err(homography ? "need n >= 4 correspondences" : "need n >= 8 correspondences"); return MI_DEGENSAC_EINVAL; }
    const DevState &ds = g_dev[device];
    uint32_t tune = prm->tuning;
    if (!tune && g_env_tuning) {
        tune = g_env_tuning;
        if (homography) tune &= ~(MI_DEGENSAC_TUNE_F_SERIAL_REPS | MI_DEGENSAC_TUNE_COOP_ALL_PASSES | (7u << 29));
        else            tune &= ~MI_DEGENSAC_TUNE_H_SERIAL_LO;
    }
    if (homography && (tune & MI_DEGENSAC_TUNE_F_SERIAL_REPS)) { set_err("MI_DEGENSAC_TUNE_F_SERIAL_REPS applies to the fundamental matrix only");
        return MI_DEGENSAC_EINVAL; }
    if (!homography && (tune & MI_DEGENSAC_TUNE_H_SERIAL_LO)) { set_err("MI_DEGENSAC_TUNE_H_SERIAL_LO applies to the homography only");
        return MI_DEGENSAC_EINVAL; }
    if (homography && (tune & MI_DEGENSAC_TUNE_COOP_ALL_PASSES)) { set_err("MI_DEGENSAC_TUNE_COOP_ALL_PASSES applies to the fundamental matrix only");
        return MI_DEGENSAC_EINVAL; }
    if (homography && (tune >> 29)) { set_err("MI_DEGENSAC_TUNE_LONG_SHIFT applies to the fundamental matrix only"); return MI_DEGENSAC_EINVAL; }
    const size_t dyn_all = (size_t)n_max * (sizeof(dg_pt) + sizeof(int)), dyn_pool = (size_t)n_max * sizeof(int);
    int variant = 0, mode;
    if (n_pairs > 2 * ds.cus && ds.static_lds[1][homography] + dyn_pool + 512 <= (size_t)ds.max_lds / 2) variant = 1;
    if (homography && n_pairs > 2 * ds.cus && ds.static_lds[2][1] + 512 <= (size_t)ds.max_lds / 4) variant = 2;
    else if (homography && n_pairs > ds.cus && ds.static_lds[1][1] + 512 <= (size_t)ds.max_lds / 2) variant = 1;
    if ((tune & 3u) == 1u) variant = 0; else if ((tune & 3u) == 2u) variant = 1; else if ((tune & 3u) == 3u) variant = 2;
    const size_t room = (size_t)(ds.max_lds - ds.static_lds[variant][homography] - 256);
    if (variant >= 1)           mode = dyn_pool <= room ? DG_MODE_POOL_LDS : DG_MODE_HBM;
    else if (dyn_all <= room)   mode = DG_MODE_LDS;
    else                        mode = dyn_pool <= room ? DG_MODE_POOL_LDS : DG_MODE_HBM;
    if (homography && variant >= 1 && mode == DG_MODE_POOL_LDS) {
        const long long fit_pool = (long long)((size_t)ds.max_lds / (ds.static_lds[variant][1] + dyn_pool + 256));
        long long fit_hbm = (long long)((size_t)ds.max_lds / (ds.static_lds[variant][1] + 256)); if (fit_hbm > 8) fit_hbm = 8;
        if (fit_pool * ds.cus < n_pairs && fit_hbm > fit_pool) mode = DG_MODE_HBM;
    }
    switch ((tune >> 2) & 3u) {
    case 1: mode = DG_MODE_HBM; break;
    case 2: if (dyn_all <= room) mode = DG_MODE_LDS; break;
    case 3: if (dyn_pool <= room) mode = DG_MODE_POOL_LDS; break;
    default: break;
    }
    const size_t dyn = mode == DG_MODE_LDS ? dyn_all : (mode == DG_MODE_POOL_LDS ? dyn_pool : 0);
    int per_cu = 0;
    hipError_t oe = g_variant_resident[variant](homography, mode, dyn, &per_cu);
    if (oe != hipSuccess || per_cu < 1) { (void)hipGetLastError(); per_cu = 1; }
    {
        const int by_lds = (int)((size_t)ds.max_lds / (ds.static_lds[variant][homography] + dyn + 256));
        if (by_lds >= 1 && per_cu > by_lds) per_cu = by_lds;
        if (per_cu > 8) per_cu = 8;
        static const int env_per_cu = [] { const char *e = getenv("MI_DEGENSAC_PER_CU"); const int v = e ? atoi(e) : 0; return v > 0 ? v : 0; }();
        const int cap_pc = g_per_cu_cap.load() > 0 ? g_per_cu_cap.load() : env_per_cu;
        if (cap_pc > 0 && per_cu > cap_pc) per_cu = cap_pc;
    }
    const long long capacity = (long long)per_cu * ds.cus;
    int coop_k = 0;
    if (!homography && mode == DG_MODE_HBM) {
        const unsigned th_ = (tune >> 8) & 255u;
        if (th_ == 0) { if (n_max >= 8192 && (long long)n_pairs * 24 <= capacity) coop_k = 23;
            else if (n_max >= 8192 && (long long)n_pairs * 16 <= capacity) coop_k = 15; }
        else if (th_ != 255u) coop_k = (int)th_;
        while (coop_k > 0 && (long long)(coop_k + 1) > capacity) coop_k--;
    }
    long long owners = coop_k > 0 ? capacity / (coop_k + 1) : capacity; if (owners > n_pairs) owners = n_pairs;
    {
        const unsigned gc = (tune >> 24) & 31u;
        if (gc > 0 && coop_k == 0 && owners > (long long)gc) owners = gc;
    }
    long long grid = owners * (coop_k + 1);
    int stream_mode = g_stream_mode.load();
    if (prm->flags & MI_DEGENSAC_FLAG_NO_STREAM) stream_mode = 0;
    else if (prm->flags & MI_DEGENSAC_FLAG_STREAM_ON) stream_mode = 1 | (int)(((prm->flags >> 8) & 3u) << 1);
    else if (prm->flags & MI_DEGENSAC_FLAG_STREAM_AUTO) stream_mode = -1;
    const int hjob_mode = (prm->flags & MI_DEGENSAC_FLAG_NO_HJOB) ? 0 : (prm->flags & MI_DEGENSAC_FLAG_HJOB_ON) ? 1 : g_hjob_mode.load();
    bool stream_on = !homography && coop_k == 0 && mode != DG_MODE_HBM && !(diag && (diag->d_resids || diag->d_hist)) && stream_mode != 0 &&
                     prm->max_iters >= 8192 && ((tune >> 24) & 31u) == 0 && (stream_mode > 0 || (long long)n_pairs <= 2 * capacity);
    bool stream_early = false;
    if (stream_on && grid < capacity) { long long extra = capacity - grid; if (extra > n_pairs) extra = n_pairs; stream_early = extra >= n_pairs; grid += extra;
        owners = grid; }
    const bool hjob_on = homography && mode != DG_MODE_LDS && !(diag && diag->d_resids) && !(tune & MI_DEGENSAC_TUNE_H_SERIAL_LO) && hjob_mode != 0 &&
                         ((tune >> 24) & 31u) == 0;
    if (hjob_on && grid < capacity) { long long extra = capacity - grid; if (extra > 2 * (long long)n_pairs) extra = 2 * (long long)n_pairs; grid += extra;
        owners = grid; }
    int fan_k = 0;
    if (!homography && variant == 0 && coop_k > 0 && mode == DG_MODE_HBM && stream_mode != 0 && owners >= n_pairs && !(diag && (diag->d_resids || diag->d_hist))
        &&
        ((tune >> 24) & 31u) == 0 && !(prm->flags & MI_DEGENSAC_FLAG_LEGACY_F)) {
        static const int env_fan = [] { const char *e = getenv("MI_DEGENSAC_FAN"); return e ? atoi(e) : -1; }();
        long long k = (capacity - grid) / owners;
        const long long want = g_fan_k.load() >= 0 ? g_fan_k.load() : (env_fan >= 0 ? env_fan : 32);
        if (k > want) k = want;
        if (k >= 8) fan_k = (int)k;
    }
    if (fan_k > 0) grid += owners * fan_k;
    int park_sam = 0; long long spares = 0; size_t park_bytes = 0;
    if (stream_on) park_bytes = align_up((size_t)ds.static_lds[variant][0], 256) + align_up(dyn, 256);
    if (!homography && coop_k == 0 && !(diag && (diag->d_resids || diag->d_hist)) && (long long)n_pairs > owners) {
        const unsigned pt = (tune >> 16) & 255u;
        if (pt == 0) park_sam = 1024;
        else if (pt != 255u) park_sam = (int)pt * 256;
        if (park_sam > 0) {
            spares = (long long)n_pairs - owners;
            park_bytes = align_up((size_t)ds.static_lds[variant][0], 256) + align_up(dyn, 256);
        }
    }
    A.wl = make_layout(n_max, mode != DG_MODE_LDS, g_variant_threads[variant] / 64, coop_k, park_bytes, homography != 0);
    if (spares > 0) {
        size_t free_b = 0, total_b = 0;
        if (hipMemGetInfo(&free_b, &total_b) != hipSuccess) { (void)hipGetLastError(); free_b = (size_t)4 << 30; }
        size_t budget = (free_b + cached_scratch_locked(device, stream)) / 2;
        if (budget > ((size_t)24 << 30)) budget = (size_t)24 << 30;
        const long long room_ws = (long long)(budget / (A.wl.stride + A.wl.stride / 8)) - owners;
        if (spares > room_ws) spares = room_ws > 0 ? room_ws : 0;
    }
    const size_t hdr_coop = DG_HDR_BYTES + align_up((size_t)owners * sizeof(dg_coop_cb), 256);
    const size_t hdr_cb = hdr_coop + ((stream_on || hjob_on || fan_k > 0) ? align_up((size_t)owners * sizeof(dg_stream_cb), 256) : 0);
    const size_t ent_bytes = align_up(sizeof(dg_stream_ent), 256);
    int stream_depth = g_stream_depth.load();
    if (stream_depth <= 0) { stream_depth = prm->max_iters / 256 + 2; if (stream_depth > 512) stream_depth = 512; if (stream_depth < 8) stream_depth = 8; }
    if (stream_on || fan_k > 0) {
        size_t free_b = 0, total_b = 0;
        if (hipMemGetInfo(&free_b, &total_b) != hipSuccess) { (void)hipGetLastError(); free_b = (size_t)4 << 30; }
        size_t budget = (free_b + cached_scratch_locked(device, stream)) / 4; if (budget > ((size_t)8 << 30)) budget = (size_t)8 << 30;
        const size_t fit = budget / ((size_t)owners * ent_bytes);
        if (fit < (size_t)stream_depth) stream_depth = (int)fit;
        if (stream_depth < 8) { stream_on = false; if (fan_k > 0) { grid -= owners * fan_k; fan_k = 0; } }
    }
    const size_t fan_ws = fan_k > 0 ? (size_t)owners * fan_k : 0;
    size_t hdr, ring_bytes; char *ws;
    for (;;) {
        hdr = hdr_cb + align_up((size_t)2 * spares * sizeof(long long), 256);
        ring_bytes = (stream_on || fan_k > 0) ? (size_t)owners * stream_depth * (ent_bytes + (fan_k > 0 ? 128 : 0)) : 0;
        rc = get_scratch_locked(device, stream, hdr + A.wl.stride * (size_t)(owners + spares + fan_ws) + ring_bytes, &ws);
        if (rc != MI_DEGENSAC_ENOMEM || (spares == 0 && !stream_on)) break;
        if (spares > 0) spares /= 2;
        else stream_on = false;
    }
    if (rc) return rc;
    HIPCHK(hipMemsetAsync(ws, 0, (coop_k > 0 || stream_on || hjob_on) ? hdr_cb : DG_HDR_BYTES, stream));
    if (fan_k > 0) HIPCHK(hipMemsetAsync(ws + hdr + A.wl.stride * (size_t)(owners + spares + fan_ws) + (size_t)owners * stream_depth * ent_bytes, 0,
        (size_t)owners * stream_depth * 128, stream));
    if (spares > 0) HIPCHK(hipMemsetAsync(ws + hdr_cb, 0xff, (size_t)2 * spares * sizeof(long long), stream));
    A.ticket = (int *)ws; A.park_ctl = (int *)(ws + 128); A.park_q = (long long *)(ws + hdr_cb); A.park_cap = (int)spares;
    A.park_sam = spares > 0 ? park_sam : 0; A.n_res = (int)owners; A.n_ws = (int)(owners + spares); A.dyn_bytes = (int)dyn;
    {
        const unsigned lg = (tune >> 29) & 7u;
        A.park_long = park_sam << (lg ? lg : 3);
    }
    A.coop = (dg_coop_cb *)(ws + DG_HDR_BYTES);
    A.done_pairs = (int *)(ws + 768); A.err_flag = (int *)(ws + 896);
    A.stream_on = stream_on ? 1 : 0; A.scb = (dg_stream_cb *)(ws + hdr_coop); A.stream_depth = stream_depth; A.stream_ent_bytes = ent_bytes;
    A.ring = ws + hdr + A.wl.stride * (size_t)(owners + spares + fan_ws);
    A.fan_k = fan_k; A.fan_ws0 = (int)(owners + spares); A.fan_flags = fan_k > 0 ? (int *)(A.ring + (size_t)owners * stream_depth * ent_bytes) : nullptr;
    A.hjob = hjob_on ? (dg_hjob_cb *)(ws + hdr_coop) : nullptr;
    (void)stream_early;
    A.stream_early = stream_on ? 1 : 0;
    A.stream_min_sam = g_stream_min_sam >= 0 ? g_stream_min_sam : 0; A.stream_min_left = 4096;
    A.stream_test = stream_mode > 0 ? (stream_mode >> 1) : 0;
    { const long long wt = g_wait_ticks.load(); A.wait_ticks = wt > 2000000000ll ? 2000000000 : (int)wt; }
    A.coop_k = coop_k; A.ws = ws + hdr; A.order = nullptr;
    A.coop_pass_min = (coop_k > 0 && (tune & MI_DEGENSAC_TUNE_COOP_ALL_PASSES)) ? 0 : 8192;
    A.pts1 = d_p1; A.pts2 = d_p2; A.offsets = (const long long *)d_off; A.seeds = d_seeds;
    A.lo_serial = (homography && (tune & MI_DEGENSAC_TUNE_H_SERIAL_LO)) ? 1 : 0;
    A.innerh_serial = (!homography && (tune & MI_DEGENSAC_TUNE_F_SERIAL_REPS)) ? 1 : 0;
    A.dev_knob = g_dev_knob.load();
    A.lo_width = g_lo_width.load() >= 0 ? g_lo_width.load() : 0;
    A.pool_seq = (!ds.pool_par_ok || (tune & MI_DEGENSAC_TUNE_SEQ_POOL)) ? 1 : 0;
    A.variant_threads = g_variant_threads[variant]; A.mode = mode;
#ifdef MI_DEGENSAC_DEV
    A.trace = g_trace_dev; A.trace_cap = g_trace_cap; A.phase_out = g_phase_dev;
#endif
    if (diag && diag->d_resids && diag->resid_runs > 0) { A.resids_out = diag->d_resids; A.resid_runs = diag->resid_runs; }
    if (diag && diag->d_hist && !homography) A.hist_out = diag->d_hist;
    if (diag && (size_t)diag->struct_size >= offsetof(mi_degensac_diag, d_screen) + sizeof(int32_t *) && diag->d_screen &&
        !homography) A.screen_out = diag->d_screen;
    A.model_out = d_model; A.mask_out = d_mask; A.stats_out = d_stats; A.dim = dim; A.n_pairs = n_pairs; A.pts_in_lds = mode == DG_MODE_LDS;
    HIPCHK(g_variant_launch[variant](homography, mode, (int)grid, dyn, stream, A));
    if (d_err_copy) HIPCHK(hipMemcpyAsync(d_err_copy, A.err_flag, sizeof(int), hipMemcpyDeviceToDevice, stream));
    return 0;
}

static int batch_dev(int homography, const double *d_pts1, const double *d_pts2, const int64_t *d_offsets, const int64_t *offsets_host,
                     int n_pairs, int dim, const mi_degensac_params *prm, const uint32_t *d_seeds, int device, void *stream,
                     double *d_M, uint8_t *d_mask, int32_t *d_stats, const mi_degensac_diag *diag = nullptr)
{
    if (device < 0 || device >= 64) { set_err("bad device index"); return MI_DEGENSAC_EINVAL; }
    if (mi_degensac_device_count() == 0) { set_err("no HIP device: this library has no CPU path"); return MI_DEGENSAC_ENODEV; }
    DevGuard g; int rc = g.enter(device); if (rc) return rc;
    return launch_batch(homography, d_pts1, d_pts2, d_offsets, offsets_host, n_pairs, dim, prm, d_seeds, device, (hipStream_t)stream, d_M, d_mask, d_stats,
        diag);
}
extern "C" int mi_degensac_find_fundamental_batch_dev(const double *d_pts1, const double *d_pts2, const int64_t *d_offsets,
        const int64_t *offsets_host, int n_pairs, int dim, const mi_degensac_params *prm, const uint32_t *d_seeds, int device,
        void *stream, double *d_F, uint8_t *d_mask, int32_t *d_stats)
{ return batch_dev(0, d_pts1, d_pts2, d_offsets, offsets_host, n_pairs, dim, prm, d_seeds, device, stream, d_F, d_mask, d_stats); }
extern "C" int mi_degensac_find_homography_batch_dev(const double *d_pts1, const double *d_pts2, const int64_t *d_offsets,
        const int64_t *offsets_host, int n_pairs, int dim, const mi_degensac_params *prm, const uint32_t *d_seeds, int device,
        void *stream, double *d_H, uint8_t *d_mask, int32_t *d_stats)
{ return batch_dev(1, d_pts1, d_pts2, d_offsets, offsets_host, n_pairs, dim, prm, d_seeds, device, stream, d_H, d_mask, d_stats); }

extern "C" int mi_degensac_find_fundamental_batch_dev_ex(const double *d_pts1, const double *d_pts2, const int64_t *d_offsets,
        const int64_t *offsets_host, int n_pairs, int dim, const mi_degensac_params *prm, const uint32_t *d_seeds, int device,
        void *stream, double *d_F, uint8_t *d_mask, int32_t *d_stats, const mi_degensac_diag *diag)
{ return batch_dev(0, d_pts1, d_pts2, d_offsets, offsets_host, n_pairs, dim, prm, d_seeds, device, stream, d_F, d_mask, d_stats, diag); }
extern "C" int mi_degensac_find_homography_batch_dev_ex(const double *d_pts1, const double *d_pts2, const int64_t *d_offsets,
        const int64_t *offsets_host, int n_pairs, int dim, const mi_degensac_params *prm, const uint32_t *d_seeds, int device,
        void *stream, double *d_H, uint8_t *d_mask, int32_t *d_stats, const mi_degensac_diag *diag)
{ return batch_dev(1, d_pts1, d_pts2, d_offsets, offsets_host, n_pairs, dim, prm, d_seeds, device, stream, d_H, d_mask, d_stats, diag); }

struct mi_degensac_ctx {
    int device = 0; hipStream_t stream = nullptr;
    char *h_pin = nullptr; size_t h_cap = 0;
    char *d_io = nullptr;  size_t d_cap = 0;
    int stream_mode = -2, hjob_mode = -2;
};

static int ctx_reserve(mi_degensac_ctx *c, size_t bytes)
{
    if (c->h_cap < bytes) {
        if (c->h_pin) { HIPCHK(hipStreamSynchronize(c->stream)); (void)hipHostFree(c->h_pin); c->h_pin = nullptr; c->h_cap = 0; }
        const size_t want = bytes + bytes / 4 + 4096;
        if (hipHostMalloc((void **)&c->h_pin, want, hipHostMallocDefault) != hipSuccess) { (void)hipGetLastError(); set_err("pinned host allocation failed");
            return MI_DEGENSAC_ENOMEM; }
        c->h_cap = want;
    }
    if (c->d_cap < bytes) {
        if (c->d_io) { HIPCHK(hipStreamSynchronize(c->stream)); (void)hipFree(c->d_io); c->d_io = nullptr; c->d_cap = 0; }
        const size_t want = bytes + bytes / 4 + 4096;
        if (hipMalloc((void **)&c->d_io, want) != hipSuccess) { (void)hipGetLastError(); set_err("device allocation failed"); return MI_DEGENSAC_ENOMEM; }
        c->d_cap = want;
    }
    return 0;
}

extern "C" int mi_degensac_ctx_create(int device, mi_degensac_ctx **out)
{
    if (!out) { set_err("NULL argument"); return MI_DEGENSAC_EINVAL; }
    *out = nullptr;
    if (device < 0 || device >= 64) { set_err("bad device index"); return MI_DEGENSAC_EINVAL; }
    if (mi_degensac_device_count() == 0) { set_err("no HIP device: this library has no CPU path"); return MI_DEGENSAC_ENODEV; }
    if (device >= mi_degensac_device_count()) { set_err("device index out of range"); return MI_DEGENSAC_ENODEV; }
    DevGuard g; int rc = g.enter(device); if (rc) return rc;
    rc = dev_init(device); if (rc) return rc;
    mi_degensac_ctx *c = new (std::nothrow) mi_degensac_ctx; if (!c) { set_err("out of memory"); return MI_DEGENSAC_ENOMEM; }
    c->device = device;
    hipError_t e = hipStreamCreateWithFlags(&c->stream, hipStreamNonBlocking);
    if (e != hipSuccess) { delete c; set_err("hipStreamCreate failed: %s", hipGetErrorString(e)); (void)hipGetLastError(); return MI_DEGENSAC_EHIP; }
    *out = c;
    return 0;
}

extern "C" void mi_degensac_ctx_destroy(mi_degensac_ctx *c)
{
    if (!c) return;
    DevGuard g; if (g.enter(c->device)) { delete c; return; }
    (void)hipStreamSynchronize(c->stream);
    (void)mi_degensac_release_scratch(c->device, c->stream);
    if (c->h_pin) (void)hipHostFree(c->h_pin);
    if (c->d_io) (void)hipFree(c->d_io);
    (void)hipStreamDestroy(c->stream);
// ... 651 lines not shown
```

Measured before the change: 97.37 million.

## Add lean fundamental-matrix kernel variant without streaming, fan, coop and diagnostics paths

Instantiates a compile-time 'lean' feature variant of the fundamental-matrix kernel for the LDS and pool-LDS modes. It strips streaming, fan-out, cooperative, histogram, trace and legacy-symmetry code paths via if constexpr. The host selects this variant automatically when no diagnostics, legacy flag, streaming or coop features are requested. The aim is to lower register and code pressure and remove runtime branches in the hot loop. In exchange the code grows through more kernel instantiations, and inner LO routines always use the wave-parallel path.

```diff
diff --git a/include/mi_degensac.h b/include/mi_degensac.h
--- a/include/mi_degensac.h
+++ b/include/mi_degensac.h
@@ -256,6 +256,10 @@
 int mi_degensac_set_call_timing(int on);
 int mi_degensac_last_call_timing(double *out );
 
+int mi_degensac_set_kernel_features(int mode);
+int mi_degensac_kernel_features_for(int homography, uint32_t flags, uint32_t tuning, int have_resids, int have_hist, int have_screen,
+                                    int trace, int lo_width, int n_max, int n_pairs, int threads, int mode, int stream_on, int fan_k, int coop_k);
+
 int         mi_degensac_device_count(void);
 const char *mi_degensac_last_error(void);
 const char *mi_degensac_version(void);
diff --git a/pydegensac_amd/_lib.py b/pydegensac_amd/_lib.py
--- a/pydegensac_amd/_lib.py
+++ b/pydegensac_amd/_lib.py
@@ -212,6 +212,11 @@
             l.mi_degensac_set_call_timing.argtypes = [C.c_int]
             l.mi_degensac_last_call_timing.restype = C.c_int
             l.mi_degensac_last_call_timing.argtypes = [dp]
+        if hasattr(l, "mi_degensac_set_kernel_features"):
+            l.mi_degensac_set_kernel_features.restype = C.c_int
+            l.mi_degensac_set_kernel_features.argtypes = [C.c_int]
+            l.mi_degensac_kernel_features_for.restype = C.c_int
+            l.mi_degensac_kernel_features_for.argtypes = [C.c_int, C.c_uint32, C.c_uint32] + [C.c_int] * 12
         l.mi_degensac_last_error.restype = C.c_char_p
         l.mi_degensac_version.restype = C.c_char_p
         l.mi_degensac_kernel_name.restype = C.c_char_p
@@ -274,11 +279,23 @@
     return {k: float(v) for k, v in zip(TIMING_NAMES, out)}
 
 
+def set_kernel_features(mode):
+    return int(lib().mi_degensac_set_kernel_features(int(mode)))
+
+
+def kernel_features_for(homography=0, flags=0, tuning=0, have_resids=0, have_hist=0, have_screen=0, trace=0, lo_width=0, n_max=2000,
+                        n_pairs=4096, threads=256, mode=2, stream_on=0, fan_k=0, coop_k=0):
+    return int(lib().mi_degensac_kernel_features_for(int(homography), int(flags), int(tuning), int(have_resids), int(have_hist), int(have_screen),
+                                                     int(trace), int(lo_width), int(n_max), int(n_pairs), int(threads), int(mode), int(stream_on),
+                                                     int(fan_k), int(coop_k)))
+
+
 def stats_dict(st):
     d = {k: int(v) for k, v in zip(STAT_NAMES, st)}
     d["set_aside"] = (d["placement"] >> 8) & 1
     d["streamed"] = (d["placement"] >> 9) & 1
     d["discarded"] = (d["placement"] >> 10) & 1
     d["rerun"] = (d["placement"] >> 11) & 1
+    d["lean"] = (d["placement"] >> 12) & 1
     d["placement"] &= 255
     return d
diff --git a/pydegensac_amd/csrc/dg_f_lo.h b/pydegensac_amd/csrc/dg_f_lo.h
--- a/pydegensac_amd/csrc/dg_f_lo.h
+++ b/pydegensac_amd/csrc/dg_f_lo.h
@@ -463,9 +463,10 @@
     return maxS;
 }
 
-template <int LDSPTS>
+template <int LDSPTS, int FT = DG_FT_FULL>
 __device__ __forceinline__ dg_score dg_inFrani(CTX &c, int ninl, double th, double *Fout, int *iterID, int mk_full, int mk_ex, int *kindBest)
 {
+    if constexpr (FT == DG_FT_LEAN) return dg_inFrani_waves<LDSPTS, false>(c, ninl, th, Fout, iterID, mk_full, mk_ex, kindBest);
     if (c.rrun || c.A->innerh_serial || c.A->trace) return dg_inFrani_serial<LDSPTS>(c, ninl, th, Fout, iterID, mk_full, mk_ex, kindBest);
     if (c.cb) {
         if constexpr (LDSPTS == 0) return dg_inFrani_waves<LDSPTS, true>(c, ninl, th, Fout, iterID, mk_full, mk_ex, kindBest);
diff --git a/pydegensac_amd/csrc/dg_f_sched.h b/pydegensac_amd/csrc/dg_f_sched.h
--- a/pydegensac_amd/csrc/dg_f_sched.h
+++ b/pydegensac_amd/csrc/dg_f_sched.h
@@ -1,7 +1,7 @@
 #ifndef DG_F_SCHED_H
 #define DG_F_SCHED_H
 
-#define DG_FLAST(M) do { if (legacy_sym) { __syncthreads(); if (tid < 9) S->flast[tid] = (M)[tid]; D.flast_k = no_sam; __syncthreads(); } } while (0)
+#define DG_FLAST(M) do { if constexpr (!LEAN) if (legacy_sym) { __syncthreads(); if (tid < 9) S->flast[tid] = (M)[tid]; D.flast_k = no_sam; __syncthreads(); } } while (0)
 #define DG_PARK_SPARE   0
 #define DG_PARK_CLAIMED 32
 #define DG_PARK_HEAD    64
diff --git a/pydegensac_amd/csrc/dg_kernel_common.h b/pydegensac_amd/csrc/dg_kernel_common.h
--- a/pydegensac_amd/csrc/dg_kernel_common.h
+++ b/pydegensac_amd/csrc/dg_kernel_common.h
@@ -91,6 +91,7 @@
 struct dg_coop_rec { unsigned I, nL, nL2, nJ; };
 #define DG_COOP_MAX_SLICES 64
 
+enum { DG_FT_FULL = 0, DG_FT_LEAN = 1 };
 enum { DG_ST_IDLE = 0, DG_ST_REQ = 1, DG_ST_BUSY = 2, DG_ST_ATTACHED = 3, DG_ST_RELEASED = 4 };
 struct dg_stream_cb {
     int state;
diff --git a/pydegensac_amd/csrc/dg_kernel_f.h b/pydegensac_amd/csrc/dg_kernel_f.h
--- a/pydegensac_amd/csrc/dg_kernel_f.h
+++ b/pydegensac_amd/csrc/dg_kernel_f.h
@@ -182,6 +182,7 @@
 #define DG_TRACE(c, tag, I, J) do { if ((c).A->trace && (c).tid == 0) { int *t_ = (c).A->trace; int k_ = t_[0]; \
     if (k_ < (c).A->trace_cap) { long long jb_ = __double_as_longlong((double)(J)); t_[1+4*k_] = (tag); t_[2+4*k_] = (int)(I); \
     t_[3+4*k_] = (int)(jb_ & 0xffffffffll); t_[4+4*k_] = (int)(jb_ >> 32); t_[0] = k_ + 1; } } } while (0)
+#define DG_TRACE_IF(on, c, tag, I, J) do { if constexpr (on) DG_TRACE(c, tag, I, J); } while (0)
 
 template <int LDSPTS>
 __device__ __noinline__ dg_pass_res dg_coop_pass(CTX &c, const double *Fm , int kind, const dg_pass_cfg &cfg);
@@ -251,12 +252,12 @@
     }
 }
 
-template <int LDSPTS>
+template <int LDSPTS, int FT = DG_FT_FULL>
 __device__ __forceinline__ int dg_f_checks(CTX &c, const double *f, const int *list, int cnt, dg_score &S, const dg_score &maxS, int mkind)
 {
     const dg_params &pr = c.A->prm;
     if (pr.sym_th > 0) {
-        dg_pass_cfg cfg = pr.legacy ? dg_cfg0(c.n) : dg_cfg0(cnt); if (!pr.legacy) cfg.src = list; cfg.wantC = 1; cfg.thC = pr.sym_th;
+        dg_pass_cfg cfg = (FT != DG_FT_LEAN && pr.legacy) ? dg_cfg0(c.n) : dg_cfg0(cnt); if (!(FT != DG_FT_LEAN && pr.legacy)) cfg.src = list; cfg.wantC = 1; cfg.thC = pr.sym_th;
         dg_pass_res r = dg_f_pass(c, f, DG_K_FSYM, cfg);
         S.Is = r.C;
         if (S.Is < maxS.Is) return 0;
@@ -655,10 +656,12 @@
     }
 }
 
-template <int LDSPTS>
+template <int LDSPTS, int FT = DG_FT_FULL>
 __device__ __forceinline__ unsigned dg_innerH(CTX &c, double *H , double th, unsigned inlLimit, unsigned char *inl_flags)
 {
-    if (c.A->innerh_serial || inlLimit > 12) return dg_innerH_serial<LDSPTS>(c, H, th, inlLimit, inl_flags);
+    if constexpr (FT != DG_FT_LEAN) {
+        if (c.A->innerh_serial || inlLimit > 12) return dg_innerH_serial<LDSPTS>(c, H, th, inlLimit, inl_flags);
+    }
     return dg_innerH_waves<LDSPTS>(c, H, th, inlLimit, inl_flags);
 }
 
diff --git a/pydegensac_amd/csrc/dg_kernel_f_main.h b/pydegensac_amd/csrc/dg_kernel_f_main.h
--- a/pydegensac_amd/csrc/dg_kernel_f_main.h
+++ b/pydegensac_amd/csrc/dg_kernel_f_main.h
@@ -11,21 +11,24 @@
 #include "dg_f_fan.h"
 #include "dg_f_coop.h"
 
-template <int T, int LDSPTS>
+template <int T, int LDSPTS, int FT>
 __device__ __forceinline__ int dg_f_pair(const dg_args &A, dg_f_shared *S, unsigned char *dyn_smem, const int pair, const int slot, const int wsid,
                                          const int resume, int &coop_gen, const int own_wsid, const int oslot)
 {
-    const int producer = resume == 2;
-    dg_stream_cb *const scb = (A.stream_on || A.fan_k > 0) ? A.scb + oslot : (dg_stream_cb *)0;
+    constexpr bool LEAN = FT == DG_FT_LEAN;
+    static_assert(!LEAN || LDSPTS != 0, "the lean driver is instantiated with the sampler pool in LDS only");
+    const int producer = LEAN ? 0 : resume == 2;
+    dg_stream_cb *const scb = (!LEAN && (A.stream_on || A.fan_k > 0)) ? A.scb + oslot : (dg_stream_cb *)0;
     int head_seen = 0;
     int gpar = 0, pend_draws = 0;
     int mtab = 0, presolved = 0;
     int strm = 0, img_sam = 0;
-    const int coopK = LDSPTS == 0 ? A.coop_k : 0;
+    const int coopK = (LDSPTS == 0 && !LEAN) ? A.coop_k : 0;
     dg_coop_cb *const cb = coopK > 0 ? A.coop + slot : (dg_coop_cb *)0;
     const int tid = threadIdx.x, lane = tid & 63, wave = tid >> 6;
-    const bool fan = LDSPTS == 0 && A.fan_k > 0 && coopK > 0 && !resume && !(A.prm.legacy && A.prm.sym_th > 0);
-    const bool deep = DG_NW >= 8 && LDSPTS == 0 && coopK > 0 && !A.hist_out && !fan;
+#define DG_HIST (!LEAN && A.hist_out)
+    const bool fan = !LEAN && LDSPTS == 0 && A.fan_k > 0 && coopK > 0 && !resume && !(A.prm.legacy && A.prm.sym_th > 0);
+    const bool deep = DG_NW >= 8 && LDSPTS == 0 && coopK > 0 && !DG_HIST && !fan;
     const long long off = A.offsets[pair];
     const int n = (int)(A.offsets[pair + 1] - off);
     const dg_params &pr = A.prm;
@@ -52,7 +55,7 @@
     const int mk_full = pr.error_type == 1 ? DG_K_FSYM : DG_K_FDS;
     const int mk_ex   = pr.error_type == 1 ? DG_K_EXFSYM : DG_K_FDS;
     const int doSym = pr.sym_th > 0, doLaf = pr.laf_coef > 0;
-    const int legacy_sym = pr.legacy && doSym;
+    const int legacy_sym = !LEAN && pr.legacy && doSym;
 
     dg_f_drv D;
     dg_score &maxS = D.maxS, &maxSs = D.maxSs;
@@ -83,7 +86,7 @@
     }
     if (lane == 0) { S->extw[wave][0] = ex0; S->extw[wave][1] = ex1; S->extw[wave][2] = ex2; S->extw[wave][3] = ex3; }
     dg_ht_init(c.ht, tid);
-    if (A.hist_out) for (int j = tid; j < n + 3; j += DG_T) A.hist_out[(size_t)off + 3 * (size_t)pair + j] = 0;
+    if (DG_HIST) for (int j = tid; j < n + 3; j += DG_T) A.hist_out[(size_t)off + 3 * (size_t)pair + j] = 0;
     if (tid < 9) { S->F[tid] = 0; S->FBest[tid] = 0; }
     if (tid == 0) { S->n_lafrej = 0; S->scnt[0] = S->scnt[1] = S->scnt[2] = S->scnt[3] = 0; }
     __syncthreads();
@@ -114,7 +117,7 @@
     cur = 0; chunk_s[0] = chunk_s[1] = chunk_s[2] = 0; chunk_base = 0;
     if (tid == 0) S->itmp[23] = 0;
     {
-        const int first = (A.stream_on || coopK > 0) ? DG_CHUNK : (DG_CHUNK < 64 ? DG_CHUNK : 64);
+        const int first = ((!LEAN && A.stream_on) || coopK > 0) ? DG_CHUNK : (DG_CHUNK < 64 ? DG_CHUNK : 64);
         int cn0 = max_sam - no_sam; if (cn0 > first) cn0 = first; if (cn0 < 0) cn0 = 0;
         int cn1 = max_sam - no_sam - cn0; if (cn1 > DG_CHUNK) cn1 = DG_CHUNK; if (cn1 < 0) cn1 = 0;
         chunk_s[0] = cn0; chunk_s[1] = cn1;
@@ -132,7 +135,7 @@
         if (deep) { int cn2_ = max_sam - no_sam - cn0 - cn1; if (cn2_ > DG_CHUNK) cn2_ = DG_CHUNK; if (cn2_ < 0) cn2_ = 0; chunk_s[2] = cn2_; }
         __syncthreads();
         seed = (unsigned)S->itmp[31];
-        if (fan) {
+        if constexpr (LEAN) {} else if (fan) {
             if (tid == 0) {
                 scb->pair = pair; scb->wsid = wsid; scb->img_sam = 0; scb->fan_kind = mk_full; scb->fan_th = th;
                 for (int i = 0; i < 4; i++) scb->fan_ext[i] = S->ext[i];
@@ -175,7 +178,7 @@
         int ff = 0, tail_p = 0;
         int seq = no_sam / DG_CHUNK;
         dg_stream_ent *ent = (dg_stream_ent *)0;
-        if (producer) {
+        if constexpr (LEAN) {} else if (producer) {
             __syncthreads();
             if (tid == 0) {
                 S->itmp[24] = __hip_atomic_load(&scb->stop, __ATOMIC_RELAXED, __HIP_MEMORY_SCOPE_AGENT);
@@ -250,7 +253,7 @@
                 } else if (act == 2) strm = 2;
             }
         }
-        if (fan) {
+        if constexpr (LEAN) {} else if (fan) {
             DG_PH(3);
             {
                 const double tau_now = maxS.J < maxSs.J ? maxS.J : maxSs.J;
@@ -333,7 +336,7 @@
         int Mtot = 0, nxt = cur, cn2 = 0;
         double tau_scored = 0.0;
       int full = 1;
-      if (strm == 2) {
+      if constexpr (LEAN) {} else if (strm == 2) {
         if (!fan && seq >= head_seen) {
             const int h_ = dg_stream_wait(A, &scb->head, (int *)0, [=](int h) { return h > seq; }, &S->itmp[28], A.wait_ticks);
             if (h_ < 0) { done = 1; break; }
@@ -345,7 +348,7 @@
         if (tid == 0) { S->itmp[24] = e_->cn; S->itmp[25] = e_->Mtot; S->itmp[26] = e_->n_ev; S->itmp[27] = e_->overflow; S->dtmp[31] = e_->tau_used; }
         __syncthreads();
         const int cn_ = S->itmp[24], n_ev = S->itmp[26], ovf = S->itmp[27];
-        const double tau_used = S->dtmp[31], tau_now = A.hist_out ? 0.0 : (maxS.J < maxSs.J ? maxS.J : maxSs.J);
+        const double tau_used = S->dtmp[31], tau_now = DG_HIST ? 0.0 : (maxS.J < maxSs.J ? maxS.J : maxSs.J);
         if (n_ev == 0 && !ovf && !(tau_used > tau_now) && !(A.stream_test & 1) && no_sam >= DG_ITER_SAM && cn_ > 0 && no_sam + cn_ < max_sam) {
             const int Mt_ = S->itmp[25];
             __syncthreads();
@@ -435,8 +438,8 @@
             __syncthreads();
         }
         Mtot = (ff || fuse) ? 0 : __builtin_amdgcn_readfirstlane((int)S->moff[DG_CHUNK]);
-        double tau_c = A.hist_out ? 0.0 : (maxS.J < maxSs.J ? maxS.J : maxSs.J);
-        if (producer) {
+        double tau_c = DG_HIST ? 0.0 : (maxS.J < maxSs.J ? maxS.J : maxSs.J);
+        if constexpr (LEAN) {} else if (producer) {
             __syncthreads();
             if (tid == 0) S->dtmp[31] = __longlong_as_double((long long)__hip_atomic_load(&scb->tau_bits, __ATOMIC_RELAXED, __HIP_MEMORY_SCOPE_AGENT));
             __syncthreads();
@@ -593,7 +596,7 @@
                 S->dbg);
         }
         DG_PH(2);
-        if (producer) {
+        if constexpr (LEAN) {} else if (producer) {
             if (!ff) {
                 __syncthreads();
                 if (tid == 0) S->itmp[24] = 0;
@@ -683,7 +686,7 @@
                     if (doSym || doLaf) {
                         dg_pass_cfg cl = dg_cfg0(n); cl.list = c.K->L[0]; cl.thL = th;
                         dg_pass_res rl = dg_f_pass(c, S->f, mk_full, cl);
-                        pass = dg_f_checks(c, S->f, c.K->L[0], (int)rl.nL, Sc, maxS, mk_full);
+                        pass = dg_f_checks<LDSPTS, FT>(c, S->f, c.K->L[0], (int)rl.nL, Sc, maxS, mk_full);
                     }
                     if (!pass) continue;
                     { int t = perm[ri]; perm[ri] = perm[3]; perm[3] = t; }
@@ -695,7 +698,7 @@
                 }
                 if (maxSs.J < Sc.J) {
                     maxSs = Sc;
-                    DG_TRACE(c, 30, Sc.I, Sc.J);
+                    DG_TRACE_IF(!LEAN, c, 30, Sc.I, Sc.J);
                     int degenerate = 0;
                     if (pr.degen) {
                         __syncthreads();
@@ -719,16 +722,16 @@
                         dg_pass_cfg ch = dg_cfg0(n); ch.flags = c.K->Fl[1]; ch.thF = th*3;
                         dg_pass_res rh = dg_h_pass(c, S->H, ch); c.n_hds++;
                         unsigned I = rh.nF;
-                        DG_TRACE(c, 31, I, no_sam);
-                        if (I < 8) { DG_FLAST(S->f); brk = 1; c.n_fds -= (nvk - 1 - r); if (A.hist_out) { __syncthreads();
+                        DG_TRACE_IF(!LEAN, c, 31, I, no_sam);
+                        if (I < 8) { DG_FLAST(S->f); brk = 1; c.n_fds -= (nvk - 1 - r); if (DG_HIST) { __syncthreads();
                             if (tid == 0) S->nv[k] = (unsigned char)(r + 1); __syncthreads(); } break; }
-                        { long long ti0 = DG_CLK(); I = dg_innerH(c, S->H, 16*th, 10, c.K->Fl[0]); DG_DEVT(if (tid == 0) S->dbg[0] += DG_CLK() - ti0);
+                        { long long ti0 = DG_CLK(); I = dg_innerH<LDSPTS, FT>(c, S->H, 16*th, 10, c.K->Fl[0]); DG_DEVT(if (tid == 0) S->dbg[0] += DG_CLK() - ti0);
                             (void)ti0; }
-                        DG_TRACE(c, 32, I, 0);
+                        DG_TRACE_IF(!LEAN, c, 32, I, 0);
                         if ((int)I > Ihmax) Ihmax = (int)I;
                         if (I > 6) {
                             I = dg_rFtH(c, c.K->Fl[0], th, S->H, S->f);
-                            DG_TRACE(c, 33, I, maxS.I);
+                            DG_TRACE_IF(!LEAN, c, 33, I, maxS.I);
                             if (ri == (int)S->nsolv[k] - 1) DG_FLAST(S->f);
                             int dphys;
                             if (I > maxS.I) {
@@ -746,9 +749,9 @@
                             ++degen_cnt;
                             {
                                 const double tau_new = maxS.J < maxSs.J ? maxS.J : maxSs.J;
-                                if (tau_new < tau_scored && !A.hist_out && th != 0) {
+                                if (tau_new < tau_scored && !DG_HIST && th != 0) {
                                     __syncthreads();
-                                    if (strm == 2 && !full) {
+                                    if constexpr (LEAN) {} else if (strm == 2 && !full) {
                                         if (tid >= k && tid < chunk) {
                                             unsigned rixp = 0;
                                             const int r_ = dg_solve7_lane(P, c.draws[tid], c.K->gmodels + (size_t)tid * 27, &rixp, (double *)&S->ww[wave]);
@@ -789,7 +792,7 @@
                 }
             }
             if (no_sam == DG_ITER_SAM && non_degen) do_iterate = 1;
-            if (scb && strm >= 1 && tid == 0) {
+            if constexpr (LEAN) {} else if (scb && strm >= 1 && tid == 0) {
                 const double tau_ = maxS.J < maxSs.J ? maxS.J : maxSs.J;
                 __hip_atomic_store(&scb->tau_bits, (unsigned long long)__double_as_longlong(tau_ < 0 ? 0.0 : tau_), __ATOMIC_RELAXED, __HIP_MEMORY_SCOPE_AGENT);
                 __hip_atomic_store(&scb->max_sam, max_sam, __ATOMIC_RELAXED, __HIP_MEMORY_SCOPE_AGENT);
@@ -804,22 +807,22 @@
                 }
                 iter_cnt++; track = 0;
                 DG_PH(3);
-                dg_resid_begin(c, iter_cnt - 1); __syncthreads();
-                dg_dump_resid(c, 0, e4F, e4kind);
+                if constexpr (!LEAN) { dg_resid_begin(c, iter_cnt - 1); __syncthreads(); }
+                if constexpr (!LEAN) dg_dump_resid(c, 0, e4F, e4kind);
                 dg_pass_cfg ca = dg_cfg0(n); ca.list = c.K->L[0]; ca.thL = DG_TC * th * DG_MWM;
                 dg_pass_res ra = dg_f_pass(c, e4F, e4kind, ca);
-                DG_TRACE(c, 1, ra.nL, no_sam);
+                DG_TRACE_IF(!LEAN, c, 1, ra.nL, no_sam);
                 dg_u2f_list(c, c.K->L[0], (int)ra.nL, 0, 0, S->f);
                 dg_pass_cfg cb = dg_cfg0(n); cb.wantJ = 1; cb.thJ = th; cb.list = c.K->L[0]; cb.thL = th;
                 dg_pass_res rb = dg_f_pass(c, S->f, mk_full, cb); c.n_fds++;
-                dg_dump_resid(c, 1, S->f, mk_full);
-                DG_TRACE(c, 2, rb.nL, rb.J);
+                if constexpr (!LEAN) dg_dump_resid(c, 1, S->f, mk_full);
+                DG_TRACE_IF(!LEAN, c, 2, rb.nL, rb.J);
                 int kb;
                 DG_FLAST(S->f);
-                dg_score Sl = dg_inFrani(c, (int)rb.nL, th, S->Hx , &iterID, mk_full, mk_ex, &kb);
+                dg_score Sl = dg_inFrani<LDSPTS, FT>(c, (int)rb.nL, th, S->Hx , &iterID, mk_full, mk_ex, &kb);
                 if (Sl.J > 0) DG_FLAST(S->Hx);
                 if (maxS.J < Sl.J) {
-                    if (dg_f_checks(c, S->Hx, c.K->L[0], (int)Sl.I, Sl, maxS, mk_full)) {
+                    if (dg_f_checks<LDSPTS, FT>(c, S->Hx, c.K->L[0], (int)Sl.I, Sl, maxS, mk_full)) {
                         maxS = Sl;
                         __syncthreads();
                         if (tid < 9) S->F[tid] = S->Hx[tid];
@@ -827,11 +830,11 @@
                         new_max = 1; accepted = 1; finKind = kb; best_sample = no_sam; t_best = wall_clock64();
                     }
                 }
-                if (new_max && !pr.legacy) {
+                if (new_max && (LEAN || !pr.legacy)) {
                     int new_sam = dg_nsamples((int)maxS.I + 1, n, 7, pr.conf);
                     if (new_sam < max_sam) max_sam = new_sam;
                 }
-                if (scb && strm >= 1 && tid == 0) {
+                if constexpr (LEAN) {} else if (scb && strm >= 1 && tid == 0) {
                     const double tau_ = maxS.J < maxSs.J ? maxS.J : maxSs.J;
                     __hip_atomic_store(&scb->tau_bits, (unsigned long long)__double_as_longlong(tau_ < 0 ? 0.0 : tau_), __ATOMIC_RELAXED,
                         __HIP_MEMORY_SCOPE_AGENT);
@@ -839,24 +842,24 @@
                 }
                 DG_PH(4);
             }
-            if (new_max && pr.legacy) {
+            if (new_max && !LEAN && pr.legacy) {
                 int new_sam = dg_nsamples((int)maxS.I + 1, n, 7, pr.conf);
                 if (new_sam < max_sam) max_sam = new_sam;
             }
         }
-        if (A.hist_out) {
-            int *hist = A.hist_out + (size_t)off + 3 * (size_t)pair;
+        if constexpr (LEAN) {} else if (DG_HIST) {
+            int *hrow = A.hist_out + (size_t)off + 3 * (size_t)pair;
             const int reached = no_sam - chunk_base;
             if (tid < reached && tid < chunk && S->nv[tid] != 255) {
                 unsigned best = 0;
                 for (int r = 0; r < S->nv[tid]; r++) { const unsigned I_ = c.K->res_I[S->moff[tid] + r]; best = I_ > best ? I_ : best; }
-                atomicAdd(&hist[2 + best], 1);
+                atomicAdd(&hrow[2 + best], 1);
             }
         }
         if (k < chunk) { c.n_fds -= (Mtot - (int)S->moff[k]); done = 1; }
         else if (no_sam >= max_sam) done = 1;
         __syncthreads();
-        if (legacy_sym && !done) {
+        if constexpr (LEAN) {} else if (legacy_sym && !done) {
             const bool cand = tid < chunk && S->nv[tid] != 255;
             const unsigned long long bal = __ballot(cand);
             if (lane == 0) S->wave_cnt[wave] = bal ? (unsigned)(wave * 64 + 63 - __clzll((long long)bal)) : 0xffffffffu;
@@ -874,7 +877,7 @@
             if (pre_cnt > 0) { mtab ^= 1; if (tid == 0) S->K.gmodels = (double *)(ws + A.wl.off_models + (size_t)mtab * DG_MTAB_BYTES); }
         }
     }
-    if (producer) {
+    if constexpr (LEAN) {} else if (producer) {
         dg_stream_publish(&scb->head, no_sam / DG_CHUNK + (no_sam % DG_CHUNK ? 1 : 0));
         __syncthreads();
         if (tid == 0) __hip_atomic_store(&scb->state, DG_ST_RELEASED, __ATOMIC_RELAXED, __HIP_MEMORY_SCOPE_AGENT);
@@ -906,7 +909,7 @@
             dg_pass_cfg ch = dg_cfg0(n); ch.flags = c.K->Fl[1]; ch.thF = th*3;
             dg_pass_res rh = dg_h_pass(c, S->H, ch); c.n_hds++;
             unsigned I = rh.nF;
-            if (I >= 8) I = dg_innerH(c, S->H, 16*th, 10, c.K->Fl[0]);
+            if (I >= 8) I = dg_innerH<LDSPTS, FT>(c, S->H, 16*th, 10, c.K->Fl[0]);
             else { for (int j = tid; j < n; j += DG_T) c.K->Fl[0][j] = 0; __syncthreads(); }
             if ((int)I > Ihmax) Ihmax = (int)I;
             if (I > 6) {
@@ -930,19 +933,19 @@
             }
         } else {
             iter_cnt++;
-            dg_resid_begin(c, iter_cnt - 1); __syncthreads();
+            if constexpr (!LEAN) { dg_resid_begin(c, iter_cnt - 1); __syncthreads(); }
             dg_pass_cfg ca = dg_cfg0(n); ca.list = c.K->L[0]; ca.thL = DG_TC * th * DG_MWM;
             dg_pass_res ra = dg_f_pass(c, S->FBest, mk_full, ca);
             dg_u2f_list(c, c.K->L[0], (int)ra.nL, 0, 0, S->f);
             dg_pass_cfg cb = dg_cfg0(n); cb.list = c.K->L[0]; cb.thL = th;
             dg_pass_res rb = dg_f_pass(c, S->f, mk_full, cb); c.n_fds++;
-            dg_dump_resid(c, 1, S->f, mk_full);
+            if constexpr (!LEAN) dg_dump_resid(c, 1, S->f, mk_full);
             int kb;
             DG_FLAST(S->f);
-            dg_score Sl = dg_inFrani(c, (int)rb.nL, th, S->Hx, &iterID, mk_full, mk_ex, &kb);
+            dg_score Sl = dg_inFrani<LDSPTS, FT>(c, (int)rb.nL, th, S->Hx, &iterID, mk_full, mk_ex, &kb);
             if (Sl.J > 0) DG_FLAST(S->Hx);
             if (maxS.J < Sl.J) {
-                if (dg_f_checks(c, S->Hx, c.K->L[0], (int)Sl.I, Sl, maxS, mk_full)) {
+                if (dg_f_checks<LDSPTS, FT>(c, S->Hx, c.K->L[0], (int)Sl.I, Sl, maxS, mk_full)) {
                     maxS = Sl;
                     __syncthreads();
                     if (tid < 9) S->F[tid] = S->Hx[tid];
@@ -1000,7 +1003,7 @@
         }
     }
     if (tid < 9) A.model_out[(size_t)pair * 9 + tid] = accepted ? S->F[tid] : 0.0;
-    if (A.hist_out && tid == 0) { int *hist = A.hist_out + (size_t)off + 3 * (size_t)pair; hist[0] = no_sam; hist[1] = iter_cnt; }
+    if (DG_HIST && tid == 0) { int *hrow = A.hist_out + (size_t)off + 3 * (size_t)pair; hrow[0] = no_sam; hrow[1] = iter_cnt; }
     if (A.screen_out && tid == 0) { int *so = A.screen_out + (size_t)pair * 4; for (int i = 0; i < 4; i++) so[i] = (int)S->scnt[i]; }
     if (A.stats_out && tid == 0) {
         int *st = A.stats_out + (size_t)pair * 16;
@@ -1008,9 +1011,9 @@
         st[0] = no_sam; st[1] = iter_cnt; st[2] = S->n_lafrej; st[3] = (int)maxS.I; st[4] = c.n_fds + c.n_exfds;
         st[5] = degen_cnt; st[6] = Ihmax; st[7] = best_sample; st[8] = c.n_fds; st[9] = c.n_exfds;
         st[10] = c.n_hds; st[11] = c.n_aux; st[12] = (int)(t_best - t_start); st[13] = (int)(t_end - t_start);
-        st[14] = A.variant_threads; st[15] = A.mode | (resume ? 256 : 0) | (strm == 2 ? 512 : 0);
+        st[14] = A.variant_threads; st[15] = A.mode | (resume ? 256 : 0) | (strm == 2 ? 512 : 0) | (LEAN ? 4096 : 0);
     }
-    if (fan) {
+    if constexpr (LEAN) {} else if (fan) {
         if (tid == 0) __hip_atomic_store(&scb->stop, 1, __ATOMIC_RELAXED, __HIP_MEMORY_SCOPE_AGENT);
     } else if (scb && strm >= 1) {
         __syncthreads();
@@ -1043,6 +1046,7 @@
     DG_DEVT(if (A.phase_out && tid == 0) { S->ph[7] = DG_CLK() - t_start; for (int i = 0; i < 8; i++) A.phase_out[(size_t)pair * 16 + i] = S->ph[i];
         for (int i = 0; i < 8; i++) A.phase_out[(size_t)pair * 16 + 8 + i] = S->dbg[i]; A.phase_out[(size_t)pair * 16 + 15] = DG_CLK(); });
 #undef DG_PH
+#undef DG_HIST
     return -1;
 }
 
@@ -1071,7 +1075,7 @@
     if (A.stats_out && threadIdx.x == 0) { A.stats_out[(size_t)pair * 16 + 3] = 0; A.stats_out[(size_t)pair * 16 + 15] |= 1024; }
 }
 
-template <int T, int LDSPTS>
+template <int T, int LDSPTS, int FT = DG_FT_FULL>
 __global__ __launch_bounds__(DG_T, DG_MINW) void dg_find_fundamental_kernel(dg_args A)
 {
     extern __shared__ __attribute__((aligned(16))) unsigned char dyn_smem[];
@@ -1081,7 +1085,8 @@
     __shared__ dg_args As;
     if (threadIdx.x == 0) As = A;
     __syncthreads();
-    if (LDSPTS == 0 && As.fan_k > 0) {
+    constexpr bool LEAN = FT == DG_FT_LEAN;
+    if (!LEAN && LDSPTS == 0 && As.fan_k > 0) {
         const int base = As.n_res * (As.coop_k + 1);
         if ((int)blockIdx.x >= base) {
             const int w = (int)blockIdx.x - base;
@@ -1092,7 +1097,7 @@
     }
     int slot = (int)blockIdx.x, coop_gen = 0;
     DG_DEVT(if (As.phase_out && threadIdx.x == 0) { long long *o_ = As.phase_out + ((size_t)As.n_pairs + blockIdx.x) * 16; o_[10] = DG_CLK(); o_[11] = 0; });
-    if (LDSPTS == 0 && As.coop_k > 0) {
+    if (!LEAN && LDSPTS == 0 && As.coop_k > 0) {
         slot = (int)blockIdx.x / (As.coop_k + 1);
         const int h = (int)blockIdx.x % (As.coop_k + 1);
         if (h != 0) { dg_f_helper<T>(As, &Sh, slot, h, &next_pair); return; }
@@ -1108,16 +1113,16 @@
             if (e >= 0) { pair = (int)(e >> 32); wsid = (int)(e & 0xffffffffll); resume = 1; }
         }
         int img_wsid = wsid, oslot = slot;
-        if (pair < 0 && As.stream_on) {
+        if constexpr (LEAN) {} else if (pair < 0 && As.stream_on) {
             const int j = dg_stream_find(As, &next_pair);
             if (j >= 0) { pair = As.scb[j].pair; img_wsid = As.scb[j].wsid; oslot = j; resume = 2; }
         }
         if (pair < 0) break;
-        const int spare = dg_f_pair<T, LDSPTS>(As, &Sh, dyn_smem, pair, slot, img_wsid, resume, coop_gen, wsid, oslot);
+        const int spare = dg_f_pair<T, LDSPTS, FT>(As, &Sh, dyn_smem, pair, slot, img_wsid, resume, coop_gen, wsid, oslot);
         if (spare >= 0) wsid = spare;
         else if (resume != 2) dg_discard_if_failed(As, pair, &next_pair);
     }
-    if (LDSPTS == 0 && As.coop_k > 0 && threadIdx.x == 0)
+    if (!LEAN && LDSPTS == 0 && As.coop_k > 0 && threadIdx.x == 0)
         __hip_atomic_store(&As.coop[slot].gen, -1, __ATOMIC_RELAXED, __HIP_MEMORY_SCOPE_AGENT);
     DG_DEVT(if (As.phase_out && threadIdx.x == 0) As.phase_out[((size_t)As.n_pairs + blockIdx.x) * 16] = DG_CLK());
     DG_DEVT(if (As.phase_out && (threadIdx.x & 63) == 0) As.phase_out[((size_t)As.n_pairs + blockIdx.x) * 16 + 1 + (threadIdx.x >> 6)] =
diff --git a/pydegensac_amd/csrc/dg_variant.h b/pydegensac_amd/csrc/dg_variant.h
--- a/pydegensac_amd/csrc/dg_variant.h
+++ b/pydegensac_amd/csrc/dg_variant.h
@@ -8,9 +8,10 @@
 #define DG_VARIANT_DECL(T_) \
     hipError_t dg_variant_##T_##_init(const unsigned C[8][32], const unsigned Ct[32][8], const unsigned G[32], const unsigned T[31][32], int max_lds, \
         int static_lds[2]); \
-    hipError_t dg_variant_##T_##_resident(int homography, int mode, size_t dyn, int *blocks_per_cu); \
-    hipError_t dg_variant_##T_##_launch(int homography, int mode, int grid, size_t dyn, hipStream_t stream, const dg_args &A);
+    hipError_t dg_variant_##T_##_resident(int homography, int mode, int features, size_t dyn, int *blocks_per_cu); \
+    hipError_t dg_variant_##T_##_launch(int homography, int mode, int features, int grid, size_t dyn, hipStream_t stream, const dg_args &A);
 DG_VARIANT_DECL(512)
 DG_VARIANT_DECL(256)
 DG_VARIANT_DECL(128)
+static inline int dg_variant_has_lean(int threads, int mode) { return threads != 128 && (mode == DG_MODE_LDS || mode == DG_MODE_POOL_LDS); }
 #endif
diff --git a/pydegensac_amd/csrc/dg_variant_impl.h b/pydegensac_amd/csrc/dg_variant_impl.h
--- a/pydegensac_amd/csrc/dg_variant_impl.h
+++ b/pydegensac_amd/csrc/dg_variant_impl.h
@@ -13,6 +13,10 @@
     hipFuncAttributes fa;
     const void *kf[3] = {(const void *)dg_find_fundamental_kernel<DG_T, DG_MODE_LDS>, (const void *)dg_find_fundamental_kernel<DG_T, DG_MODE_POOL_LDS>,
                          (const void *)dg_find_fundamental_kernel<DG_T, DG_MODE_HBM>};
+#if DG_T != 128
+    const void *kl[2] = {(const void *)dg_find_fundamental_kernel<DG_T, DG_MODE_LDS, DG_FT_LEAN>,
+                         (const void *)dg_find_fundamental_kernel<DG_T, DG_MODE_POOL_LDS, DG_FT_LEAN>};
+#endif
     const void *kh[3] = {(const void *)dg_find_homography_kernel<DG_T, DG_MODE_LDS>, (const void *)dg_find_homography_kernel<DG_T, DG_MODE_POOL_LDS>,
                          (const void *)dg_find_homography_kernel<DG_T, DG_MODE_HBM>};
     for (int h = 0; h < 2; h++) {
@@ -22,14 +26,31 @@
             if ((e = hipFuncGetAttributes(&fa, k[m])) != hipSuccess) return e;
             if ((int)fa.sharedSizeBytes > static_lds[h]) static_lds[h] = (int)fa.sharedSizeBytes;
         }
+#if DG_T != 128
+        if (!h) for (int m = 0; m < 2; m++) {
+            if ((e = hipFuncGetAttributes(&fa, kl[m])) != hipSuccess) return e;
+            if ((int)fa.sharedSizeBytes > static_lds[h]) static_lds[h] = (int)fa.sharedSizeBytes;
+        }
+#endif
         for (int m = 0; m < 2; m++)
             if ((e = hipFuncSetAttribute(k[m], hipFuncAttributeMaxDynamicSharedMemorySize, max_lds - static_lds[h] - 256)) != hipSuccess) return e;
+#if DG_T != 128
+        if (!h) for (int m = 0; m < 2; m++)
+            if ((e = hipFuncSetAttribute(kl[m], hipFuncAttributeMaxDynamicSharedMemorySize, max_lds - static_lds[h] - 256)) != hipSuccess) return e;
+#endif
     }
     return hipSuccess;
 }
 
-static const void *DG_VCAT(dg_variant_, DG_T, _fn)(int homography, int mode)
+static const void *DG_VCAT(dg_variant_, DG_T, _fn)(int homography, int mode, int features)
 {
+#if DG_T != 128
+    if (!homography && features == DG_FT_LEAN) {
+        if (mode == DG_MODE_LDS)      return (const void *)dg_find_fundamental_kernel<DG_T, DG_MODE_LDS, DG_FT_LEAN>;
+        if (mode == DG_MODE_POOL_LDS) return (const void *)dg_find_fundamental_kernel<DG_T, DG_MODE_POOL_LDS, DG_FT_LEAN>;
+    }
+#endif
+    (void)features;
     if (!homography) {
         if (mode == DG_MODE_LDS)      return (const void *)dg_find_fundamental_kernel<DG_T, DG_MODE_LDS>;
         if (mode == DG_MODE_POOL_LDS) return (const void *)dg_find_fundamental_kernel<DG_T, DG_MODE_POOL_LDS>;
@@ -40,14 +61,22 @@
     return (const void *)dg_find_homography_kernel<DG_T, DG_MODE_HBM>;
 }
 
-hipError_t DG_VCAT(dg_variant_, DG_T, _resident)(int homography, int mode, size_t dyn, int *blocks_per_cu)
+hipError_t DG_VCAT(dg_variant_, DG_T, _resident)(int homography, int mode, int features, size_t dyn, int *blocks_per_cu)
 {
-    return hipOccupancyMaxActiveBlocksPerMultiprocessor(blocks_per_cu, DG_VCAT(dg_variant_, DG_T, _fn)(homography, mode), DG_T, dyn);
+    return hipOccupancyMaxActiveBlocksPerMultiprocessor(blocks_per_cu, DG_VCAT(dg_variant_, DG_T, _fn)(homography, mode, features), DG_T, dyn);
 }
 
-hipError_t DG_VCAT(dg_variant_, DG_T, _launch)(int homography, int mode, int grid, size_t dyn, hipStream_t stream, const dg_args &A)
+hipError_t DG_VCAT(dg_variant_, DG_T, _launch)(int homography, int mode, int features, int grid, size_t dyn, hipStream_t stream, const dg_args &A)
 {
     const dim3 g(grid), b(DG_T);
+#if DG_T != 128
+    if (!homography && features == DG_FT_LEAN && (mode == DG_MODE_LDS || mode == DG_MODE_POOL_LDS)) {
+        if (mode == DG_MODE_LDS) hipLaunchKernelGGL((dg_find_fundamental_kernel<DG_T, DG_MODE_LDS, DG_FT_LEAN>), g, b, dyn, stream, A);
+        else                     hipLaunchKernelGGL((dg_find_fundamental_kernel<DG_T, DG_MODE_POOL_LDS, DG_FT_LEAN>), g, b, dyn, stream, A);
+        return hipGetLastError();
+    }
+#endif
+    (void)features;
     if (!homography) {
         if (mode == DG_MODE_LDS)           hipLaunchKernelGGL((dg_find_fundamental_kernel<DG_T, DG_MODE_LDS>), g, b, dyn, stream, A);
         else if (mode == DG_MODE_POOL_LDS) hipLaunchKernelGGL((dg_find_fundamental_kernel<DG_T, DG_MODE_POOL_LDS>), g, b, dyn, stream, A);
diff --git a/pydegensac_amd/csrc/mi_degensac_host.inc b/pydegensac_amd/csrc/mi_degensac_host.inc
--- a/pydegensac_amd/csrc/mi_degensac_host.inc
+++ b/pydegensac_amd/csrc/mi_degensac_host.inc
@@ -25,8 +25,8 @@
 struct DevState { bool init = false; int max_lds = 0, cus = 0, pool_par_ok = 0;
                   int static_lds[3][2] = {{0, 0}, {0, 0}, {0, 0}};    };
 static const int g_variant_threads[3] = {512, 256, 128};
-typedef hipError_t (*dg_resident_fn)(int, int, size_t, int *);
-typedef hipError_t (*dg_launch_fn)(int, int, int, size_t, hipStream_t, const dg_args &);
+typedef hipError_t (*dg_resident_fn)(int, int, int, size_t, int *);
+typedef hipError_t (*dg_launch_fn)(int, int, int, int, size_t, hipStream_t, const dg_args &);
 static const dg_resident_fn g_variant_resident[3] = {dg_variant_512_resident, dg_variant_256_resident, dg_variant_128_resident};
 static const dg_launch_fn   g_variant_launch[3]   = {dg_variant_512_launch, dg_variant_256_launch, dg_variant_128_launch};
 static DevState g_dev[64];
@@ -286,6 +286,31 @@
 extern "C" int mi_degensac_dev_set_lo_width(int w) { return g_lo_width.exchange(w); }
 extern "C" int mi_degensac_dev_set_knob(int v) { return g_dev_knob.exchange(v); }
 #endif
+static std::atomic<int> g_kernel_features{0};
+extern "C" int mi_degensac_set_kernel_features(int mode) { return g_kernel_features.exchange(mode == 1 ? 1 : 0); }
+static int dg_f_features(int homography, uint32_t flags, const mi_degensac_diag *diag, int trace_on, uint32_t tune, int lo_width, int n_max,
+                         int n_pairs, int threads, int mode, int stream_on, int fan_k, int coop_k, int force_full)
+{
+    (void)n_max; (void)n_pairs;
+    if (homography || force_full) return DG_FT_FULL;
+    if (flags & MI_DEGENSAC_FLAG_LEGACY_F) return DG_FT_FULL;
+    if (diag && ((diag->d_resids && diag->resid_runs > 0) || diag->d_hist)) return DG_FT_FULL;
+    if (trace_on || (tune & MI_DEGENSAC_TUNE_F_SERIAL_REPS) || lo_width > 0) return DG_FT_FULL;
+    if (stream_on || fan_k > 0 || coop_k > 0) return DG_FT_FULL;
+    return dg_variant_has_lean(threads, mode) ? DG_FT_LEAN : DG_FT_FULL;
+}
+extern "C" int mi_degensac_kernel_features_for(int homography, uint32_t flags, uint32_t tuning, int have_resids, int have_hist, int have_screen,
+        int trace, int lo_width, int n_max, int n_pairs, int threads, int mode, int stream_on, int fan_k, int coop_k)
+{
+    mi_degensac_diag d; memset(&d, 0, sizeof d); d.struct_size = (int)sizeof d;
+    static double dummy_d; static int32_t dummy_i;
+    if (have_resids) { d.d_resids = &dummy_d; d.resid_runs = 1; }
+    if (have_hist) d.d_hist = &dummy_i;
+    if (have_screen) d.d_screen = &dummy_i;
+    return dg_f_features(homography, flags, &d, trace, tuning, lo_width, n_max, n_pairs, threads, mode, stream_on, fan_k, coop_k,
+                         g_kernel_features.load()) == DG_FT_LEAN ? 1 : 0;
+}
+
 static std::atomic<long long> g_wait_ticks{400000000ll};
 extern "C" long long mi_degensac_set_wait_ticks(long long ticks) { return g_wait_ticks.exchange(ticks >= 0 ? ticks : 400000000ll); }
 
@@ -361,7 +386,7 @@
     }
     const size_t dyn = mode == DG_MODE_LDS ? dyn_all : (mode == DG_MODE_POOL_LDS ? dyn_pool : 0);
     int per_cu = 0;
-    hipError_t oe = g_variant_resident[variant](homography, mode, dyn, &per_cu);
+    hipError_t oe = g_variant_resident[variant](homography, mode, DG_FT_FULL, dyn, &per_cu);
     if (oe != hipSuccess || per_cu < 1) { (void)hipGetLastError(); per_cu = 1; }
     {
         const int by_lds = (int)((size_t)ds.max_lds / (ds.static_lds[variant][homography] + dyn + 256));
@@ -493,7 +518,13 @@
     if (diag && (size_t)diag->struct_size >= offsetof(mi_degensac_diag, d_screen) + sizeof(int32_t *) && diag->d_screen &&
         !homography) A.screen_out = diag->d_screen;
     A.model_out = d_model; A.mask_out = d_mask; A.stats_out = d_stats; A.dim = dim; A.n_pairs = n_pairs; A.pts_in_lds = mode == DG_MODE_LDS;
-    HIPCHK(g_variant_launch[variant](homography, mode, (int)grid, dyn, stream, A));
+    int trace_on = 0;
+#ifdef MI_DEGENSAC_DEV
+    trace_on = A.trace != nullptr;
+#endif
+    const int features = dg_f_features(homography, prm->flags, diag, trace_on, tune, A.lo_width, n_max, n_pairs, g_variant_threads[variant], mode,
+                                       A.stream_on, fan_k, coop_k, g_kernel_features.load());
+    HIPCHK(g_variant_launch[variant](homography, mode, features, (int)grid, dyn, stream, A));
     if (d_err_copy) HIPCHK(hipMemcpyAsync(d_err_copy, A.err_flag, sizeof(int), hipMemcpyDeviceToDevice, stream));
     return 0;
 }
```

Result: no change. 98.20 million, median of 6 (+0.9%).
